# aliftffd/ViT-vs-Raw-IQ

Hardware: AMD Instinct MI355X
Metric: IQ frames/sec training (fwd+loss+bwd+clip+AdamW) (higher is better)
Workload: dtype bf16; 1 GPU; ViT-Tiny/16 224x224 C=1 19cls (BASELINE configs[1]); config_id=B, per_gpu_batch=256, global_batch=256, parallelism=dp1, hipgraph=True

## Files before the change

### include/iqvit.h

```cpp
#ifndef IQVIT_H
#define IQVIT_H
#include <stddef.h>
#include <stdint.h>

#ifdef __cplusplus
extern "C" {
#endif

typedef void* iq_stream_t;

enum { IQ_STATUS_OK = 0, IQ_STATUS_ARG = 1, IQ_STATUS_UNSUPPORTED = 2, IQ_STATUS_LAUNCH = 3 };

typedef struct iq_dropout {
  uint64_t seed;
  uint32_t step;
  uint32_t site;
  float p;
  const uint32_t* step_dev;
} iq_dropout_t;
#define IQ_SITE_IMPAIR 0xFFFFFFFFu
#define IQ_SITE_SYNTH 0xFFFFFFFEu

int iq_ln_supported(int D);
int iq_ln_fwd(const void* z, const float* gamma, const float* beta, void* x, float* mean, float* rstd, int M, int D,
              float eps, iq_stream_t stream);
size_t iq_ln_bwd_ws_bytes(int D);
int iq_ln_bwd(const void* dx, const void* z, const float* mean, const float* rstd, const float* gamma, void* dz,
              void* dy, const iq_dropout_t* drop, float* dgamma, float* dbeta, float* ws, int accumulate, int M,
              int D, iq_stream_t stream);
int iq_ln_bwd_partial_rows(int M, int D);

typedef struct iq_epilogue {
  const float* bias;
  int relu;
  const float* pe;
  int tok, seq, cls_off;
  iq_dropout_t drop;
  const void* gate;
  int ldg;
  float gate_scale;
  const void* residual;
  int ldr;
} iq_epilogue_t;
int iq_gemm_bf16_nt(const void* A, int lda, const void* B, int ldb, void* C, int ldc, int M, int N, int K,
                    const iq_epilogue_t* epi, iq_stream_t stream);

int iq_gemm_ln_supported(int D, int K);
int iq_gemm_bf16_ln(const void* A, int lda, const void* W, int ldw, const float* bias, const void* residual, int ldr,
                    const iq_dropout_t* drop, const float* gamma, const float* beta, float eps, void* Z, void* X,
                    float* mean, float* rstd, int M, int D, int K, iq_stream_t stream);

int iq_gemm_lnbwd_supported(int D, int K);
int iq_gemm_lnbwd_partial_rows(int M);
int iq_gemm_bf16_lnbwd(const void* A, int lda, const void* Wt, int ldw, const void* residual, int ldr, const void* z,
                       const float* mean, const float* rstd, const float* gamma, const iq_dropout_t* drop, void* dz,
                       void* dy, float* partial, int M, int D, int K, iq_stream_t stream);

int iq_ffn_chain_supported(int S, int D, int F);
int iq_ffn_chain_bwd_partial_rows(int M);
size_t iq_ffn_chain_gate_bytes(int M, int F);
int iq_ffn_chain_bwd(const void* dO, const void* W2t, const void* gate_bits, float gate_scale, void* gH, const void* W1t,
                     const void* residual, const void* z1, const float* mean, const float* rstd, const float* gamma,
                     const iq_dropout_t* drop, void* dz, void* dy, float* partial, const void* Wot, void* dA, int frames, int S,
                     int D, int F, iq_stream_t stream);
int iq_qkv_dgrad_ffn_chain_bwd(const void* gQKV, const void* Wqkv_t, const void* residual0, const void* z2, const float* mean2,
                               const float* rstd2, const float* gamma2, const iq_dropout_t* drop2, void* dz2, void* dy2, float* partial2,
                               const void* W2t, const void* gate_bits, float gate_scale, void* gH, const void* W1t, const void* residual,
                               const void* z1, const float* mean, const float* rstd, const float* gamma, const iq_dropout_t* drop, void* dz,
                               void* dy, float* partial, const void* Wot, void* dA, int frames, int S, int D, int F, iq_stream_t stream);
int iq_ffn_chain_fwd(const void* X1, const void* W1, const float* b1, const iq_dropout_t* drop1, void* H, const void* W2,
                     const float* b2, const iq_dropout_t* drop2, const float* gamma, const float* beta, float eps, void* Z,
                     void* X, float* mean, float* rstd, void* gate_bits, int frames, int S, int D, int F, iq_stream_t stream);
int iq_attn_out_ffn_chain_fwd(const void* A, const void* Wo, const float* bo, const iq_dropout_t* drop0, const void* R,
                              const float* gamma1, const float* beta1, void* Z1, void* X1, float* mean1, float* rstd1,
                              const void* W1, const float* b1, const iq_dropout_t* drop1, void* H, const void* W2, const float* b2,
                              const iq_dropout_t* drop2, const float* gamma2, const float* beta2, float eps, void* Z2, void* X,
                              float* mean2, float* rstd2, void* gate_bits, const void* Wq, const float* bq, void* Yq, int frames,
                              int S, int D, int F, iq_stream_t stream);

size_t iq_wgrad_ws_bytes(int M, int N, int K);
int iq_gemm_bf16_wgrad(const void* dY, int ldy, const void* X, int ldx, float* dW, float* dbias, int M, int N, int K,
                       float* ws, size_t ws_bytes, int accumulate, iq_stream_t stream);

typedef struct iq_wgrad_problem {
  const void* dY;
  int ldy;
  const void* X;
  int ldx;
  float* dW;
  float* dbias;
  int N, K;
} iq_wgrad_problem_t;
typedef struct iq_reduce_seg {
  const float* partials;
  int rows;
  int64_t row_stride;
  float* out;
  int64_t n;
} iq_reduce_seg_t;
size_t iq_wgrad_grouped_ws_bytes(const iq_wgrad_problem_t* probs, int nprob, int M, int max_workgroups);
int iq_gemm_bf16_wgrad_grouped(const iq_wgrad_problem_t* probs, int nprob, int M, float* ws, size_t ws_bytes,
                               int accumulate, int max_workgroups, const iq_reduce_seg_t* extra, int nextra,
                               iq_stream_t stream);

#define IQ_REDUCE_JOB_SEGS 12
typedef struct iq_reduce_job_seg {
  const float* partials;
  float* out;
  int64_t n;
  int64_t stride;
  int rows;
  int blk0;
  int tall;
} iq_reduce_job_seg_t;
typedef struct iq_reduce_job {
  iq_reduce_job_seg_t seg[IQ_REDUCE_JOB_SEGS];
  int nseg;
  int nblk;
  int accumulate;
} iq_reduce_job_t;
int iq_gemm_bf16_wgrad_grouped_deferred(const iq_wgrad_problem_t* probs, int nprob, int M, float* ws, size_t ws_bytes,
                                        int accumulate, int max_workgroups, const iq_reduce_seg_t* extra, int nextra,
                                        iq_reduce_job_t* job, iq_stream_t stream);
int iq_reduce_job_run(const iq_reduce_job_t* job, iq_stream_t stream);
int iq_gemm_lnbwd_ride_workgroups(int M, int D, int K, int job_blocks);
int iq_gemm_bf16_lnbwd_ride(const void* A, int lda, const void* Wt, int ldw, const void* residual, int ldr, const void* z,
                            const float* mean, const float* rstd, const float* gamma, const iq_dropout_t* drop, void* dz,
                            void* dy, float* partial, int M, int D, int K, const iq_reduce_job_t* job, iq_stream_t stream);

int iq_attn_supported(int S, int dh);
int iq_attn_fwd(const void* qkv, void* out, float* lse, int B, int S, int H, int dh, iq_stream_t stream);
int iq_attn_bwd(const void* qkv, const void* out, const void* dout, const float* lse, void* dqkv, int B, int S, int H,
                int dh, iq_stream_t stream);
int iq_attn_fwd_masked(const void* qkv, void* out, float* lse, const uint8_t* mask, long mask_hstride, int B, int S,
                       int H, int dh, iq_stream_t stream);
int iq_attn_bwd_masked(const void* qkv, const void* out, const void* dout, const float* lse, void* dqkv,
                       const uint8_t* mask, long mask_hstride, int B, int S, int H, int dh, iq_stream_t stream);
int iq_attn_probs(const void* qkv, const float* lse, float* out, long out_bstride, int B, int S, int H, int dh,
                  int rows, int heads, iq_stream_t stream);
int iq_attn_grad_probs(const void* qkv, const float* lse, const void* dout, float* out, long out_bstride, int B, int S,
                       int H, int dh, int rows, int heads, int positive, iq_stream_t stream);
int iq_attn_relevance_step(const void* qkv, const float* lse, const void* dout, const float* r_in, float* r_out, int B,
                           int S, int H, int dh, iq_stream_t stream);

int iq_frames_preprocess(const float* raw, float* out, int n_frames, int len, int take, const float* stats,
                         iq_stream_t stream);
typedef struct iq_impair {
  float phase_lo, phase_hi;
  float cfo_lo, cfo_hi;
  int   rot90;
  int   conj;
  int   shift_max;
  float gain_db_lo, gain_db_hi;
  float snr_db_lo, snr_db_hi;
  uint64_t seed; uint32_t step;
  uint64_t frame_base;
} iq_impair_t;
int iq_frames_impair(const float* raw, float* out, float* drawn, int n_frames, int len, int take, const float* stats,
                     const iq_impair_t* imp, iq_stream_t stream);
#define IQ_SYNTH_MAX_CLASSES 128
#define IQ_SYNTH_MAX_SNRS 64
typedef struct iq_synth_class { int kind; int offset; int count; } iq_synth_class_t;
typedef struct iq_synth {
  const float* points;
  const iq_synth_class_t* classes; int n_classes;
  const float* snrs_db; int n_snrs;
  int balanced;
  uint64_t seed; uint32_t stream;
  uint64_t frame_base;
} iq_synth_t;
int iq_frames_synth(float* raw , int64_t* labels, float* snr ,
                    float* drawn ,
                    int32_t* symbols , int n_frames, int len, const iq_synth_t* par, iq_stream_t stream);
typedef struct iq_waveform {
  const float* points; const iq_synth_class_t* classes; int n_classes;
  const float* snrs_db; int n_snrs; int balanced;
  uint64_t seed; uint32_t stream; uint64_t frame_base;
  int sps;
  int span;
  int n_phase;
  int timing;
  const float* pulse;
  const int32_t* fpulse;
  int n_taps;
  float los;
  float tap_sigma[8];
} iq_waveform_t;
int iq_frames_waveform(float* raw , int64_t* labels, float* snr, float* drawn ,
                       int32_t* symbols , float* taps , int n_frames, int len,
                       const iq_waveform_t* par, iq_stream_t stream);
enum { IQ_RX_GIVEN = 0, IQ_RX_OERDER_MEYR = 1, IQ_RX_ENERGY = 2 };
typedef struct iq_receiver {
  int sps;
  int span;
  int n_frac;
  int mode;
  int normalise;
  const float* table;
  const int32_t* u;
} iq_receiver_t;
int iq_frames_receive(const float* raw , float* sym , float* est ,
                      float* energy , int n_frames, int len, const iq_receiver_t* par, iq_stream_t stream);
int iq_frames_receive_bwd(const float* dsym , const float* sym, const float* est, float* dx ,
                          int n_frames, int len, const iq_receiver_t* par, iq_stream_t stream);
typedef struct iq_spectrogram {
  int n_fft;
  int hop;
  int pad;
  int width;
  int mode;
  float inv_norm, floor, scale, shift;
} iq_spectrogram_t;
int iq_frames_spectrogram(const float* x , const float* table ,
                          float* out , int n_frames, int len, const iq_spectrogram_t* par,
                          iq_stream_t stream);
int iq_frames_spectrogram_bwd(const float* x, const float* table, const float* dout ,
                              float* dx , int n_frames, int len, const iq_spectrogram_t* par,
                              iq_stream_t stream);
typedef struct iq_cyclic {
  int n_fft;
  int hop;
  int pad;
  int columns;
  int kind;
  int mode;
  float inv_norm, floor, scale, shift;
} iq_cyclic_t;
int iq_frames_cyclic(const float* x , const float* table , const float* rot ,
                     float* out , int n_frames, int len, const iq_cyclic_t* par, iq_stream_t stream);
int iq_frames_cyclic_bwd(const float* x, const float* table, const float* rot, const float* dout ,
                         float* dx , int n_frames, int len, const iq_cyclic_t* par, iq_stream_t stream);
int iq_patchify(const float* src, void* patches, int kind, int B, int C, int H, int W, int p, int Kpad,
                iq_stream_t stream);
int iq_cls_rows(const float* cls, const float* pe, void* x0, int B, int S, int D, const iq_dropout_t* drop,
                iq_stream_t stream);
int iq_embed_bwd_gather(const void* dx0, void* demb, float* dcls, int B, int S, int tok, int D, int has_cls,
                        const iq_dropout_t* drop, int accumulate, iq_stream_t stream);
int iq_embed_dgrad(const void* demb, const void* w_bf16, int Kpad, float* dsrc, int kind, int B, int C, int H, int W, int p,
                   int D, iq_stream_t stream);
int iq_linf_step(float* x_adv, const float* grad, const float* x0, float alpha, float eps, float lo, float hi, size_t n,
                 iq_stream_t stream);

int iq_head_fwd(const void* x, const float* ln_g, const float* ln_b, const float* W, const float* b, float* featn,
                float* hstat, float* logits, int B, int S, int D, int K, int pool, iq_stream_t stream);
int iq_ce_fwd_bwd(const float* logits, const int64_t* labels, int B, int K, float smoothing, float denom,
                  float* loss_sum, int32_t* n_correct, float* dlogits, iq_stream_t stream);
int iq_head_bwd(const float* dlogits, const float* featn, const float* hstat, const float* ln_g, const float* ln_b,
                const float* W, float* dW, float* db, float* dln_g, float* dln_b, void* dx, int B, int S, int D, int K,
                int pool, int accumulate, iq_stream_t stream);

size_t iq_gradnorm_ws_bytes(size_t n);
int iq_gradnorm_sq(const float* g, size_t n, float grad_scale, float* ws, float* out, iq_stream_t stream);
int iq_adamw_step(float* p, const float* g, float* m, float* v, void* shadow_bf16, size_t n, float lr, float beta1,
                  float beta2, float eps, float weight_decay, int step, const float* gnorm_sq, float max_norm,
                  float grad_scale, const float* dyn, iq_stream_t stream);
int iq_counter_add(uint32_t* ctr_u32, uint32_t inc_u32, float* ctr_f32, float inc_f32, iq_stream_t stream);
int iq_cast_bf16(const float* src, void* dst, size_t n, iq_stream_t stream);
int iq_transpose_cast_bf16(const float* src, void* dst, int rows, int cols, iq_stream_t stream);

typedef struct iq_model_cfg {
  int kind;
  int in_channels;
  int img_h, img_w, patch;
  int seq_length, conv_k, use_cls;
  int num_classes, d_model, n_head, n_layers, ffn_hidden;
  float drop_prob;
} iq_model_cfg_t;

typedef struct iq_model iq_model_t;

int iq_model_create(const iq_model_cfg_t* cfg, iq_model_t** out);
void iq_model_destroy(iq_model_t* m);
const char* iq_model_last_error(const iq_model_t* m);
int iq_model_tokens(const iq_model_t* m);
size_t iq_model_param_floats(const iq_model_t* m);
int iq_model_param_entries(const iq_model_t* m);
int iq_model_param_entry(const iq_model_t* m, int i, char* name, int name_cap, size_t* offset, int* ndim, int* dims);
size_t iq_model_shadow_bytes(const iq_model_t* m);
size_t iq_model_workspace_bytes(const iq_model_t* m, int batch, int training);
int iq_model_bind(iq_model_t* m, float* params, float* grads, const float* pe, void* shadow);
int iq_model_bind_step_counter(iq_model_t* m, uint32_t* counter);
int iq_model_refresh_shadow(iq_model_t* m, iq_stream_t stream);
int iq_model_refresh_transposed(iq_model_t* m, iq_stream_t stream);
int iq_model_forward(iq_model_t* m, const float* src, int batch, void* workspace, size_t ws_bytes, int training,
                     uint64_t seed, uint32_t step, float* enc_out, float* logits, iq_stream_t stream);
int iq_model_backward(iq_model_t* m, const float* dlogits, const float* denc, int batch, void* workspace,
                      size_t ws_bytes, int accumulate, int stage_hi, int stage_lo, iq_stream_t stream);
int iq_model_grad_range(const iq_model_t* m, int stage_hi, int stage_lo, size_t* off, size_t* len);
#define IQ_BWD_PARAM_GRADS 1
int iq_model_backward_input(iq_model_t* m, const float* dlogits, const float* denc, int batch, void* workspace,
                            size_t ws_bytes, float* dsrc, int flags, iq_stream_t stream);
int iq_model_attention(iq_model_t* m, const void* workspace, size_t ws_bytes, int batch, int layer, int rows,
                       int heads, float* out, long out_bstride, iq_stream_t stream);
int iq_model_attention_rollout(iq_model_t* m, const void* workspace, size_t ws_bytes, int batch, float alpha,
                               float* out, iq_stream_t stream);
int iq_model_attention_relevance(iq_model_t* m, const float* dlogits, int batch, void* workspace, size_t ws_bytes,
                                 float* rel, float* const* maps, int rows, int heads, int positive, long out_bstride,
                                 iq_stream_t stream);

#define IQ_PROF_FAMILIES 8
int iq_prof_enable(int on);
int iq_prof_collect(double* ms, long long* count);
size_t iq_prof_kernels(char* out, size_t cap, int reset);

#ifdef __cplusplus
}
#endif
#endif
```

### vit-vs-raw-iq_amd/_native.py

```python
from __future__ import annotations

import ctypes as C
import os

_HERE = os.path.dirname(os.path.abspath(__file__))
LIB_PATH = os.environ.get("IQ_LIBIQVIT") or os.path.join(_HERE, "libiqvit.so")

BWD_PARAM_GRADS = 1

STATUS = {0: "ok", 1: "invalid argument", 2: "unsupported shape/configuration", 3: "HIP launch error"}


class IqError(RuntimeError):
    pass


class Dropout(C.Structure):
    _fields_ = [("seed", C.c_uint64), ("step", C.c_uint32), ("site", C.c_uint32), ("p", C.c_float),
                ("step_dev", C.c_void_p)]


class Impair(C.Structure):
    _fields_ = [("phase_lo", C.c_float), ("phase_hi", C.c_float), ("cfo_lo", C.c_float), ("cfo_hi", C.c_float),
                ("rot90", C.c_int), ("conj", C.c_int), ("shift_max", C.c_int), ("gain_db_lo", C.c_float),
                ("gain_db_hi", C.c_float), ("snr_db_lo", C.c_float), ("snr_db_hi", C.c_float), ("seed", C.c_uint64),
                ("step", C.c_uint32), ("frame_base", C.c_uint64)]


class SynthClass(C.Structure):
    _fields_ = [("kind", C.c_int), ("offset", C.c_int), ("count", C.c_int)]


class Synth(C.Structure):
    _fields_ = [("points", C.c_void_p), ("classes", C.POINTER(SynthClass)), ("n_classes", C.c_int),
                ("snrs_db", C.POINTER(C.c_float)), ("n_snrs", C.c_int), ("balanced", C.c_int), ("seed", C.c_uint64),
                ("stream", C.c_uint32), ("frame_base", C.c_uint64)]


class Waveform(C.Structure):
    _fields_ = [("points", C.c_void_p), ("classes", C.POINTER(SynthClass)), ("n_classes", C.c_int),
                ("snrs_db", C.POINTER(C.c_float)), ("n_snrs", C.c_int), ("balanced", C.c_int), ("seed", C.c_uint64),
                ("stream", C.c_uint32), ("frame_base", C.c_uint64), ("sps", C.c_int), ("span", C.c_int), ("n_phase", C.c_int),
                ("timing", C.c_int), ("pulse", C.c_void_p), ("fpulse", C.c_void_p), ("n_taps", C.c_int), ("los", C.c_float),
                ("tap_sigma", C.c_float * 8)]


class Receiver(C.Structure):
    _fields_ = [("sps", C.c_int), ("span", C.c_int), ("n_frac", C.c_int), ("mode", C.c_int), ("normalise", C.c_int),
                ("table", C.c_void_p), ("u", C.c_void_p)]


class Spectrogram(C.Structure):
    _fields_ = [("n_fft", C.c_int), ("hop", C.c_int), ("pad", C.c_int), ("width", C.c_int), ("mode", C.c_int),
                ("inv_norm", C.c_float), ("floor", C.c_float), ("scale", C.c_float), ("shift", C.c_float)]


class Cyclic(C.Structure):
    _fields_ = [("n_fft", C.c_int), ("hop", C.c_int), ("pad", C.c_int), ("columns", C.c_int), ("kind", C.c_int),
                ("mode", C.c_int), ("inv_norm", C.c_float), ("floor", C.c_float), ("scale", C.c_float), ("shift", C.c_float)]


class Epilogue(C.Structure):
    _fields_ = [("bias", C.c_void_p), ("relu", C.c_int), ("pe", C.c_void_p), ("tok", C.c_int), ("seq", C.c_int),
                ("cls_off", C.c_int), ("drop", Dropout), ("gate", C.c_void_p), ("ldg", C.c_int),
                ("gate_scale", C.c_float), ("residual", C.c_void_p), ("ldr", C.c_int)]


class WgradProblem(C.Structure):
    _fields_ = [("dY", C.c_void_p), ("ldy", C.c_int), ("X", C.c_void_p), ("ldx", C.c_int), ("dW", C.c_void_p),
                ("dbias", C.c_void_p), ("N", C.c_int), ("K", C.c_int)]


class ReduceSeg(C.Structure):
    _fields_ = [("partials", C.c_void_p), ("rows", C.c_int), ("row_stride", C.c_int64), ("out", C.c_void_p),
                ("n", C.c_int64)]


class ReduceJobSeg(C.Structure):
    _fields_ = [("partials", C.c_void_p), ("out", C.c_void_p), ("n", C.c_int64), ("stride", C.c_int64), ("rows", C.c_int),
                ("blk0", C.c_int), ("tall", C.c_int)]


class ReduceJob(C.Structure):
    _fields_ = [("seg", ReduceJobSeg * 12), ("nseg", C.c_int), ("nblk", C.c_int), ("accumulate", C.c_int)]


class ModelCfg(C.Structure):
    _fields_ = [("kind", C.c_int), ("in_channels", C.c_int), ("img_h", C.c_int), ("img_w", C.c_int),
                ("patch", C.c_int), ("seq_length", C.c_int), ("conv_k", C.c_int), ("use_cls", C.c_int),
                ("num_classes", C.c_int), ("d_model", C.c_int), ("n_head", C.c_int), ("n_layers", C.c_int),
                ("ffn_hidden", C.c_int), ("drop_prob", C.c_float)]


_P, _I, _Z, _F = C.c_void_p, C.c_int, C.c_size_t, C.c_float
_U64, _U32 = C.c_uint64, C.c_uint32

SIGNATURES = {
    "iq_ln_supported": (_I, [_I]),
    "iq_ln_fwd": (_I, [_P, _P, _P, _P, _P, _P, _I, _I, _F, _P]),
    "iq_ln_bwd_ws_bytes": (_Z, [_I]),
    "iq_ln_bwd_partial_rows": (_I, [_I, _I]),
    "iq_ln_bwd": (_I, [_P, _P, _P, _P, _P, _P, _P, C.POINTER(Dropout), _P, _P, _P, _I, _I, _I, _P]),
    "iq_gemm_bf16_nt": (_I, [_P, _I, _P, _I, _P, _I, _I, _I, _I, C.POINTER(Epilogue), _P]),
    "iq_gemm_ln_supported": (_I, [_I, _I]),
    "iq_gemm_bf16_ln": (_I, [_P, _I, _P, _I, _P, _P, _I, C.POINTER(Dropout), _P, _P, _F, _P, _P, _P, _P, _I, _I, _I, _P]),
    "iq_gemm_lnbwd_supported": (_I, [_I, _I]),
    "iq_gemm_lnbwd_partial_rows": (_I, [_I]),
    "iq_gemm_bf16_lnbwd": (_I, [_P, _I, _P, _I, _P, _I, _P, _P, _P, _P, C.POINTER(Dropout), _P, _P, _P, _I, _I, _I, _P]),
    "iq_ffn_chain_supported": (_I, [_I, _I, _I]),
    "iq_ffn_chain_bwd_partial_rows": (_I, [_I]),
    "iq_ffn_chain_bwd": (_I, [_P, _P, _P, _F, _P, _P, _P, _P, _P, _P, _P, C.POINTER(Dropout), _P, _P, _P, _P, _P, _I, _I, _I, _I, _P]),
    "iq_qkv_dgrad_ffn_chain_bwd": (_I, [_P, _P, _P, _P, _P, _P, _P, C.POINTER(Dropout), _P, _P, _P,
                                        _P, _P, _F, _P, _P, _P, _P, _P, _P, _P, C.POINTER(Dropout), _P, _P, _P, _P, _P, _I, _I, _I, _I, _P]),
    "iq_ffn_chain_gate_bytes": (_Z, [_I, _I]),
    "iq_ffn_chain_fwd": (_I, [_P, _P, _P, C.POINTER(Dropout), _P, _P, _P, C.POINTER(Dropout), _P, _P, _F, _P, _P, _P, _P, _P, _I, _I,
                              _I, _I, _P]),
    "iq_attn_out_ffn_chain_fwd": (_I, [_P, _P, _P, C.POINTER(Dropout), _P, _P, _P, _P, _P, _P, _P,
                                       _P, _P, C.POINTER(Dropout), _P, _P, _P, C.POINTER(Dropout), _P, _P, _F, _P, _P, _P, _P, _P,
                                       _P, _P, _P, _I, _I, _I, _I, _P]),
    "iq_wgrad_ws_bytes": (_Z, [_I, _I, _I]),
    "iq_gemm_bf16_wgrad": (_I, [_P, _I, _P, _I, _P, _P, _I, _I, _I, _P, _Z, _I, _P]),
    "iq_wgrad_grouped_ws_bytes": (_Z, [_P, _I, _I, _I]),
    "iq_gemm_bf16_wgrad_grouped": (_I, [_P, _I, _I, _P, _Z, _I, _I, _P, _I, _P]),
    "iq_gemm_bf16_wgrad_grouped_deferred": (_I, [_P, _I, _I, _P, _Z, _I, _I, _P, _I, C.POINTER(ReduceJob), _P]),
    "iq_reduce_job_run": (_I, [C.POINTER(ReduceJob), _P]),
    "iq_gemm_bf16_lnbwd_ride": (_I, [_P, _I, _P, _I, _P, _I, _P, _P, _P, _P, C.POINTER(Dropout), _P, _P, _P, _I, _I, _I,
                                     C.POINTER(ReduceJob), _P]),
    "iq_gemm_lnbwd_ride_workgroups": (_I, [_I, _I, _I, _I]),
    "iq_attn_supported": (_I, [_I, _I]),
    "iq_attn_fwd": (_I, [_P, _P, _P, _I, _I, _I, _I, _P]),
    "iq_attn_bwd": (_I, [_P, _P, _P, _P, _P, _I, _I, _I, _I, _P]),
    "iq_attn_fwd_masked": (_I, [_P, _P, _P, _P, C.c_long, _I, _I, _I, _I, _P]),
    "iq_attn_bwd_masked": (_I, [_P, _P, _P, _P, _P, _P, C.c_long, _I, _I, _I, _I, _P]),
    "iq_attn_probs": (_I, [_P, _P, _P, C.c_long, _I, _I, _I, _I, _I, _I, _P]),
    "iq_attn_grad_probs": (_I, [_P, _P, _P, _P, C.c_long, _I, _I, _I, _I, _I, _I, _I, _P]),
    "iq_attn_relevance_step": (_I, [_P, _P, _P, _P, _P, _I, _I, _I, _I, _P]),
    "iq_frames_preprocess": (_I, [_P, _P, _I, _I, _I, C.POINTER(C.c_float), _P]),
    "iq_frames_impair": (_I, [_P, _P, _P, _I, _I, _I, C.POINTER(C.c_float), C.POINTER(Impair), _P]),
    "iq_frames_synth": (_I, [_P, _P, _P, _P, _P, _I, _I, C.POINTER(Synth), _P]),
    "iq_frames_waveform": (_I, [_P, _P, _P, _P, _P, _P, _I, _I, C.POINTER(Waveform), _P]),
    "iq_frames_receive": (_I, [_P, _P, _P, _P, _I, _I, C.POINTER(Receiver), _P]),
    "iq_frames_receive_bwd": (_I, [_P, _P, _P, _P, _I, _I, C.POINTER(Receiver), _P]),
    "iq_frames_spectrogram": (_I, [_P, _P, _P, _I, _I, C.POINTER(Spectrogram), _P]),
    "iq_frames_spectrogram_bwd": (_I, [_P, _P, _P, _P, _I, _I, C.POINTER(Spectrogram), _P]),
    "iq_frames_cyclic": (_I, [_P, _P, _P, _P, _I, _I, C.POINTER(Cyclic), _P]),
    "iq_frames_cyclic_bwd": (_I, [_P, _P, _P, _P, _P, _I, _I, C.POINTER(Cyclic), _P]),
    "iq_patchify": (_I, [_P, _P, _I, _I, _I, _I, _I, _I, _I, _P]),
    "iq_cls_rows": (_I, [_P, _P, _P, _I, _I, _I, C.POINTER(Dropout), _P]),
    "iq_embed_bwd_gather": (_I, [_P, _P, _P, _I, _I, _I, _I, _I, C.POINTER(Dropout), _I, _P]),
    "iq_embed_dgrad": (_I, [_P, _P, _I, _P, _I, _I, _I, _I, _I, _I, _I, _P]),
    "iq_linf_step": (_I, [_P, _P, _P, _F, _F, _F, _F, _Z, _P]),
    "iq_head_fwd": (_I, [_P, _P, _P, _P, _P, _P, _P, _P, _I, _I, _I, _I, _I, _P]),
    "iq_ce_fwd_bwd": (_I, [_P, _P, _I, _I, _F, _F, _P, _P, _P, _P]),
    "iq_head_bwd": (_I, [_P, _P, _P, _P, _P, _P, _P, _P, _P, _P, _P, _I, _I, _I, _I, _I, _I, _P]),
    "iq_gradnorm_ws_bytes": (_Z, [_Z]),
    "iq_gradnorm_sq": (_I, [_P, _Z, _F, _P, _P, _P]),
    "iq_adamw_step": (_I, [_P, _P, _P, _P, _P, _Z, _F, _F, _F, _F, _F, _I, _P, _F, _F, _P, _P]),
    "iq_counter_add": (_I, [_P, _U32, _P, _F, _P]),
    "iq_cast_bf16": (_I, [_P, _P, _Z, _P]),
    "iq_transpose_cast_bf16": (_I, [_P, _P, _I, _I, _P]),
    "iq_model_create": (_I, [C.POINTER(ModelCfg), C.POINTER(_P)]),
    "iq_model_destroy": (None, [_P]),
    "iq_model_last_error": (C.c_char_p, [_P]),
    "iq_model_tokens": (_I, [_P]),
    "iq_model_param_floats": (_Z, [_P]),
    "iq_model_param_entries": (_I, [_P]),
    "iq_model_param_entry": (_I, [_P, _I, C.c_char_p, _I, C.POINTER(_Z), C.POINTER(_I), C.POINTER(_I)]),
    "iq_model_shadow_bytes": (_Z, [_P]),
    "iq_model_workspace_bytes": (_Z, [_P, _I, _I]),
    "iq_model_bind": (_I, [_P, _P, _P, _P, _P]),
    "iq_model_bind_step_counter": (_I, [_P, _P]),
    "iq_model_refresh_shadow": (_I, [_P, _P]),
    "iq_model_refresh_transposed": (_I, [_P, _P]),
    "iq_model_forward": (_I, [_P, _P, _I, _P, _Z, _I, _U64, _U32, _P, _P, _P]),
    "iq_model_backward": (_I, [_P, _P, _P, _I, _P, _Z, _I, _I, _I, _P]),
    "iq_model_grad_range": (_I, [_P, _I, _I, C.POINTER(_Z), C.POINTER(_Z)]),
    "iq_model_backward_input": (_I, [_P, _P, _P, _I, _P, _Z, _P, _I, _P]),
    "iq_model_attention": (_I, [_P, _P, _Z, _I, _I, _I, _I, _P, C.c_long, _P]),
    "iq_model_attention_rollout": (_I, [_P, _P, _Z, _I, _F, _P, _P]),
    "iq_model_attention_relevance": (_I, [_P, _P, _I, _P, _Z, _P, C.POINTER(_P), _I, _I, _I, C.c_long, _P]),
    "iq_prof_enable": (_I, [_I]),
    "iq_prof_collect": (_I, [C.POINTER(C.c_double), C.POINTER(C.c_longlong)]),
    "iq_prof_kernels": (_Z, [C.c_char_p, _Z, _I]),
}

_lib = None


def lib():
    global _lib
    if _lib is None:
        if not os.path.exists(LIB_PATH):
            raise IqError(
                f"{LIB_PATH} not found: the HIP extension is not built. Run "
                "`python -c 'import __graft_entry__ as g; g.build()'` (or `make -C vit-vs-raw-iq_amd/csrc`). "
                "There is no CPU fallback.")
        L = C.CDLL(LIB_PATH)
        for name, (res, args) in SIGNATURES.items():
            fn = getattr(L, name)
            fn.restype = res
            fn.argtypes = args
        _lib = L
    return _lib


def check(rc, what, model=None):
    if rc != 0:
        detail = ""
        if model is not None:
            msg = lib().iq_model_last_error(model)
            if msg:
                detail = ": " + msg.decode()
        raise IqError(f"{what} failed: {STATUS.get(rc, rc)}{detail}")


def ptr(t):
    return None if t is None else t.data_ptr()


def stream_handle():
    import torch
    return torch.cuda.current_stream().cuda_stream
```

### vit-vs-raw-iq_amd/csrc/layernorm.hip

```cpp
#include "common.h"
#include "iqvit.h"
#include "prof.h"

namespace {

template <int LPR>
__device__ __forceinline__ float group_sum(float v) {
#pragma unroll
  for (int o = LPR / 2; o > 0; o >>= 1) v += __shfl_xor(v, o, 64);
  return v;
}

constexpr int LN_THREADS = 256;

template <int LPR, int NV, bool MASK = false>
__global__ __launch_bounds__(LN_THREADS) void ln_fwd_kernel(const bf16* __restrict__ Z, const float* __restrict__ gamma,
                                                            const float* __restrict__ beta, bf16* __restrict__ X,
                                                            float* __restrict__ mean_out, float* __restrict__ rstd_out,
                                                            int M, int D, float eps) {
  constexpr int RPW = 64 / LPR;
  constexpr int RPB = RPW * (LN_THREADS / 64);
  const int lane = threadIdx.x & 63, wave = threadIdx.x >> 6;
  const int j = lane % LPR, rsub = lane / LPR;
  float g[NV][8], b[NV][8];
#pragma unroll
  for (int v = 0; v < NV; ++v) {
    const int c = (v * LPR + j) * 8;
    const bool cv = !MASK || c < D;
#pragma unroll
    for (int e = 0; e < 8; ++e) { g[v][e] = cv ? gamma[c + e] : 0.f; b[v][e] = cv ? beta[c + e] : 0.f; }
  }
  const float invD = 1.0f / (float)D;
  for (long row0 = (long)blockIdx.x * RPB; row0 < M; row0 += (long)gridDim.x * RPB) {
    const long row = row0 + wave * RPW + rsub;
    const bool ok = row < M;
    float x[NV][8];
    float s = 0.f;
#pragma unroll
    for (int v = 0; v < NV; ++v) {
      bf16x8 t = {};
      if (ok && (!MASK || (v * LPR + j) * 8 < D)) t = *reinterpret_cast<const bf16x8*>(Z + row * D + (v * LPR + j) * 8);
      unpack8(t, x[v]);
#pragma unroll
      for (int e = 0; e < 8; ++e) s += x[v][e];
    }
    const float mean = group_sum<LPR>(s) * invD;
    float q = 0.f;
#pragma unroll
    for (int v = 0; v < NV; ++v)
#pragma unroll
      for (int e = 0; e < 8; ++e) { float d = x[v][e] - mean; q += (!MASK || (v * LPR + j) * 8 < D) ? d * d : 0.f; }
    const float var = group_sum<LPR>(q) * invD;
    const float rstd = 1.0f / sqrtf(var + eps);
    if (ok) {
#pragma unroll
      for (int v = 0; v < NV; ++v) {
        float y[8];
#pragma unroll
        for (int e = 0; e < 8; ++e) y[e] = g[v][e] * ((x[v][e] - mean) * rstd) + b[v][e];
        if (!MASK || (v * LPR + j) * 8 < D) *reinterpret_cast<bf16x8*>(X + row * D + (v * LPR + j) * 8) = pack8(y);
      }
      if (j == 0) { mean_out[row] = mean; rstd_out[row] = rstd; }
    }
  }
}

template <int LPR, int NV, bool DROP, bool MASK = false>
__global__ __launch_bounds__(LN_THREADS) void ln_bwd_kernel(const bf16* __restrict__ dX, const bf16* __restrict__ Z,
                                                            const float* __restrict__ mean_in, const float* __restrict__ rstd_in,
                                                            const float* __restrict__ gamma, bf16* __restrict__ dZ,
                                                            bf16* __restrict__ dY, IqRng rng, uint32_t thresh, float dscale,
                                                            float* __restrict__ partial, int M, int D) {
  constexpr int RPW = 64 / LPR;
  constexpr int RPB = RPW * (LN_THREADS / 64);
  extern __shared__ __attribute__((aligned(16))) float red[];
  const int lane = threadIdx.x & 63, wave = threadIdx.x >> 6;
  const int j = lane % LPR, rsub = lane / LPR;
  float g[NV][8], ag[NV][8], ab[NV][8];
#pragma unroll
  for (int v = 0; v < NV; ++v) {
    const int c = (v * LPR + j) * 8;
#pragma unroll
    for (int e = 0; e < 8; ++e) { g[v][e] = (!MASK || c < D) ? gamma[c + e] : 0.f; ag[v][e] = 0.f; ab[v][e] = 0.f; }
  }
  const float invD = 1.0f / (float)D;
  if (DROP) rng = rng_resolve(rng);
  for (long row0 = (long)blockIdx.x * RPB; row0 < M; row0 += (long)gridDim.x * RPB) {
    const long row = row0 + wave * RPW + rsub;
    const bool ok = row < M;
    float xh[NV][8], dy[NV][8];
    float mean = 0.f, rstd = 0.f;
    if (ok) { mean = mean_in[row]; rstd = rstd_in[row]; }
    float s1 = 0.f, s2 = 0.f;
#pragma unroll
    for (int v = 0; v < NV; ++v) {
      bf16x8 tz = {}, td = {};
      const bool cv = !MASK || (v * LPR + j) * 8 < D;
      if (ok && cv) {
        tz = *reinterpret_cast<const bf16x8*>(Z + row * D + (v * LPR + j) * 8);
        td = *reinterpret_cast<const bf16x8*>(dX + row * D + (v * LPR + j) * 8);
      }
      unpack8(tz, xh[v]);
      unpack8(td, dy[v]);
#pragma unroll
      for (int e = 0; e < 8; ++e) {
        xh[v][e] = cv ? (xh[v][e] - mean) * rstd : 0.f;
        ag[v][e] += dy[v][e] * xh[v][e];
        ab[v][e] += dy[v][e];
        dy[v][e] *= g[v][e];
        s1 += dy[v][e];
        s2 += dy[v][e] * xh[v][e];
      }
    }
    const float c1 = group_sum<LPR>(s1) * invD;
    const float c2 = group_sum<LPR>(s2) * invD;
    if (ok) {
#pragma unroll
      for (int v = 0; v < NV; ++v) {
        float o[8];
#pragma unroll
        for (int e = 0; e < 8; ++e) o[e] = rstd * (dy[v][e] - c1 - xh[v][e] * c2);
        const long off = row * D + (v * LPR + j) * 8;
        if (MASK && (v * LPR + j) * 8 >= D) continue;
        *reinterpret_cast<bf16x8*>(dZ + off) = pack8(o);
        if (DROP) {
          const uint32_t keep = dropout_keep8(rng, (uint64_t)off >> 3, thresh);
#pragma unroll
          for (int e = 0; e < 8; ++e) o[e] = ((keep >> e) & 1u) ? o[e] * dscale : 0.f;
          *reinterpret_cast<bf16x8*>(dY + off) = pack8(o);
        }
      }
    }
  }
  const int rslot = wave * RPW + rsub;
#pragma unroll
  for (int v = 0; v < NV; ++v) {
    const int c = (v * LPR + j) * 8;
    if (MASK && c >= D) continue;
#pragma unroll
    for (int e = 0; e < 8; ++e) {
      red[rslot * 2 * D + c + e] = ag[v][e];
      red[rslot * 2 * D + D + c + e] = ab[v][e];
    }
  }
  __syncthreads();
  for (int c = threadIdx.x; c < 2 * D; c += LN_THREADS) {
    float s = 0.f;
    for (int r = 0; r < RPB; ++r) s += red[r * 2 * D + c];
    partial[(long)blockIdx.x * 2 * D + c] = s;
  }
}

__global__ __launch_bounds__(1024) void ln_bwd_reduce_kernel(const float* __restrict__ partial, int nblk, int D,
                                                             float* __restrict__ dgamma, float* __restrict__ dbeta,
                                                             int accumulate) {
  __shared__ float sm[32][33];
  const int cl = threadIdx.x & 31, sl = threadIdx.x >> 5;
  const int c = blockIdx.x * 32 + cl;
  float s = 0.f;
  if (c < 2 * D) {
#pragma unroll 4
    for (int b = sl; b < nblk; b += 32) s += partial[(long)b * 2 * D + c];
  }
  sm[sl][cl] = s;
  __syncthreads();
  if (sl == 0 && c < 2 * D) {
    float t = 0.f;
#pragma unroll
    for (int i = 0; i < 32; ++i) t += sm[i][cl];
    float* dst = c < D ? dgamma + c : dbeta + (c - D);
    *dst = accumulate ? *dst + t : t;
  }
}

struct LnShape { int lpr, nv; };
inline bool ln_shape(int D, LnShape* s) {
  if (D <= 0 || D % 8) return false;
  int v = D / 8, lpr = 1;
  while (lpr < 64 && v % (lpr * 2) == 0) lpr *= 2;
  s->lpr = lpr; s->nv = v / lpr;
  return true;
}

template <typename F>
inline bool ln_dispatch(const LnShape& s, F&& f) {
#define IQ_LN_CASE(L, N) \
  if (s.lpr == L && s.nv == N) { f(std::integral_constant<int, L>{}, std::integral_constant<int, N>{}); return true; }
  IQ_LN_CASE(64, 1) IQ_LN_CASE(64, 2) IQ_LN_CASE(64, 3) IQ_LN_CASE(64, 4)
  IQ_LN_CASE(32, 1) IQ_LN_CASE(32, 3) IQ_LN_CASE(32, 5)
  IQ_LN_CASE(16, 1) IQ_LN_CASE(16, 3) IQ_LN_CASE(16, 5)
  IQ_LN_CASE(8, 1) IQ_LN_CASE(8, 3) IQ_LN_CASE(8, 5)
  IQ_LN_CASE(4, 1) IQ_LN_CASE(4, 3) IQ_LN_CASE(4, 5)
  IQ_LN_CASE(2, 1) IQ_LN_CASE(2, 3) IQ_LN_CASE(1, 1) IQ_LN_CASE(1, 3)
#undef IQ_LN_CASE
  return false;
}
inline int ln_masked_nv(int D) { return (D % 8 == 0 && D > 0 && D <= 2048) ? (D / 8 + 63) / 64 : 0; }
template <typename F>
inline bool ln_dispatch_masked(int D, F&& f) {
  switch (ln_masked_nv(D)) {
    case 1: f(std::integral_constant<int, 1>{}); return true;
    case 2: f(std::integral_constant<int, 2>{}); return true;
    case 3: f(std::integral_constant<int, 3>{}); return true;
    case 4: f(std::integral_constant<int, 4>{}); return true;
    default: return false;
  }
}

constexpr int LN_MAX_BLOCKS = 512;
constexpr int LN_FWD_MAX_BLOCKS = 4096;

inline int ln_grid(int M, int rpb, int cap = LN_MAX_BLOCKS) {
  long nb = ((long)M + rpb - 1) / rpb;
  if (nb > cap) nb = cap;
  if (nb < 1) nb = 1;
  return (int)nb;
}

}

extern "C" int iq_ln_supported(int D) {
  LnShape s;
  if (!ln_shape(D, &s)) return 0;
  return (ln_dispatch(s, [](auto, auto) {}) || ln_masked_nv(D) > 0) ? 1 : 0;
}

extern "C" int iq_ln_fwd(const void* z, const float* gamma, const float* beta, void* x, float* mean, float* rstd,
                         int M, int D, float eps, iq_stream_t stream) {
  LnShape s;
  if (M <= 0) return IQ_OK;
  if (!z || !gamma || !beta || !x || !mean || !rstd) return IQ_ERR_ARG;
  if (!ln_shape(D, &s)) return IQ_ERR_UNSUPPORTED;
  hipStream_t st = (hipStream_t)stream;
  IQ_PROF(IQ_FAM_LN_FWD, st);
  const double bytes = 2.0 * (double)M * D * 2 + 8.0 * M;
  bool ok = ln_dispatch(s, [&](auto lpr, auto nv) {
    constexpr int LPR = decltype(lpr)::value, NV = decltype(nv)::value;
    IQ_PROF_K(bytes, 0.0, "ln_fwd_kernel<%d, %d, false>", LPR, NV);
    ln_fwd_kernel<LPR, NV><<<ln_grid(M, (64 / LPR) * 4, LN_FWD_MAX_BLOCKS), LN_THREADS, 0, st>>>((const bf16*)z, gamma, beta, (bf16*)x, mean,
                                                                             rstd, M, D, eps);
  });
  if (!ok) ok = ln_dispatch_masked(D, [&](auto nv) {
    constexpr int NV = decltype(nv)::value;
    IQ_PROF_K(bytes, 0.0, "ln_fwd_kernel<64, %d, true>", NV);
    ln_fwd_kernel<64, NV, true><<<ln_grid(M, 4, LN_FWD_MAX_BLOCKS), LN_THREADS, 0, st>>>((const bf16*)z, gamma, beta, (bf16*)x,
                                                                                         mean, rstd, M, D, eps);
  });
  return ok ? iq_launch_status() : IQ_ERR_UNSUPPORTED;
}

extern "C" size_t iq_ln_bwd_ws_bytes(int D) { return (size_t)LN_MAX_BLOCKS * 2 * D * sizeof(float); }

extern "C" int iq_ln_bwd_partial_rows(int M, int D) {
  LnShape s;
  if (M <= 0 || !ln_shape(D, &s)) return 0;
  int rows = 0;
  bool ok = ln_dispatch(s, [&](auto lpr, auto nv) {
    constexpr int LPR = decltype(lpr)::value;
    rows = ln_grid(M, (64 / LPR) * 4);
  });
  if (!ok) rows = ln_masked_nv(D) > 0 ? ln_grid(M, 4) : 0;
  return rows;
}

extern "C" int iq_ln_bwd(const void* dx, const void* z, const float* mean, const float* rstd, const float* gamma,
                         void* dz, void* dy, const iq_dropout_t* drop, float* dgamma, float* dbeta, float* ws,
                         int accumulate, int M, int D, iq_stream_t stream) {
  LnShape s;
  if (M <= 0) return IQ_OK;
  if (!dx || !z || !mean || !rstd || !gamma || !dz || !ws) return IQ_ERR_ARG;
  if ((dgamma == nullptr) != (dbeta == nullptr)) return IQ_ERR_ARG;
  const bool reduce_now = dgamma != nullptr;
  if (!ln_shape(D, &s)) return IQ_ERR_UNSUPPORTED;
  int dropping; IqRng rng; uint32_t thresh; float dscale;
  (void)dropout_unpack(drop, &dropping, &rng, &thresh, &dscale);
  if (dropping && !dy) return IQ_ERR_ARG;
  hipStream_t st = (hipStream_t)stream;
  IQ_PROF(IQ_FAM_LN_BWD, st);
  const double bytes = 2.0 * (double)M * D * (3 + (dropping ? 1 : 0)) + 8.0 * M;
  int rc = IQ_OK;
  bool ok = ln_dispatch(s, [&](auto lpr, auto nv) {
    constexpr int LPR = decltype(lpr)::value, NV = decltype(nv)::value;
    constexpr int RPB = (64 / LPR) * 4;
    const int nblk = ln_grid(M, RPB);
    const size_t lds = (size_t)RPB * 2 * D * sizeof(float);
    if (lds > 160 * 1024) { rc = IQ_ERR_UNSUPPORTED; return; }
    IQ_PROF_K(bytes, 0.0, "ln_bwd_kernel<%d, %d, %s, false>", LPR, NV, dropping ? "true" : "false");
    if (dropping) {
      auto k = ln_bwd_kernel<LPR, NV, true>;
      if (lds > 48 * 1024) (void)hipFuncSetAttribute((const void*)k, hipFuncAttributeMaxDynamicSharedMemorySize, (int)lds);
      k<<<nblk, LN_THREADS, lds, st>>>((const bf16*)dx, (const bf16*)z, mean, rstd, gamma, (bf16*)dz, (bf16*)dy, rng,
                                       thresh, dscale, ws, M, D);
    } else {
      auto k = ln_bwd_kernel<LPR, NV, false>;
      if (lds > 48 * 1024) (void)hipFuncSetAttribute((const void*)k, hipFuncAttributeMaxDynamicSharedMemorySize, (int)lds);
      k<<<nblk, LN_THREADS, lds, st>>>((const bf16*)dx, (const bf16*)z, mean, rstd, gamma, (bf16*)dz, (bf16*)dy, rng,
                                       thresh, dscale, ws, M, D);
    }
    if (reduce_now) ln_bwd_reduce_kernel<<<(2 * D + 31) / 32, 1024, 0, st>>>(ws, nblk, D, dgamma, dbeta, accumulate);
  });
  if (!ok) ok = ln_dispatch_masked(D, [&](auto nv) {
    constexpr int NV = decltype(nv)::value;
    constexpr int RPB = 4;
    const int nblk = ln_grid(M, RPB);
    const size_t lds = (size_t)RPB * 2 * D * sizeof(float);
    IQ_PROF_K(bytes, 0.0, "ln_bwd_kernel<64, %d, %s, true>", NV, dropping ? "true" : "false");
    if (dropping)
      ln_bwd_kernel<64, NV, true, true><<<nblk, LN_THREADS, lds, st>>>((const bf16*)dx, (const bf16*)z, mean, rstd, gamma,
                                                                      (bf16*)dz, (bf16*)dy, rng, thresh, dscale, ws, M, D);
    else
      ln_bwd_kernel<64, NV, false, true><<<nblk, LN_THREADS, lds, st>>>((const bf16*)dx, (const bf16*)z, mean, rstd, gamma,
                                                                       (bf16*)dz, (bf16*)dy, rng, thresh, dscale, ws, M, D);
    if (reduce_now) ln_bwd_reduce_kernel<<<(2 * D + 31) / 32, 1024, 0, st>>>(ws, nblk, D, dgamma, dbeta, accumulate);
  });
  if (!ok) return IQ_ERR_UNSUPPORTED;
  return rc != IQ_OK ? rc : iq_launch_status();
}
```

### vit-vs-raw-iq_amd/csrc/misc.hip

```cpp
#include "common.h"
#include "iqvit.h"
#include "prof.h"

namespace {

__global__ void patchify_kernel(const float* __restrict__ src, bf16* __restrict__ dst, int kind, int B, int C, int H,
                                int W, int p, int tok, int P, int Kpad) {
  const long nchunk = (long)B * tok * (Kpad / 8);
  for (long id = (long)blockIdx.x * blockDim.x + threadIdx.x; id < nchunk; id += (long)gridDim.x * blockDim.x) {
    const int ch = (int)(id % (Kpad / 8));
    const long row = id / (Kpad / 8);
    const int b = (int)(row / tok), t = (int)(row % tok);
    float v[8];
    if (kind == 0 && (p & 7) == 0 && (W & 3) == 0 && ch * 8 < P) {
      const int k = ch * 8, gw = W / p;
      const int c = k / (p * p), rem = k % (p * p), py = rem / p, px = rem % p;
      const int gy = t / gw, gx = t % gw;
      const float* sp = src + (((long)b * C + c) * H + gy * p + py) * W + gx * p + px;
      const f32x4 a = *reinterpret_cast<const f32x4*>(sp), bq = *reinterpret_cast<const f32x4*>(sp + 4);
      v[0] = a[0]; v[1] = a[1]; v[2] = a[2]; v[3] = a[3]; v[4] = bq[0]; v[5] = bq[1]; v[6] = bq[2]; v[7] = bq[3];
      *reinterpret_cast<bf16x8*>(dst + row * Kpad + ch * 8) = pack8(v);
      continue;
    }
#pragma unroll
    for (int e = 0; e < 8; ++e) {
      const int k = ch * 8 + e;
      float x = 0.f;
      if (k < P) {
        if (kind == 0) {
          const int gw = W / p;
          const int c = k / (p * p), rem = k % (p * p), py = rem / p, px = rem % p;
          const int gy = t / gw, gx = t % gw;
          x = src[(((long)b * C + c) * H + gy * p + py) * W + gx * p + px];
        } else {
          const int c = k / p, j = k % p;
          x = src[((long)b * C + c) * H + (long)t * p + j];
        }
      }
      v[e] = x;
    }
    *reinterpret_cast<bf16x8*>(dst + row * Kpad + ch * 8) = pack8(v);
  }
}

__global__ void cls_rows_kernel(const float* __restrict__ cls, const float* __restrict__ pe, bf16* __restrict__ x0,
                                int B, int S, int D, int drop_on, IqRng rng, uint32_t thresh, float dscale) {
  const int nch = D / 8;
  const int id = blockIdx.x * blockDim.x + threadIdx.x;
  if (id >= B * nch) return;
  if (drop_on) rng = rng_resolve(rng);
  const int b = id / nch, ch = id % nch;
  float v[8];
#pragma unroll
  for (int e = 0; e < 8; ++e) v[e] = cls[ch * 8 + e] + pe[ch * 8 + e];
  const long off = (long)b * S * D + ch * 8;
  if (drop_on) {
    const uint32_t keep = dropout_keep8(rng, (uint64_t)off >> 3, thresh);
#pragma unroll
    for (int e = 0; e < 8; ++e) v[e] = ((keep >> e) & 1u) ? v[e] * dscale : 0.f;
  }
  *reinterpret_cast<bf16x8*>(x0 + off) = pack8(v);
}

__global__ void embed_bwd_gather_kernel(const bf16* __restrict__ dx0, bf16* __restrict__ demb, int B, int S, int tok,
                                        int D, int cls_off, int drop_on, IqRng rng, uint32_t thresh, float dscale) {
  const int nch = D / 8;
  const long n = (long)B * tok * nch;
  if (drop_on) rng = rng_resolve(rng);
  for (long id = (long)blockIdx.x * blockDim.x + threadIdx.x; id < n; id += (long)gridDim.x * blockDim.x) {
    const int ch = (int)(id % nch);
    const long row = id / nch;
    const int b = (int)(row / tok), t = (int)(row % tok);
    const long off = ((long)b * S + cls_off + t) * D + ch * 8;
    bf16x8 v = *reinterpret_cast<const bf16x8*>(dx0 + off);
    if (drop_on) {
      const uint32_t keep = dropout_keep8(rng, (uint64_t)off >> 3, thresh);
      float f[8];
      unpack8(v, f);
#pragma unroll
      for (int e = 0; e < 8; ++e) f[e] = ((keep >> e) & 1u) ? f[e] * dscale : 0.f;
      v = pack8(f);
    }
    *reinterpret_cast<bf16x8*>(demb + row * D + ch * 8) = v;
  }
}

__global__ __launch_bounds__(256) void dcls_kernel(const bf16* __restrict__ dx0, float* __restrict__ dcls, int B, int S, int D,
                                                   int drop_on, IqRng rng, uint32_t thresh, float dscale, int accumulate) {
  __shared__ float part[4][8];
  const int ch = blockIdx.x, lane = threadIdx.x & 63, wave = threadIdx.x >> 6;
  if (drop_on) rng = rng_resolve(rng);
  float s[8] = {0.f, 0.f, 0.f, 0.f, 0.f, 0.f, 0.f, 0.f};
  for (int b = threadIdx.x; b < B; b += 256) {
    const long off = (long)b * S * D + ch * 8;
    float v[8];
    unpack8(*reinterpret_cast<const bf16x8*>(dx0 + off), v);
    uint32_t keep = 0xffu;
    if (drop_on) keep = dropout_keep8(rng, (uint64_t)off >> 3, thresh);
#pragma unroll
    for (int e = 0; e < 8; ++e) s[e] += ((keep >> e) & 1u) ? (drop_on ? v[e] * dscale : v[e]) : 0.f;
  }
#pragma unroll
  for (int e = 0; e < 8; ++e) {
    const float t = wave_sum(s[e]);
    if (lane == 0) part[wave][e] = t;
  }
  __syncthreads();
  if (threadIdx.x < 8) {
    const float t = part[0][threadIdx.x] + part[1][threadIdx.x] + part[2][threadIdx.x] + part[3][threadIdx.x];
    float* dst = dcls + ch * 8 + threadIdx.x;
    *dst = accumulate ? *dst + t : t;
  }
}

__global__ __launch_bounds__(64) void head_fwd_kernel(const bf16* __restrict__ x, const float* __restrict__ ln_g,
                                                      const float* __restrict__ ln_b, const float* __restrict__ W,
                                                      const float* __restrict__ bias, float* __restrict__ feat_hat,
                                                      float* __restrict__ hstat, float* __restrict__ logits, int S,
                                                      int D, int K, int pool) {
  const int b = blockIdx.x, lane = threadIdx.x;
  const bf16* xb = x + (long)b * S * D;
  float* fh = feat_hat + (long)b * D;
  float s1 = 0.f;
  for (int d = lane; d < D; d += 64) {
    float f;
    if (pool == 0) {
      f = (float)xb[d];
    } else {
      f = 0.f;
      for (int s = 0; s < S; ++s) f += (float)xb[(long)s * D + d];
      f /= (float)S;
    }
    fh[d] = f;
    s1 += f;
  }
  if (ln_g) {
    const float mean = wave_sum(s1) / (float)D;
    float s2 = 0.f;
    for (int d = lane; d < D; d += 64) { const float c = fh[d] - mean; s2 += c * c; }
    const float rstd = 1.0f / sqrtf(wave_sum(s2) / (float)D + 1e-5f);
    for (int d = lane; d < D; d += 64) fh[d] = (fh[d] - mean) * rstd;
    if (lane == 0) { hstat[2 * b] = mean; hstat[2 * b + 1] = rstd; }
  }
  __syncthreads();
  if (D % 4 == 0 && D <= 1024) {
    __shared__ float fs[1024];
    for (int d = lane; d < D; d += 64) fs[d] = ln_g ? ln_g[d] * fh[d] + ln_b[d] : fh[d];
    __syncthreads();
    int lpk = 64;
    while (lpk * 4 > D) lpk >>= 1;
    if (lpk >= 1) {
      const int kpar = 64 / lpk, kk = lane / lpk, dl = lane % lpk;
      for (int k0 = 0; k0 < K; k0 += kpar * 4) {
        float a[4] = {0.f, 0.f, 0.f, 0.f};
#pragma unroll
        for (int u = 0; u < 4; ++u) {
          const int k = min(k0 + u * kpar + kk, K - 1);
          for (int d = 4 * dl; d < D; d += 4 * lpk) {
            const f32x4 w = *reinterpret_cast<const f32x4*>(W + (long)k * D + d);
            const f32x4 f = *reinterpret_cast<const f32x4*>(fs + d);
            a[u] += w[0] * f[0] + w[1] * f[1] + w[2] * f[2] + w[3] * f[3];
          }
        }
#pragma unroll
        for (int u = 0; u < 4; ++u) {
          float t = a[u];
          for (int o = lpk >> 1; o > 0; o >>= 1) t += __shfl_xor(t, o, 64);
          const int k = k0 + u * kpar + kk;
          if (dl == 0 && k < K) logits[(long)b * K + k] = t + bias[k];
        }
      }
      return;
    }
  }
  for (int k = 0; k < K; ++k) {
    float a = 0.f;
    for (int d = lane; d < D; d += 64) {
      const float f = ln_g ? ln_g[d] * fh[d] + ln_b[d] : fh[d];
      a += f * W[(long)k * D + d];
    }
    a = wave_sum(a);
    if (lane == 0) logits[(long)b * K + k] = a + bias[k];
  }
}

template <int KMAX>
__global__ __launch_bounds__(256) void ce_kernel(const float* __restrict__ logits, const int64_t* __restrict__ labels,
                                                 int B, int K, float smoothing, float denom,
                                                 float* __restrict__ loss_sum, int32_t* __restrict__ n_correct,
                                                 float* __restrict__ dlogits) {
  __shared__ float sl[256];
  __shared__ int sc[256];
  float lacc = 0.f;
  int cacc = 0;
  for (int b = threadIdx.x; b < B; b += blockDim.x) {
    const float* z = logits + (long)b * K;
    const int y = (int)labels[b];
    const bool y_ok = y >= 0 && y < K;
    if constexpr (KMAX > 0) {
      float zr[KMAX];
#pragma unroll
      for (int k = 0; k < KMAX; ++k) zr[k] = k < K ? z[k] : -3.0e38f;
      float mx = zr[0];
      int am = 0;
#pragma unroll
      for (int k = 1; k < KMAX; ++k)
        if (zr[k] > mx) { mx = zr[k]; am = k; }
      float se = 0.f, sz = 0.f, zy = 0.f;
      float ek[KMAX];
#pragma unroll
      for (int k = 0; k < KMAX; ++k) {
        ek[k] = k < K ? expf(zr[k] - mx) : 0.f;
        se += ek[k];
        sz += k < K ? zr[k] : 0.f;
        zy = k == y ? zr[k] : zy;
      }
      const float lse = mx + logf(se);
      const float sum_logp = sz - (float)K * lse;
      const float nll = y_ok ? -(zy - lse) : __builtin_nanf("");
      lacc += (1.0f - smoothing) * nll + smoothing * (-sum_logp / (float)K);
      cacc += (am == y) ? 1 : 0;
      if (dlogits) {
        const float inv = 1.0f / se;
#pragma unroll
        for (int k = 0; k < KMAX; ++k) {
          if (k < K) {
            const float tgt = (k == y ? 1.0f - smoothing : 0.f) + smoothing / (float)K;
            dlogits[(long)b * K + k] = y_ok ? (ek[k] * inv - tgt) / denom : __builtin_nanf("");
          }
        }
      }
    } else {
      float mx = z[0];
      int am = 0;
      for (int k = 1; k < K; ++k)
        if (z[k] > mx) { mx = z[k]; am = k; }
      float se = 0.f;
      for (int k = 0; k < K; ++k) se += expf(z[k] - mx);
      const float lse = mx + logf(se);
      float sum_logp = 0.f;
      for (int k = 0; k < K; ++k) sum_logp += z[k] - lse;
      const float nll = y_ok ? -(z[y] - lse) : __builtin_nanf("");
      lacc += (1.0f - smoothing) * nll + smoothing * (-sum_logp / (float)K);
      cacc += (am == y) ? 1 : 0;
      if (dlogits) {
        for (int k = 0; k < K; ++k) {
          const float pk = expf(z[k] - lse);
          const float tgt = (k == y ? 1.0f - smoothing : 0.f) + smoothing / (float)K;
          dlogits[(long)b * K + k] = y_ok ? (pk - tgt) / denom : __builtin_nanf("");
        }
      }
    }
  }
  sl[threadIdx.x] = lacc;
  sc[threadIdx.x] = cacc;
  __syncthreads();
  for (int o = 128; o > 0; o >>= 1) {
    if ((int)threadIdx.x < o) { sl[threadIdx.x] += sl[threadIdx.x + o]; sc[threadIdx.x] += sc[threadIdx.x + o]; }
    __syncthreads();
  }
  if (threadIdx.x == 0) {
    if (loss_sum) *loss_sum += sl[0];
    if (n_correct) *n_correct += sc[0];
  }
}

__global__ __launch_bounds__(256) void head_bwd_dx_kernel(const float* __restrict__ dlogits, const float* __restrict__ feat_hat,
                                                         const float* __restrict__ hstat, const float* __restrict__ ln_g,
                                                         const float* __restrict__ W, bf16* __restrict__ dx, int S,
                                                         int D, int K, int pool) {
  extern __shared__ float df[];
  const int b = blockIdx.x, lane = threadIdx.x & 63;
  const float* dl = dlogits + (long)b * K;
  const float* fh = feat_hat + (long)b * D;
  if (threadIdx.x < 64) {
    float s1 = 0.f, s2 = 0.f;
    for (int d = lane; d < D; d += 64) {
      float a = 0.f;
      for (int k = 0; k < K; ++k) a += dl[k] * W[(long)k * D + d];
      if (ln_g) {
        a *= ln_g[d];
        s1 += a;
        s2 += a * fh[d];
      }
      df[d] = a;
    }
    if (ln_g) {
      const float c1 = wave_sum(s1) / (float)D, c2 = wave_sum(s2) / (float)D;
      const float rstd = hstat[2 * b + 1];
      for (int d = lane; d < D; d += 64) df[d] = rstd * (df[d] - c1 - fh[d] * c2);
    }
  }
  __syncthreads();
  bf16* dxb = dx + (long)b * S * D;
  const float inv = 1.0f / (float)S;
  for (long i = threadIdx.x; i < (long)S * (D / 8); i += 256) {
    const int s = (int)(i / (D / 8)), ch = (int)(i % (D / 8));
    float v[8];
#pragma unroll
    for (int e = 0; e < 8; ++e) v[e] = pool == 0 ? (s == 0 ? df[ch * 8 + e] : 0.f) : df[ch * 8 + e] * inv;
    *reinterpret_cast<bf16x8*>(dxb + (long)s * D + ch * 8) = pack8(v);
  }
}

__global__ __launch_bounds__(256) void head_bwd_w_kernel(const float* __restrict__ dlogits, const float* __restrict__ feat_hat,
                                                         const float* __restrict__ ln_g, const float* __restrict__ ln_b,
                                                         const float* __restrict__ W, float* __restrict__ dW, float* __restrict__ db,
                                                         float* __restrict__ dln_g, float* __restrict__ dln_b, int B, int D, int K,
                                                         int accumulate) {
  __shared__ float sa[8][33], sb[8][33];
  const int ol = threadIdx.x & 31, sl = threadIdx.x >> 5;
  const int id = blockIdx.x * 32 + ol;
  const int k = id / D, d = id % D;
  const bool live = k < K || (k == K && ln_g);
  float a = 0.f, b2 = 0.f;
  if (live) {
    if (k < K) {
      const float g = ln_g ? ln_g[d] : 1.f, be = ln_g ? ln_b[d] : 0.f;
#pragma unroll 4
      for (int b = sl; b < B; b += 8) {
        const float dl = dlogits[(long)b * K + k];
        a += dl * (g * feat_hat[(long)b * D + d] + be);
        b2 += dl;
      }
    } else {
      for (int b = sl; b < B; b += 8) {
        float dfn = 0.f;
        for (int kk = 0; kk < K; ++kk) dfn += dlogits[(long)b * K + kk] * W[(long)kk * D + d];
        a += dfn * feat_hat[(long)b * D + d];
        b2 += dfn;
      }
    }
  }
  sa[sl][ol] = a;
  sb[sl][ol] = b2;
  __syncthreads();
  if (sl == 0 && live) {
    float ta = 0.f, tb = 0.f;
#pragma unroll
    for (int i = 0; i < 8; ++i) { ta += sa[i][ol]; tb += sb[i][ol]; }
    if (k < K) {
      dW[(long)k * D + d] = accumulate ? dW[(long)k * D + d] + ta : ta;
      if (d == 0) db[k] = accumulate ? db[k] + tb : tb;
    } else {
      dln_g[d] = accumulate ? dln_g[d] + ta : ta;
      dln_b[d] = accumulate ? dln_b[d] + tb : tb;
    }
  }
}

template <int KMAX>
__global__ __launch_bounds__(256) void head_bwd_w2_kernel(const float* __restrict__ dlogits, const float* __restrict__ feat_hat,
                                                          const float* __restrict__ ln_g, const float* __restrict__ ln_b,
                                                          const float* __restrict__ W, float* __restrict__ dW, float* __restrict__ db,
                                                          float* __restrict__ dln_g, float* __restrict__ dln_b, int B, int D, int K,
                                                          int accumulate) {
  __shared__ float sT[8][KMAX][33];
  __shared__ float sS[8][KMAX];
  __shared__ float sdl[64][KMAX];
  const int ol = threadIdx.x & 31, sl = threadIdx.x >> 5;
  const int d = blockIdx.x * 32 + ol;
  const bool live = d < D;
  float T[KMAX], sd[KMAX];
#pragma unroll
  for (int k = 0; k < KMAX; ++k) { T[k] = 0.f; sd[k] = 0.f; }
  for (int b0 = 0; b0 < B; b0 += 64) {
    __syncthreads();
    for (int i = threadIdx.x; i < 64 * KMAX; i += 256) {
      const int bb = i / KMAX, k = i - bb * KMAX;
      sdl[bb][k] = (b0 + bb < B && k < K) ? dlogits[(long)(b0 + bb) * K + k] : 0.f;
    }
    __syncthreads();
    float fv[8];
#pragma unroll
    for (int i = 0; i < 8; ++i) {
      const int bb = sl + 8 * i;
      fv[i] = (live && b0 + bb < B) ? feat_hat[(long)(b0 + bb) * D + d] : 0.f;
    }
#pragma unroll
    for (int i = 0; i < 8; ++i) {
      const int bb = sl + 8 * i;
#pragma unroll
      for (int k = 0; k < KMAX; ++k) {
        const float dl = sdl[bb][k];
        T[k] += dl * fv[i];
        sd[k] += dl;
      }
    }
  }
#pragma unroll
  for (int k = 0; k < KMAX; ++k) {
    sT[sl][k][ol] = T[k];
    if (ol == 0) sS[sl][k] = sd[k];
  }
  __syncthreads();
  if (sl == 0 && live) {
    const float g = ln_g ? ln_g[d] : 1.f, be = ln_g ? ln_b[d] : 0.f;
    float lg = 0.f, lb = 0.f;
    for (int k = 0; k < K; ++k) {
      float t = 0.f, sk = 0.f;
#pragma unroll
      for (int i = 0; i < 8; ++i) { t += sT[i][k][ol]; sk += sS[i][k]; }
      const float v = g * t + be * sk;
      dW[(long)k * D + d] = accumulate ? dW[(long)k * D + d] + v : v;
      if (d == 0) db[k] = accumulate ? db[k] + sk : sk;
      const float w = W[(long)k * D + d];
      lg += w * t;
      lb += w * sk;
    }
    if (ln_g) {
      dln_g[d] = accumulate ? dln_g[d] + lg : lg;
      dln_b[d] = accumulate ? dln_b[d] + lb : lb;
    }
  }
}

constexpr int GN_BLOCKS = 1024;

__global__ __launch_bounds__(256) void gradnorm_partial_kernel(const float* __restrict__ g, size_t n, float scale,
                                                               float* __restrict__ partial) {
  __shared__ float sm[4];
  float s = 0.f;
  const size_t n4 = n / 4;
  for (size_t i = (size_t)blockIdx.x * blockDim.x + threadIdx.x; i < n4; i += (size_t)gridDim.x * blockDim.x) {
    const f32x4 v = reinterpret_cast<const f32x4*>(g)[i];
    s += v[0] * v[0] + v[1] * v[1] + v[2] * v[2] + v[3] * v[3];
  }
  if (blockIdx.x == 0 && threadIdx.x < (n & 3)) { const float v = g[n4 * 4 + threadIdx.x]; s += v * v; }
  s = wave_sum(s);
  if ((threadIdx.x & 63) == 0) sm[threadIdx.x >> 6] = s;
  __syncthreads();
  if (threadIdx.x == 0) partial[blockIdx.x] = (sm[0] + sm[1] + sm[2] + sm[3]) * scale * scale;
}
__global__ __launch_bounds__(256) void gradnorm_final_kernel(const float* __restrict__ partial, int n, float* __restrict__ out) {
  __shared__ float sm[4];
  float s = 0.f;
  for (int i = threadIdx.x; i < n; i += 256) s += partial[i];
  s = wave_sum(s);
  if ((threadIdx.x & 63) == 0) sm[threadIdx.x >> 6] = s;
  __syncthreads();
  if (threadIdx.x == 0) out[0] = sm[0] + sm[1] + sm[2] + sm[3];
}

struct AdamParams {
  float lr, b1, b2, eps, wd, max_norm, grad_scale;
  int step;
  const float* gnorm_sq;
  const float* dyn;
};

__global__ __launch_bounds__(256) void adamw_kernel(float* __restrict__ p, const float* __restrict__ g,
                                                    float* __restrict__ m, float* __restrict__ v,
                                                    bf16* __restrict__ shadow, size_t n, AdamParams a) {
  float lr = a.lr;
  int step = a.step;
  if (a.dyn) { lr = a.dyn[0]; step = (int)a.dyn[1]; }
  float coef = a.grad_scale;
  if (a.gnorm_sq && a.max_norm > 0.f) {
    const float total = sqrtf(a.gnorm_sq[0]);
    coef *= fminf(1.0f, a.max_norm / (total + 1e-6f));
  }
  const float bc1 = 1.0f - powf(a.b1, (float)step);
  const float bc2 = 1.0f - powf(a.b2, (float)step);
  const float step_size = lr / bc1, inv_sqrt_bc2 = 1.0f / sqrtf(bc2), decay = 1.0f - lr * a.wd;
  const size_t n4 = n / 4;
  for (size_t i = (size_t)blockIdx.x * blockDim.x + threadIdx.x; i < n4; i += (size_t)gridDim.x * blockDim.x) {
    f32x4 pv = reinterpret_cast<f32x4*>(p)[i];
    const f32x4 gv = reinterpret_cast<const f32x4*>(g)[i];
    f32x4 mv = reinterpret_cast<f32x4*>(m)[i];
    f32x4 vv = reinterpret_cast<f32x4*>(v)[i];
    bf16x4 sh;
#pragma unroll
    for (int e = 0; e < 4; ++e) {
      const float gg = gv[e] * coef;
      float x = pv[e] * decay;
      mv[e] = a.b1 * mv[e] + (1.0f - a.b1) * gg;
      vv[e] = a.b2 * vv[e] + (1.0f - a.b2) * gg * gg;
      const float den = sqrtf(vv[e]) * inv_sqrt_bc2 + a.eps;
      x -= step_size * (mv[e] / den);
      pv[e] = x;
      sh[e] = (bf16)x;
    }
    reinterpret_cast<f32x4*>(p)[i] = pv;
    reinterpret_cast<f32x4*>(m)[i] = mv;
    reinterpret_cast<f32x4*>(v)[i] = vv;
    if (shadow) reinterpret_cast<bf16x4*>(shadow)[i] = sh;
  }
}

__global__ void counter_add_kernel(uint32_t* cu, uint32_t iu, float* cf, float incf) {
  if (threadIdx.x == 0 && blockIdx.x == 0) {
    if (cu) *cu += iu;
    if (cf) *cf += incf;
  }
}

__global__ __launch_bounds__(256) void cast_kernel(const float* __restrict__ src, bf16* __restrict__ dst, size_t n) {
  const size_t n4 = n / 4;
  for (size_t i = (size_t)blockIdx.x * blockDim.x + threadIdx.x; i < n4; i += (size_t)gridDim.x * blockDim.x) {
    const f32x4 v = reinterpret_cast<const f32x4*>(src)[i];
    bf16x4 o;
#pragma unroll
    for (int e = 0; e < 4; ++e) o[e] = (bf16)v[e];
    reinterpret_cast<bf16x4*>(dst)[i] = o;
  }
  if (blockIdx.x == 0 && threadIdx.x < (n & 3)) dst[n4 * 4 + threadIdx.x] = (bf16)src[n4 * 4 + threadIdx.x];
}

__global__ __launch_bounds__(256) void transpose_cast_kernel(const float* __restrict__ src, bf16* __restrict__ dst,
                                                             int rows, int cols) {
  __shared__ float t[32][33];
  const int bx = blockIdx.x * 32, by = blockIdx.y * 32;
  const int tx = threadIdx.x & 31, ty = threadIdx.x >> 5;
  for (int i = ty; i < 32; i += 8) {
    const int r = by + i, c = bx + tx;
    t[i][tx] = (r < rows && c < cols) ? src[(long)r * cols + c] : 0.f;
  }
  __syncthreads();
  for (int i = ty; i < 32; i += 8) {
    const int c = bx + i, r = by + tx;
    if (c < cols && r < rows) dst[(long)c * rows + r] = (bf16)t[tx][i];
  }
}

inline int grid_for(size_t n, int per_block, int cap) {
  size_t b = (n + per_block - 1) / per_block;
  if (b > (size_t)cap) b = cap;
  if (b < 1) b = 1;
  return (int)b;
}

}

extern "C" int iq_patchify(const float* src, void* patches, int kind, int B, int C, int H, int W, int p, int Kpad,
                           iq_stream_t stream) {
  IQ_PROF(IQ_FAM_MISC, stream);
  if (B <= 0) return IQ_OK;
  if (!src || !patches || C <= 0 || H <= 0 || p <= 0 || (Kpad % 8)) return IQ_ERR_ARG;
  int tok, P;
  if (kind == 0) {
    if (W <= 0) return IQ_ERR_ARG;
    tok = (H / p) * (W / p); P = C * p * p;
  } else if (kind == 1) {
    tok = H / p; P = C * p;
  } else {
    return IQ_ERR_ARG;
  }
  if (tok <= 0 || Kpad < P) return IQ_ERR_ARG;
  const size_t n = (size_t)B * tok * (Kpad / 8);
  patchify_kernel<<<grid_for(n, 256, 4096), 256, 0, (hipStream_t)stream>>>(src, (bf16*)patches, kind, B, C, H, W, p, tok,
                                                                          P, Kpad);
  return iq_launch_status();
}

extern "C" int iq_cls_rows(const float* cls, const float* pe, void* x0, int B, int S, int D, const iq_dropout_t* drop,
                           iq_stream_t stream) {
  IQ_PROF(IQ_FAM_MISC, stream);
  if (B <= 0) return IQ_OK;
  if (!cls || !pe || !x0 || (D % 8)) return IQ_ERR_ARG;
  int on; IqRng r; uint32_t th; float sc;
  (void)dropout_unpack(drop, &on, &r, &th, &sc);
  const int n = B * (D / 8);
  cls_rows_kernel<<<(n + 255) / 256, 256, 0, (hipStream_t)stream>>>(cls, pe, (bf16*)x0, B, S, D, on, r, th, sc);
  return iq_launch_status();
}

extern "C" int iq_embed_bwd_gather(const void* dx0, void* demb, float* dcls, int B, int S, int tok, int D, int has_cls,
                                   const iq_dropout_t* drop, int accumulate, iq_stream_t stream) {
  IQ_PROF(IQ_FAM_MISC, stream);
  if (B <= 0) return IQ_OK;
  if (!dx0 || !demb || (D % 8) || (has_cls && !dcls)) return IQ_ERR_ARG;
  int on; IqRng r; uint32_t th; float sc;
  (void)dropout_unpack(drop, &on, &r, &th, &sc);
  const size_t n = (size_t)B * tok * (D / 8);
  hipStream_t st = (hipStream_t)stream;
  embed_bwd_gather_kernel<<<grid_for(n, 256, 4096), 256, 0, st>>>((const bf16*)dx0, (bf16*)demb, B, S, tok, D,
                                                                  has_cls ? 1 : 0, on, r, th, sc);
  if (has_cls) dcls_kernel<<<D / 8, 256, 0, st>>>((const bf16*)dx0, dcls, B, S, D, on, r, th, sc, accumulate);
  return iq_launch_status();
}

extern "C" int iq_head_fwd(const void* x, const float* ln_g, const float* ln_b, const float* W, const float* b,
                           float* featn, float* hstat, float* logits, int B, int S, int D, int K, int pool,
                           iq_stream_t stream) {
  IQ_PROF(IQ_FAM_MISC, stream);
  if (B <= 0) return IQ_OK;
  if (!x || !W || !b || !featn || !logits || (ln_g && (!ln_b || !hstat))) return IQ_ERR_ARG;
  head_fwd_kernel<<<B, 64, 0, (hipStream_t)stream>>>((const bf16*)x, ln_g, ln_b, W, b, featn, hstat, logits, S, D, K, pool);
  return iq_launch_status();
}

extern "C" int iq_ce_fwd_bwd(const float* logits, const int64_t* labels, int B, int K, float smoothing, float denom,
                             float* loss_sum, int32_t* n_correct, float* dlogits, iq_stream_t stream) {
  IQ_PROF(IQ_FAM_MISC, stream);
  if (B <= 0) return IQ_OK;
  if (!logits || !labels || K <= 0 || denom <= 0.f) return IQ_ERR_ARG;
  if (K <= 32) ce_kernel<32><<<1, 256, 0, (hipStream_t)stream>>>(logits, labels, B, K, smoothing, denom, loss_sum, n_correct, dlogits);
  else ce_kernel<0><<<1, 256, 0, (hipStream_t)stream>>>(logits, labels, B, K, smoothing, denom, loss_sum, n_correct, dlogits);
  return iq_launch_status();
}

extern "C" int iq_head_bwd(const float* dlogits, const float* featn, const float* hstat, const float* ln_g,
                           const float* ln_b, const float* W, float* dW, float* db, float* dln_g, float* dln_b,
                           void* dx, int B, int S, int D, int K, int pool, int accumulate, iq_stream_t stream) {
  IQ_PROF(IQ_FAM_MISC, stream);
  if (B <= 0) return IQ_OK;
  if (!dlogits || !featn || !W || !dW || !db || !dx || (D % 8)) return IQ_ERR_ARG;
  if (ln_g && (!ln_b || !hstat || !dln_g || !dln_b)) return IQ_ERR_ARG;
  hipStream_t st = (hipStream_t)stream;
  head_bwd_dx_kernel<<<B, 256, D * sizeof(float), st>>>(dlogits, featn, hstat, ln_g, W, (bf16*)dx, S, D, K, pool);
  if (K <= 32) {
    head_bwd_w2_kernel<32><<<(D + 31) / 32, 256, 0, st>>>(dlogits, featn, ln_g, ln_b, W, dW, db, dln_g, dln_b, B, D, K, accumulate);
  } else {
    const int n = (K + 1) * D;
    head_bwd_w_kernel<<<(n + 31) / 32, 256, 0, st>>>(dlogits, featn, ln_g, ln_b, W, dW, db, dln_g, dln_b, B, D, K, accumulate);
  }
  return iq_launch_status();
}

extern "C" size_t iq_gradnorm_ws_bytes(size_t n) { (void)n; return GN_BLOCKS * sizeof(float); }

extern "C" int iq_gradnorm_sq(const float* g, size_t n, float grad_scale, float* ws, float* out, iq_stream_t stream) {
  IQ_PROF(IQ_FAM_OPT, stream);
  if (!g || !ws || !out || ((uintptr_t)g & 15)) return IQ_ERR_ARG;
  hipStream_t st = (hipStream_t)stream;
  const int nb = grid_for(n / 4 + 1, 256 * 4, GN_BLOCKS);
  gradnorm_partial_kernel<<<nb, 256, 0, st>>>(g, n, grad_scale, ws);
  gradnorm_final_kernel<<<1, 256, 0, st>>>(ws, nb, out);
  return iq_launch_status();
}

extern "C" int iq_adamw_step(float* p, const float* g, float* m, float* v, void* shadow_bf16, size_t n, float lr,
                             float beta1, float beta2, float eps, float weight_decay, int step, const float* gnorm_sq,
                             float max_norm, float grad_scale, const float* dyn, iq_stream_t stream) {
  IQ_PROF(IQ_FAM_OPT, stream);
  if (!p || !g || !m || !v || (n % 4)) return IQ_ERR_ARG;
  if (((uintptr_t)p | (uintptr_t)g | (uintptr_t)m | (uintptr_t)v) & 15) return IQ_ERR_ARG;
  if (step < 1 && !dyn) return IQ_ERR_ARG;
  AdamParams a = {lr, beta1, beta2, eps, weight_decay, max_norm, grad_scale, step, gnorm_sq, dyn};
  adamw_kernel<<<grid_for(n / 4, 256, 2048), 256, 0, (hipStream_t)stream>>>(p, g, m, v, (bf16*)shadow_bf16, n, a);
  return iq_launch_status();
}

extern "C" int iq_counter_add(uint32_t* ctr_u32, uint32_t inc_u32, float* ctr_f32, float inc_f32, iq_stream_t stream) {
  counter_add_kernel<<<1, 64, 0, (hipStream_t)stream>>>(ctr_u32, inc_u32, ctr_f32, inc_f32);
  return iq_launch_status();
}

extern "C" int iq_cast_bf16(const float* src, void* dst, size_t n, iq_stream_t stream) {
  IQ_PROF(IQ_FAM_MISC, stream);
  if (n == 0) return IQ_OK;
  if (!src || !dst || ((uintptr_t)src & 15) || ((uintptr_t)dst & 7)) return IQ_ERR_ARG;
  cast_kernel<<<grid_for(n / 4 + 1, 256, 2048), 256, 0, (hipStream_t)stream>>>(src, (bf16*)dst, n);
  return iq_launch_status();
}

extern "C" int iq_transpose_cast_bf16(const float* src, void* dst, int rows, int cols, iq_stream_t stream) {
  IQ_PROF(IQ_FAM_MISC, stream);
  if (rows <= 0 || cols <= 0) return IQ_OK;
  if (!src || !dst) return IQ_ERR_ARG;
  dim3 grid((cols + 31) / 32, (rows + 31) / 32);
  transpose_cast_kernel<<<grid, 256, 0, (hipStream_t)stream>>>(src, (bf16*)dst, rows, cols);
  return iq_launch_status();
}

__global__ __launch_bounds__(256) void frames_preprocess_kernel(const float* __restrict__ raw, float* __restrict__ out, long n_samp,
                                                                int len, int take, float i_mean, float i_std, float q_mean,
                                                                float q_std) {
  for (long id = (long)blockIdx.x * blockDim.x + threadIdx.x; id < n_samp; id += (long)gridDim.x * blockDim.x) {
    const long f = id / take;
    const int t = (int)(id - f * take);
    const float2 v = *reinterpret_cast<const float2*>(raw + (f * len + t) * 2);
    out[f * 2 * take + t] = (v.x - i_mean) / i_std;
    out[f * 2 * take + take + t] = (v.y - q_mean) / q_std;
  }
}

extern "C" int iq_frames_preprocess(const float* raw, float* out, int n_frames, int len, int take, const float* stats,
                                    iq_stream_t stream) {
  if (n_frames <= 0) return IQ_OK;
  if (!raw || !out || !stats || len <= 0 || take <= 0 || take > len) return IQ_ERR_ARG;
  if (!(stats[1] > 0.f) || !(stats[3] > 0.f)) return IQ_ERR_ARG;
  if ((uintptr_t)raw & 7) return IQ_ERR_ARG;
  hipStream_t st = (hipStream_t)stream;
  IQ_PROF(IQ_FAM_MISC, st);
  const long n = (long)n_frames * take;
  long nb = (n + 255) / 256;
  if (nb > 8192) nb = 8192;
  frames_preprocess_kernel<<<(int)nb, 256, 0, st>>>(raw, out, n, len, take, stats[0], stats[1], stats[2], stats[3]);
  return iq_launch_status();
}

int head_bwd_dx_launch(const float* dlogits, const float* featn, const float* hstat, const float* ln_g, const float* W, void* dx,
                       int B, int S, int D, int K, int pool, hipStream_t st) {
  IQ_PROF(IQ_FAM_MISC, st);
  if (B <= 0) return IQ_OK;
  head_bwd_dx_kernel<<<B, 256, D * sizeof(float), st>>>(dlogits, featn, hstat, ln_g, W, (bf16*)dx, S, D, K, pool);
  return iq_launch_status();
}

int embed_bwd_gather_launch(const void* dx0, void* demb, int B, int S, int tok, int D, int has_cls, const iq_dropout_t* drop,
                            hipStream_t st) {
  IQ_PROF(IQ_FAM_MISC, st);
  if (B <= 0) return IQ_OK;
  int on; IqRng r; uint32_t th; float sc;
  (void)dropout_unpack(drop, &on, &r, &th, &sc);
  const size_t n = (size_t)B * tok * (D / 8);
  embed_bwd_gather_kernel<<<grid_for(n, 256, 4096), 256, 0, st>>>((const bf16*)dx0, (bf16*)demb, B, S, tok, D, has_cls ? 1 : 0,
                                                                  on, r, th, sc);
  return iq_launch_status();
}

__global__ __launch_bounds__(256) void linf_step_kernel(float* __restrict__ x, const float* __restrict__ g, const float* __restrict__ x0,
                                                        float alpha, float eps, float lo, float hi, int has_lo, int has_hi, long n) {
  for (long i = (long)blockIdx.x * blockDim.x + threadIdx.x; i < n; i += (long)gridDim.x * blockDim.x) {
    const float gv = g[i];
    const float s = gv > 0.f ? 1.f : gv < 0.f ? -1.f : 0.f;
    float v = __fadd_rn(x[i], __fmul_rn(alpha, s));
    const float c = x0[i];
    v = fminf(fmaxf(v, __fsub_rn(c, eps)), __fadd_rn(c, eps));
    if (has_lo) v = fmaxf(v, lo);
    if (has_hi) v = fminf(v, hi);
    x[i] = v;
  }
}

extern "C" int iq_linf_step(float* x_adv, const float* grad, const float* x0, float alpha, float eps, float lo, float hi, size_t n,
                            iq_stream_t stream) {
  if (!x_adv || !grad || !x0) return IQ_ERR_ARG;
  if (!(alpha >= 0.f) || !(eps >= 0.f) || !(alpha < INFINITY) || !(eps < INFINITY)) return IQ_ERR_ARG;
  const bool has_lo = lo == lo, has_hi = hi == hi;
  if (has_lo && has_hi && lo > hi) return IQ_ERR_ARG;
  if (n == 0) return IQ_OK;
  hipStream_t st = (hipStream_t)stream;
  IQ_PROF(IQ_FAM_MISC, st);
  linf_step_kernel<<<grid_for(n, 256, 8192), 256, 0, st>>>(x_adv, grad, x0, alpha, eps, lo, hi, has_lo ? 1 : 0, has_hi ? 1 : 0,
                                                           (long)n);
  return iq_launch_status();
}
```

### vit-vs-raw-iq_amd/csrc/model.hip

```cpp
#include <hip/hip_runtime.h>
#include <stdio.h>
#include <string.h>

#include <string>
#include <vector>

#include "attn_maps.h"
#include "common.h"
#include "iqvit.h"
#include "prof.h"

int head_bwd_dx_launch(const float* dlogits, const float* featn, const float* hstat, const float* ln_g, const float* W, void* dx,
                       int B, int S, int D, int K, int pool, hipStream_t st);
int embed_bwd_gather_launch(const void* dx0, void* demb, int B, int S, int tok, int D, int has_cls, const iq_dropout_t* drop,
                            hipStream_t st);

namespace {

struct Entry {
  std::string name;
  size_t off;
  int ndim;
  int dims[4];
};

struct LayerOff {
  size_t wqkv, bqkv, wo, bo, g1, be1, w1, b1, w2, b2, g2, be2, end;
  size_t t_wqkv, t_wo, t_w1, t_w2;
};

inline size_t align_up(size_t v, size_t a) { return (v + a - 1) / a * a; }

struct WsPlan {
  size_t step_ctr, patches, x0, head_feat, head_stat;
  struct L { size_t qkv, att, lse, z1, mean1, rstd1, x1, hid, gate, z2, mean2, rstd2, x2; };
  std::vector<L> layers;
  size_t gA, gB, gAtt, demb, wgrad_ws, wgrad_ws_bytes, ln_part[3], embw_scratch;
  size_t gZ, gY, gZ1, gY1, gH, gQKV;
  size_t total;
};

__global__ void bf16_to_f32_kernel(const bf16* __restrict__ s, float* __restrict__ d, size_t n8) {
  for (size_t i = (size_t)blockIdx.x * blockDim.x + threadIdx.x; i < n8; i += (size_t)gridDim.x * blockDim.x) {
    const bf16x8 v = reinterpret_cast<const bf16x8*>(s)[i];
    f32x4 a = {(float)v[0], (float)v[1], (float)v[2], (float)v[3]};
    f32x4 b = {(float)v[4], (float)v[5], (float)v[6], (float)v[7]};
    reinterpret_cast<f32x4*>(d)[2 * i] = a;
    reinterpret_cast<f32x4*>(d)[2 * i + 1] = b;
  }
}
__global__ void f32_into_bf16_kernel(const float* __restrict__ s, bf16* __restrict__ d, size_t n8, int add) {
  for (size_t i = (size_t)blockIdx.x * blockDim.x + threadIdx.x; i < n8; i += (size_t)gridDim.x * blockDim.x) {
    const f32x4 a = reinterpret_cast<const f32x4*>(s)[2 * i], b = reinterpret_cast<const f32x4*>(s)[2 * i + 1];
    float f[8] = {a[0], a[1], a[2], a[3], b[0], b[1], b[2], b[3]};
    if (add) {
      const bf16x8 o = reinterpret_cast<const bf16x8*>(d)[i];
#pragma unroll
      for (int e = 0; e < 8; ++e) f[e] += (float)o[e];
    }
    reinterpret_cast<bf16x8*>(d)[i] = pack8(f);
  }
}
__global__ void cast_pad_kernel(const float* __restrict__ s, bf16* __restrict__ d, int rows, int cols, int ld) {
  const long n = (long)rows * ld;
  for (long i = (long)blockIdx.x * blockDim.x + threadIdx.x; i < n; i += (long)gridDim.x * blockDim.x) {
    const int r = (int)(i / ld), c = (int)(i % ld);
    d[i] = (bf16)(c < cols ? s[(long)r * cols + c] : 0.f);
  }
}
__global__ void unpad_kernel(const float* __restrict__ s, float* __restrict__ d, int rows, int cols, int ld, int add) {
  const long n = (long)rows * cols;
  for (long i = (long)blockIdx.x * blockDim.x + threadIdx.x; i < n; i += (long)gridDim.x * blockDim.x) {
    const int r = (int)(i / cols), c = (int)(i % cols);
    const float v = s[(long)r * ld + c];
    d[i] = add ? d[i] + v : v;
  }
}
struct TransDesc { unsigned long long src_off, dst_off; int rows, cols, tile0, tiles_x; };
__global__ __launch_bounds__(256) void transpose_table_kernel(const float* __restrict__ params, unsigned char* __restrict__ shadow,
                                                              const TransDesc* __restrict__ tab, int nent) {
  __shared__ float t[32][33];
  int e = 0;
  while (e + 1 < nent && (int)blockIdx.x >= tab[e + 1].tile0) ++e;
  const TransDesc d = tab[e];
  const int local = blockIdx.x - d.tile0;
  const int bx = (local % d.tiles_x) * 32, by = (local / d.tiles_x) * 32;
  const float* src = params + d.src_off;
  bf16* dst = reinterpret_cast<bf16*>(shadow + d.dst_off);
  const int tx = threadIdx.x & 31, ty = threadIdx.x >> 5;
  for (int i = ty; i < 32; i += 8) {
    const int r = by + i, c = bx + tx;
    t[i][tx] = (r < d.rows && c < d.cols) ? src[(long)r * d.cols + c] : 0.f;
  }
  __syncthreads();
  for (int i = ty; i < 32; i += 8) {
    const int c = bx + i, r = by + tx;
    if (c < d.cols && r < d.rows) dst[(long)c * d.rows + r] = (bf16)t[tx][i];
  }
}

__global__ void rel_start_kernel(float* r, int n, int S, int cls) {
  for (int i = blockIdx.x * blockDim.x + threadIdx.x; i < n; i += gridDim.x * blockDim.x) {
    const int k = i % S;
    r[i] = cls ? (k == 0 ? 1.f : 0.f) : 1.0f / S;
  }
}

struct RelHook {
  float* const* maps;
  int rows, heads, positive;
  long bstride;
  float* rel;
  float* r[2];
};

__global__ void set_u32_kernel(uint32_t* p, uint32_t v, int bump) {
  if (threadIdx.x == 0 && blockIdx.x == 0) *p = bump ? *p + 1u : v;
}

inline int blocks_for(size_t n, int cap = 4096) {
  size_t b = (n + 255) / 256;
  if (b > (size_t)cap) b = cap;
  if (b < 1) b = 1;
  return (int)b;
}

}

struct iq_model {
  iq_model_cfg_t c;
  int S, tok, has_cls, P, Ppad, dh, pool, head_ln;
  std::vector<Entry> entries;
  size_t nparam;
  size_t emb_w, emb_b, cls, emb_end;
  std::vector<LayerOff> L;
  size_t hln_g, hln_b, head_w, head_b, head_begin;
  size_t sh_flat, sh_embw, sh_table, shadow_bytes;
  std::vector<TransDesc> ttab;
  int ttiles = 0;
  const void* table_uploaded_to = nullptr;
  float* params = nullptr;
  float* grads = nullptr;
  const float* pe = nullptr;
  unsigned char* shadow = nullptr;
  std::string err;
  uint32_t* step_ctr = nullptr;
  uint64_t last_seed = 0;
  bool last_tr = false;
  bool last_train_fwd = false;
  const void* fwd_ws = nullptr;
  int fwd_batch = 0;

  iq_dropout_t bwd_site(uint32_t id, const uint32_t* step_dev, bool tr) const {
    iq_dropout_t d;
    d.seed = last_seed; d.step = 0; d.site = id; d.p = tr ? c.drop_prob : 0.f; d.step_dev = step_dev;
    return d;
  }

  size_t add(const std::string& name, std::vector<int> dims, size_t& cur, bool aligned = true) {
    if (aligned) cur = align_up(cur, 64);
    Entry e;
    e.name = name; e.off = cur; e.ndim = (int)dims.size();
    size_t n = 1;
    for (int i = 0; i < 4; ++i) { e.dims[i] = i < e.ndim ? dims[i] : 1; n *= (size_t)e.dims[i]; }
    entries.push_back(e);
    cur += n;
    return e.off;
  }
  const bf16* sh(size_t off) const { return reinterpret_cast<const bf16*>(shadow + sh_flat) + off; }
  const bf16* sht(size_t byte_off) const { return reinterpret_cast<const bf16*>(shadow + byte_off); }
};

namespace {

int fail(iq_model* m, int code, const std::string& msg) {
  if (m) m->err = msg;
  return code;
}

WsPlan plan_ws(const iq_model* m, int B) {
  WsPlan w;
  const size_t D = m->c.d_model, F = m->c.ffn_hidden, S = m->S, H = m->c.n_head;
  const size_t M = (size_t)B * S, MT = (size_t)B * m->tok;
  size_t cur = 0;
  auto take = [&](size_t bytes) { size_t o = cur; cur = align_up(cur + bytes, 256); return o; };
  w.step_ctr = take(256);
  w.patches = take(MT * m->Ppad * 2);
  w.x0 = take(M * D * 2);
  w.head_feat = take((size_t)B * D * 4);
  w.head_stat = take((size_t)B * 2 * 4);
  w.layers.resize(m->c.n_layers);
  for (auto& l : w.layers) {
    l.qkv = take(M * 3 * D * 2);
    l.att = take(M * D * 2);
    l.lse = take((size_t)B * H * S * 4);
    l.z1 = take(M * D * 2);
    l.mean1 = take(M * 4);
    l.rstd1 = take(M * 4);
    l.x1 = take(M * D * 2);
    l.hid = take(M * F * 2);
    l.gate = take(iq_ffn_chain_gate_bytes((int)M, (int)F));
    l.z2 = take(M * D * 2);
    l.mean2 = take(M * 4);
    l.rstd2 = take(M * 4);
    l.x2 = take(M * D * 2);
  }
  w.gA = take(M * D * 2);
  w.gB = take(M * D * 2);
  w.gZ = take(M * D * 2);
  w.gY = take(M * D * 2);
  w.gZ1 = take(M * D * 2);
  w.gY1 = take(M * D * 2);
  w.gH = take(M * F * 2);
  w.gQKV = take(M * 3 * D * 2);
  w.gAtt = take(M * D * 2);
  w.demb = take(MT * D * 2);
  size_t wb = 0;
  auto mx = [&](size_t v) { if (v > wb) wb = v; };
  {
    iq_wgrad_problem_t g[4];
    memset(g, 0, sizeof(g));
    g[0].N = (int)D; g[0].K = (int)F;
    g[1].N = (int)F; g[1].K = (int)D;
    g[2].N = (int)D; g[2].K = (int)D;
    g[3].N = (int)(3 * D); g[3].K = (int)D;
    mx(iq_wgrad_grouped_ws_bytes(g, 4, (int)M, 0));
    for (int k = 0; k < 4; ++k) mx(iq_wgrad_grouped_ws_bytes(g + k, 1, (int)M, 0));
  }
  mx(iq_wgrad_ws_bytes((int)MT, (int)D, m->Ppad));
  w.wgrad_ws_bytes = wb;
  w.wgrad_ws = take(wb);
  size_t ln_rows_fused = (size_t)iq_gemm_lnbwd_partial_rows((int)M);
  if ((size_t)iq_ffn_chain_bwd_partial_rows((int)M) > ln_rows_fused) ln_rows_fused = (size_t)iq_ffn_chain_bwd_partial_rows((int)M);
  ln_rows_fused *= 2 * D * sizeof(float);
  const size_t ln_bytes = ln_rows_fused > iq_ln_bwd_ws_bytes((int)D) ? ln_rows_fused : iq_ln_bwd_ws_bytes((int)D);
  for (int k = 0; k < 3; ++k) w.ln_part[k] = take(ln_bytes);
  w.embw_scratch = take((size_t)D * m->Ppad * 4 + 256);
  w.total = cur;
  return w;
}

inline bool use_fused_ln(int D, int K) { return iq_gemm_ln_supported(D, K) && (D <= 192 || K <= 256); }

struct Route {
  bool chain;
  bool chain_takes_qkv_dgrad;
};
inline Route layer_route(int M, int S, int D, int F) {
  Route r;
  r.chain = iq_ffn_chain_supported(S, D, F) && M >= 8192;
  r.chain_takes_qkv_dgrad = r.chain && M <= 32768;
  return r;
}

#define IQ_TRY(expr, what)                                                              \
  do {                                                                                  \
    int rc_ = (expr);                                                                   \
    if (rc_ != IQ_OK) return fail(m, rc_, std::string(what) + " failed (status " + std::to_string(rc_) + ")"); \
  } while (0)

iq_dropout_t site(const iq_model* m, uint64_t seed, const uint32_t* step_dev, uint32_t id, bool training) {
  iq_dropout_t d;
  d.seed = seed; d.step = 0; d.site = id; d.p = training ? m->c.drop_prob : 0.f; d.step_dev = step_dev;
  return d;
}

}

extern "C" int iq_model_create(const iq_model_cfg_t* cfg, iq_model_t** out) {
  if (!cfg || !out) return IQ_ERR_ARG;
  *out = nullptr;
  iq_model* m = new iq_model();
  m->c = *cfg;
  const iq_model_cfg_t& c = m->c;
  auto bad = [&](const char* msg) { fprintf(stderr, "iq_model_create: %s\n", msg); delete m; return IQ_ERR_UNSUPPORTED; };
  if (c.d_model <= 0 || c.n_head <= 0 || c.n_layers < 0 || c.ffn_hidden <= 0 || c.num_classes <= 0 || c.in_channels <= 0)
    { delete m; return IQ_ERR_ARG; }
  if (c.d_model % c.n_head) return bad("d_model must be divisible by n_head");
  m->dh = c.d_model / c.n_head;
  if (m->dh != 16 && m->dh != 32 && m->dh != 64) return bad("head dim (d_model/n_head) must be 16, 32 or 64");
  if (c.ffn_hidden % 8) return bad("ffn_hidden must be a multiple of 8");
  if (!iq_ln_supported(c.d_model)) return bad("d_model not supported by the LayerNorm kernel");
  if (!(c.drop_prob >= 0.f && c.drop_prob < 1.f)) return bad("drop_prob must be in [0,1)");
  if (c.kind == 0) {
    if (c.patch <= 0 || c.img_h < c.patch || c.img_w < c.patch) return bad("bad image / patch size");
    m->tok = (c.img_h / c.patch) * (c.img_w / c.patch);
    m->has_cls = 1;
    m->P = c.in_channels * c.patch * c.patch;
    m->pool = 0;
    m->head_ln = 0;
  } else if (c.kind == 1) {
    if (c.conv_k <= 0 || c.seq_length < c.conv_k || (c.seq_length % c.conv_k)) return bad("bad seq_length / segment_size");
    m->tok = c.seq_length / c.conv_k;
    m->has_cls = c.use_cls ? 1 : 0;
    m->P = c.in_channels * c.conv_k;
    m->pool = m->has_cls ? 0 : 1;
    m->head_ln = 1;
  } else {
    delete m;
    return IQ_ERR_ARG;
  }
  m->S = m->tok + m->has_cls;
  m->Ppad = (int)align_up((size_t)m->P, 32);
  if (!iq_attn_supported(m->S, m->dh)) return bad("sequence too long for the attention backward kernel at this head dim");

  const int D = c.d_model, F = c.ffn_hidden, K = c.num_classes;
  size_t cur = 0;
  const std::string emb = c.kind == 0 ? "encoder.patch_embedding.projection" : "encoder.sequence_embedding.projection";
  if (c.kind == 0) m->emb_w = m->add(emb + ".weight", {D, c.in_channels, c.patch, c.patch}, cur);
  else m->emb_w = m->add(emb + ".weight", {D, c.in_channels, c.conv_k}, cur);
  m->emb_b = m->add(emb + ".bias", {D}, cur);
  m->cls = 0;
  if (m->has_cls) m->cls = m->add("encoder.cls_token", {1, 1, D}, cur);
  cur = align_up(cur, 64);
  m->emb_end = cur;
  m->L.resize(c.n_layers);
  for (int i = 0; i < c.n_layers; ++i) {
    LayerOff& o = m->L[i];
    const std::string p = "encoder.layers." + std::to_string(i) + ".";
    o.wqkv = m->add(p + "attention.w_q.weight", {D, D}, cur);
    m->add(p + "attention.w_k.weight", {D, D}, cur, false);
    m->add(p + "attention.w_v.weight", {D, D}, cur, false);
    o.bqkv = m->add(p + "attention.w_q.bias", {D}, cur);
    m->add(p + "attention.w_k.bias", {D}, cur, false);
    m->add(p + "attention.w_v.bias", {D}, cur, false);
    o.wo = m->add(p + "attention.w_concat.weight", {D, D}, cur);
    o.bo = m->add(p + "attention.w_concat.bias", {D}, cur);
    o.g1 = m->add(p + "norm1.gamma", {D}, cur);
    o.be1 = m->add(p + "norm1.beta", {D}, cur);
    o.w1 = m->add(p + "ffn.linear1.weight", {F, D}, cur);
    o.b1 = m->add(p + "ffn.linear1.bias", {F}, cur);
    o.w2 = m->add(p + "ffn.linear2.weight", {D, F}, cur);
    o.b2 = m->add(p + "ffn.linear2.bias", {D}, cur);
    o.g2 = m->add(p + "norm2.gamma", {D}, cur);
    o.be2 = m->add(p + "norm2.beta", {D}, cur);
    cur = align_up(cur, 64);
    o.end = cur;
  }
  m->head_begin = cur;
  m->hln_g = m->hln_b = 0;
  if (m->head_ln) {
    m->hln_g = m->add("mlp_head.0.weight", {D}, cur);
    m->hln_b = m->add("mlp_head.0.bias", {D}, cur);
    m->head_w = m->add("mlp_head.1.weight", {K, D}, cur);
    m->head_b = m->add("mlp_head.1.bias", {K}, cur);
  } else {
    m->head_w = m->add("mlp_head.weight", {K, D}, cur);
    m->head_b = m->add("mlp_head.bias", {K}, cur);
  }
  m->nparam = align_up(cur, 64);

  size_t sb = 0;
  m->sh_flat = sb; sb = align_up(sb + m->nparam * 2, 256);
  m->sh_embw = sb; sb = align_up(sb + (size_t)D * m->Ppad * 2, 256);
  for (auto& o : m->L) {
    o.t_wqkv = sb; sb = align_up(sb + (size_t)3 * D * D * 2, 256);
    o.t_wo = sb; sb = align_up(sb + (size_t)D * D * 2, 256);
    o.t_w1 = sb; sb = align_up(sb + (size_t)F * D * 2, 256);
    o.t_w2 = sb; sb = align_up(sb + (size_t)D * F * 2, 256);
  }
  for (auto& o : m->L) {
    auto push = [&](size_t src, size_t dst, int rows, int cols) {
      TransDesc d;
      d.src_off = src; d.dst_off = dst; d.rows = rows; d.cols = cols; d.tile0 = m->ttiles; d.tiles_x = (cols + 31) / 32;
      m->ttiles += d.tiles_x * ((rows + 31) / 32);
      m->ttab.push_back(d);
    };
    push(o.wqkv, o.t_wqkv, 3 * D, D);
    push(o.wo, o.t_wo, D, D);
    push(o.w1, o.t_w1, F, D);
    push(o.w2, o.t_w2, D, F);
  }
  m->sh_table = sb; sb = align_up(sb + m->ttab.size() * sizeof(TransDesc) + 64, 256);
  m->shadow_bytes = sb;
  *out = m;
  return IQ_OK;
}

extern "C" void iq_model_destroy(iq_model_t* m) {
  if (!m) return;
  delete m;
}
extern "C" const char* iq_model_last_error(const iq_model_t* m) { return m ? m->err.c_str() : "null model"; }
extern "C" int iq_model_tokens(const iq_model_t* m) { return m ? m->S : 0; }
extern "C" size_t iq_model_param_floats(const iq_model_t* m) { return m ? m->nparam : 0; }
extern "C" int iq_model_param_entries(const iq_model_t* m) { return m ? (int)m->entries.size() : 0; }
extern "C" int iq_model_param_entry(const iq_model_t* m, int i, char* name, int name_cap, size_t* offset, int* ndim,
                                    int* dims) {
  if (!m || i < 0 || i >= (int)m->entries.size() || !name || name_cap <= 0 || !offset || !ndim || !dims) return IQ_ERR_ARG;
  const Entry& e = m->entries[i];
  snprintf(name, (size_t)name_cap, "%s", e.name.c_str());
  *offset = e.off;
  *ndim = e.ndim;
  for (int k = 0; k < 4; ++k) dims[k] = e.dims[k];
  return IQ_OK;
}
extern "C" size_t iq_model_shadow_bytes(const iq_model_t* m) { return m ? m->shadow_bytes : 0; }
extern "C" size_t iq_model_workspace_bytes(const iq_model_t* m, int batch, int training) {
  (void)training;
  if (!m || batch <= 0) return 0;
  return plan_ws(m, batch).total;
}

extern "C" int iq_model_bind(iq_model_t* m, float* params, float* grads, const float* pe, void* shadow) {
  if (!m) return IQ_ERR_ARG;
  if (!params || !pe || !shadow) return fail(m, IQ_ERR_ARG, "bind: params, pe and shadow are required");
  if (((uintptr_t)params | (uintptr_t)grads | (uintptr_t)shadow) & 255) return fail(m, IQ_ERR_ARG, "bind: buffers must be 256 B aligned");
  m->params = params; m->grads = grads; m->pe = pe; m->shadow = (unsigned char*)shadow;
  if (m->table_uploaded_to != shadow && !m->ttab.empty()) {
    if (hipMemcpy(m->shadow + m->sh_table, m->ttab.data(), m->ttab.size() * sizeof(TransDesc), hipMemcpyHostToDevice) != hipSuccess)
      return fail(m, IQ_ERR_LAUNCH, "bind: uploading the transpose table failed");
    m->table_uploaded_to = shadow;
  }
  return IQ_OK;
}

extern "C" int iq_model_bind_step_counter(iq_model_t* m, uint32_t* counter) {
  if (!m) return IQ_ERR_ARG;
  if ((uintptr_t)counter & 3) return fail(m, IQ_ERR_ARG, "bind_step_counter: counter must be 4 B aligned");
  m->step_ctr = counter;
  return IQ_OK;
}

static int refresh_impl(iq_model_t* m, bool cast_flat, iq_stream_t stream) {
  if (!m || !m->params || !m->shadow) return fail(m, IQ_ERR_ARG, "refresh_shadow: model not bound");
  hipStream_t st = (hipStream_t)stream;
  const int D = m->c.d_model;
  if (cast_flat) IQ_TRY(iq_cast_bf16(m->params, m->shadow + m->sh_flat, m->nparam, stream), "cast params");
  IQ_PROF(IQ_FAM_MISC, st);
  cast_pad_kernel<<<blocks_for((size_t)D * m->Ppad), 256, 0, st>>>(m->params + m->emb_w, (bf16*)(m->shadow + m->sh_embw), D,
                                                                  m->P, m->Ppad);
  if (m->ttiles > 0)
    transpose_table_kernel<<<m->ttiles, 256, 0, st>>>(m->params, m->shadow, (const TransDesc*)(m->shadow + m->sh_table),
                                                     (int)m->ttab.size());
  return iq_launch_status();
}

extern "C" int iq_model_refresh_shadow(iq_model_t* m, iq_stream_t stream) { return refresh_impl(m, true, stream); }
extern "C" int iq_model_refresh_transposed(iq_model_t* m, iq_stream_t stream) { return refresh_impl(m, false, stream); }

extern "C" int iq_model_forward(iq_model_t* m, const float* src, int batch, void* workspace, size_t ws_bytes,
                                int training, uint64_t seed, uint32_t step, float* enc_out, float* logits,
                                iq_stream_t stream) {
  if (!m) return IQ_ERR_ARG;
  if (!m->params || !m->shadow || !m->pe) return fail(m, IQ_ERR_ARG, "forward: model not bound");
  if (!src || !workspace || batch <= 0) return fail(m, IQ_ERR_ARG, "forward: bad arguments");
  if ((uintptr_t)workspace & 255) return fail(m, IQ_ERR_ARG, "forward: workspace must be 256 B aligned");
  const WsPlan w = plan_ws(m, batch);
  if (ws_bytes < w.total) return fail(m, IQ_ERR_ARG, "forward: workspace too small");
  hipStream_t st = (hipStream_t)stream;
  unsigned char* ws = (unsigned char*)workspace;
  const iq_model_cfg_t& c = m->c;
  const int D = c.d_model, F = c.ffn_hidden, S = m->S, H = c.n_head, B = batch;
  const int M = B * S, MT = B * m->tok;
  const Route route = layer_route(M, S, D, F);
  const bool tr = training != 0 && c.drop_prob > 0.f;
  uint32_t* step_dev = m->step_ctr ? m->step_ctr : (uint32_t*)(ws + w.step_ctr);
  m->last_tr = tr;
  m->last_train_fwd = true;
  if (tr) {
    set_u32_kernel<<<1, 64, 0, st>>>(step_dev, step, step == 0xFFFFFFFFu ? 1 : 0);
    m->last_seed = seed;
  }
  const float* P = m->params;
  m->fwd_ws = nullptr;

  if (c.kind == 0) IQ_TRY(iq_patchify(src, ws + w.patches, 0, B, c.in_channels, c.img_h, c.img_w, c.patch, m->Ppad, stream), "patchify");
  else IQ_TRY(iq_patchify(src, ws + w.patches, 1, B, c.in_channels, c.seq_length, 0, c.conv_k, m->Ppad, stream), "patchify");
  const iq_dropout_t d0 = site(m, seed, step_dev, 0, tr);
  if (m->has_cls) IQ_TRY(iq_cls_rows(P + m->cls, m->pe, ws + w.x0, B, S, D, &d0, stream), "cls rows");
  {
    iq_epilogue_t e;
    memset(&e, 0, sizeof(e));
    e.bias = P + m->emb_b; e.pe = m->pe; e.tok = m->tok; e.seq = S; e.cls_off = m->has_cls; e.drop = d0;
    IQ_TRY(iq_gemm_bf16_nt(ws + w.patches, m->Ppad, m->shadow + m->sh_embw, m->Ppad, ws + w.x0, D, MT, D, m->Ppad, &e, stream),
           "embedding GEMM");
  }
  const unsigned char* x = ws + w.x0;
  bool qkv_done = false;
  for (int l = 0; l < c.n_layers; ++l) {
    const LayerOff& o = m->L[l];
    const WsPlan::L& a = w.layers[l];
    iq_epilogue_t e;
    if (!qkv_done) {
      memset(&e, 0, sizeof(e));
      e.bias = P + o.bqkv;
      IQ_TRY(iq_gemm_bf16_nt(x, D, m->sh(o.wqkv), D, ws + a.qkv, 3 * D, M, 3 * D, D, &e, stream), "qkv GEMM");
    }
    qkv_done = false;
    IQ_TRY(iq_attn_fwd(ws + a.qkv, ws + a.att, (float*)(ws + a.lse), B, S, H, m->dh, stream), "attention fwd");
    const iq_dropout_t dr1 = site(m, seed, step_dev, 1 + 3 * l, tr);
    const iq_dropout_t drh = site(m, seed, step_dev, 2 + 3 * l, tr);
    const iq_dropout_t dr2 = site(m, seed, step_dev, 3 + 3 * l, tr);
    if (route.chain) {
      const bool next = l + 1 < c.n_layers;
      IQ_TRY(iq_attn_out_ffn_chain_fwd(ws + a.att, m->sh(o.wo), P + o.bo, &dr1, x, P + o.g1, P + o.be1, ws + a.z1, ws + a.x1,
                                       (float*)(ws + a.mean1), (float*)(ws + a.rstd1), m->sh(o.w1), P + o.b1, &drh, ws + a.hid,
                                       m->sh(o.w2), P + o.b2, &dr2, P + o.g2, P + o.be2, 1e-12f, ws + a.z2, ws + a.x2,
                                       (float*)(ws + a.mean2), (float*)(ws + a.rstd2), ws + a.gate,
                                       next ? m->sh(m->L[l + 1].wqkv) : nullptr, next ? P + m->L[l + 1].bqkv : nullptr,
                                       next ? ws + w.layers[l + 1].qkv : nullptr, B, S, D, F, stream),
             "out-proj + norm1 + ffn chain + norm2 (+ next q,k,v)");
      qkv_done = next;
      x = ws + a.x2;
      continue;
    }
    if (use_fused_ln(D, D)) {
      IQ_TRY(iq_gemm_bf16_ln(ws + a.att, D, m->sh(o.wo), D, P + o.bo, x, D, &dr1, P + o.g1, P + o.be1, 1e-12f, ws + a.z1,
                             ws + a.x1, (float*)(ws + a.mean1), (float*)(ws + a.rstd1), M, D, D, stream), "out-proj GEMM + norm1");
    } else {
      memset(&e, 0, sizeof(e));
      e.bias = P + o.bo; e.drop = dr1; e.residual = x; e.ldr = D;
      IQ_TRY(iq_gemm_bf16_nt(ws + a.att, D, m->sh(o.wo), D, ws + a.z1, D, M, D, D, &e, stream), "out-proj GEMM");
      IQ_TRY(iq_ln_fwd(ws + a.z1, P + o.g1, P + o.be1, ws + a.x1, (float*)(ws + a.mean1), (float*)(ws + a.rstd1), M, D, 1e-12f, stream), "norm1");
    }
    memset(&e, 0, sizeof(e));
    e.bias = P + o.b1; e.relu = 1; e.drop = drh;
    IQ_TRY(iq_gemm_bf16_nt(ws + a.x1, D, m->sh(o.w1), D, ws + a.hid, F, M, F, D, &e, stream), "ffn1 GEMM");
    if (use_fused_ln(D, F)) {
      IQ_TRY(iq_gemm_bf16_ln(ws + a.hid, F, m->sh(o.w2), F, P + o.b2, ws + a.x1, D, &dr2, P + o.g2, P + o.be2, 1e-12f,
                             ws + a.z2, ws + a.x2, (float*)(ws + a.mean2), (float*)(ws + a.rstd2), M, D, F, stream), "ffn2 GEMM + norm2");
    } else {
      memset(&e, 0, sizeof(e));
      e.bias = P + o.b2; e.drop = dr2; e.residual = ws + a.x1; e.ldr = D;
      IQ_TRY(iq_gemm_bf16_nt(ws + a.hid, F, m->sh(o.w2), F, ws + a.z2, D, M, D, F, &e, stream), "ffn2 GEMM");
      IQ_TRY(iq_ln_fwd(ws + a.z2, P + o.g2, P + o.be2, ws + a.x2, (float*)(ws + a.mean2), (float*)(ws + a.rstd2), M, D, 1e-12f, stream), "norm2");
    }
    x = ws + a.x2;
  }
  if (logits) {
    IQ_TRY(iq_head_fwd(x, m->head_ln ? P + m->hln_g : nullptr, m->head_ln ? P + m->hln_b : nullptr, P + m->head_w,
                       P + m->head_b, (float*)(ws + w.head_feat), (float*)(ws + w.head_stat), logits, B, S, D,
                       c.num_classes, m->pool, stream), "head");
  }
  if (enc_out) bf16_to_f32_kernel<<<blocks_for((size_t)M * D / 8), 256, 0, st>>>((const bf16*)x, enc_out, (size_t)M * D / 8);
  const int rc = iq_launch_status();
  if (rc == IQ_OK) { m->fwd_ws = workspace; m->fwd_batch = batch; }
  return rc;
}

static int maps_check(iq_model_t* m, const void* workspace, size_t ws_bytes, int batch, const char* what, WsPlan* w) {
  if (!workspace || batch <= 0) return fail(m, IQ_ERR_ARG, std::string(what) + ": bad arguments");
  if (!m->fwd_ws) return fail(m, IQ_ERR_ARG, std::string(what) + ": no forward has run in a workspace");
  if (m->fwd_ws != workspace) return fail(m, IQ_ERR_ARG, std::string(what) + ": the last forward ran in another workspace");
  if (m->fwd_batch != batch)
    return fail(m, IQ_ERR_ARG, std::string(what) + ": the last forward in this workspace had batch " + std::to_string(m->fwd_batch) +
                                   ", not " + std::to_string(batch));
  *w = plan_ws(m, batch);
  if (ws_bytes < w->total) return fail(m, IQ_ERR_ARG, std::string(what) + ": workspace too small");
  return IQ_OK;
}

extern "C" int iq_model_attention(iq_model_t* m, const void* workspace, size_t ws_bytes, int batch, int layer, int rows,
                                  int heads, float* out, long out_bstride, iq_stream_t stream) {
  if (!m) return IQ_ERR_ARG;
  WsPlan w;
  const int rc = maps_check(m, workspace, ws_bytes, batch, "attention", &w);
  if (rc != IQ_OK) return rc;
  if (layer < 0 || layer >= m->c.n_layers) return fail(m, IQ_ERR_ARG, "attention: layer index out of range");
  if (rows < 0 || rows > 2 || heads < 0 || heads > 1) return fail(m, IQ_ERR_ARG, "attention: rows must be 0, 1 or 2 and heads 0 or 1");
  if (!out) return fail(m, IQ_ERR_ARG, "attention: out is NULL");
  const int S = m->S, H = m->c.n_head;
  if (out_bstride < (long)(heads ? 1 : H) * S * (rows == 0 ? S : 1)) return fail(m, IQ_ERR_ARG, "attention: out_bstride too small");
  const unsigned char* ws = (const unsigned char*)workspace;
  const WsPlan::L& a = w.layers[layer];
  IQ_TRY(iq_attn_probs(ws + a.qkv, (const float*)(ws + a.lse), out, out_bstride, batch, S, H, m->dh, rows, heads, stream),
         "attention probabilities");
  return IQ_OK;
}

extern "C" int iq_model_attention_rollout(iq_model_t* m, const void* workspace, size_t ws_bytes, int batch, float alpha,
                                          float* out, iq_stream_t stream) {
  if (!m) return IQ_ERR_ARG;
  WsPlan w;
  const int rc = maps_check(m, workspace, ws_bytes, batch, "attention rollout", &w);
  if (rc != IQ_OK) return rc;
  if (!(alpha >= 0.f && alpha <= 1.f)) return fail(m, IQ_ERR_ARG, "attention rollout: alpha must be in [0, 1]");
  if (!out) return fail(m, IQ_ERR_ARG, "attention rollout: out is NULL");
  const unsigned char* ws = (const unsigned char*)workspace;
  const int L = m->c.n_layers;
  const long qs = L > 1 ? (long)(w.layers[1].qkv - w.layers[0].qkv) : 0, ls = L > 1 ? (long)(w.layers[1].lse - w.layers[0].lse) : 0;
  for (int l = 0; l < L; ++l)
    if ((long)(w.layers[l].qkv - w.layers[0].qkv) != l * qs || (long)(w.layers[l].lse - w.layers[0].lse) != l * ls)
      return fail(m, IQ_ERR_UNSUPPORTED, "attention rollout: workspace layers are not evenly spaced");
  const size_t q0 = L ? w.layers[0].qkv : 0, l0 = L ? w.layers[0].lse : 0;
  IQ_TRY(attn_rollout_launch(ws + q0, qs, ws + l0, ls, L, out, batch, m->S, m->c.n_head, m->dh, m->has_cls, alpha,
                             (hipStream_t)stream),
         "attention rollout");
  return IQ_OK;
}

extern "C" int iq_model_grad_range(const iq_model_t* m, int stage_hi, int stage_lo, size_t* off, size_t* len) {
  if (!m || !off || !len) return IQ_ERR_ARG;
  const int Lr = m->c.n_layers;
  if (stage_lo < 0 || stage_hi > Lr + 1 || stage_lo > stage_hi) return IQ_ERR_ARG;
  auto begin = [&](int s) { return s == 0 ? (size_t)0 : (s <= Lr ? (s == 1 ? m->emb_end : m->L[s - 2].end) : m->head_begin); };
  auto end = [&](int s) { return s == 0 ? m->emb_end : (s <= Lr ? m->L[s - 1].end : m->nparam); };
  *off = begin(stage_lo);
  *len = end(stage_hi) - *off;
  return IQ_OK;
}

static int backward_impl(iq_model_t* m, const float* dlogits, const float* denc, int batch, void* workspace, size_t ws_bytes,
                         int accumulate, int stage_hi, int stage_lo, bool pgrads, iq_stream_t stream,
                         const RelHook* rh = nullptr) {
  if (!m->params || (pgrads && !m->grads) || !m->shadow) return fail(m, IQ_ERR_ARG, "backward: model not bound (grads required)");
  if (!workspace || batch <= 0) return fail(m, IQ_ERR_ARG, "backward: bad arguments");
  const iq_model_cfg_t& c = m->c;
  const int Lr = c.n_layers;
  if (stage_lo < 0 || stage_hi > Lr + 1 || stage_lo > stage_hi) return fail(m, IQ_ERR_ARG, "backward: bad stage range");
  const WsPlan w = plan_ws(m, batch);
  if (ws_bytes < w.total) return fail(m, IQ_ERR_ARG, "backward: workspace too small");
  hipStream_t st = (hipStream_t)stream;
  unsigned char* ws = (unsigned char*)workspace;
  const int D = c.d_model, F = c.ffn_hidden, S = m->S, H = c.n_head, B = batch, K = c.num_classes;
  const int M = B * S, MT = B * m->tok;
  const bool tr = m->last_tr;
  const uint32_t* step_dev = m->step_ctr ? m->step_ctr : (const uint32_t*)(ws + w.step_ctr);
  const float* P = m->params;
  float* G = m->grads;
  float* wws = (float*)(ws + w.wgrad_ws);
  const float dscale = tr ? dropout_scale(c.drop_prob) : 1.f;

  if (stage_hi == Lr + 1) {
    if (!dlogits && !denc) return fail(m, IQ_ERR_ARG, "backward: dlogits or denc required at the head stage");
    if (dlogits && !pgrads) {
      IQ_TRY(head_bwd_dx_launch(dlogits, (const float*)(ws + w.head_feat), (const float*)(ws + w.head_stat),
                                m->head_ln ? P + m->hln_g : nullptr, P + m->head_w, ws + w.gA, B, S, D, K, m->pool, st), "head bwd (dx)");
    } else if (dlogits) {
      IQ_TRY(iq_head_bwd(dlogits, (const float*)(ws + w.head_feat), (const float*)(ws + w.head_stat),
                         m->head_ln ? P + m->hln_g : nullptr, m->head_ln ? P + m->hln_b : nullptr, P + m->head_w,
                         G + m->head_w, G + m->head_b, m->head_ln ? G + m->hln_g : nullptr,
                         m->head_ln ? G + m->hln_b : nullptr, ws + w.gA, B, S, D, K, m->pool, accumulate, stream), "head bwd");
    } else if (!accumulate && pgrads) {
      (void)hipMemsetAsync(G + m->head_begin, 0, (m->nparam - m->head_begin) * sizeof(float), st);
    }
    if (denc) f32_into_bf16_kernel<<<blocks_for((size_t)M * D / 8), 256, 0, st>>>(denc, (bf16*)(ws + w.gA), (size_t)M * D / 8, dlogits ? 1 : 0);
  }
  const bool fuse1 = iq_gemm_lnbwd_supported(D, F) != 0, fuse2 = iq_gemm_lnbwd_supported(D, 3 * D) != 0;
  const Route route = layer_route(M, S, D, F);
  const bool chain = fuse1 && m->last_train_fwd && route.chain;
  bool deferred = false;
  for (int sidx = (stage_hi > Lr ? Lr : stage_hi); sidx >= 1 && sidx >= stage_lo; --sidx) {
    const int l = sidx - 1;
    const LayerOff& o = m->L[l];
    const WsPlan::L& a = w.layers[l];
    const unsigned char* xin = l == 0 ? ws + w.x0 : ws + w.layers[l - 1].x2;
    unsigned char *gZ = ws + w.gZ, *gY = ws + w.gY, *gZ1 = ws + w.gZ1, *gY1 = ws + w.gY1;
    unsigned char *gH = ws + w.gH, *gQKV = ws + w.gQKV;
    iq_epilogue_t e;
    auto ln2_part = [&](int layer) { return (float*)(ws + w.ln_part[(layer & 1) ? 2 : 0]); };
    float* lp2 = ln2_part(l);
    float* lp1 = (float*)(ws + w.ln_part[1]);
    const bool norm2_here = l == Lr - 1 || !fuse2;
    if (norm2_here) {
      const iq_dropout_t dr2 = m->bwd_site(3 + 3 * l, step_dev, tr);
      IQ_TRY(iq_ln_bwd(ws + w.gA, ws + a.z2, (const float*)(ws + a.mean2), (const float*)(ws + a.rstd2), P + o.g2,
                       gZ, gY, &dr2, nullptr, nullptr, lp2, accumulate, M, D, stream), "norm2 bwd");
    }
    const unsigned char* dO2 = tr ? gY : gZ;
    const unsigned char* dAo = tr ? gY1 : gZ1;
    const iq_wgrad_problem_t wg[4] = {
        {dO2, D, ws + a.hid, F, G + o.w2, G + o.b2, D, F},
        {gH, F, ws + a.x1, D, G + o.w1, G + o.b1, F, D},
        {dAo, D, ws + a.att, D, G + o.wo, G + o.bo, D, D},
        {gQKV, 3 * D, xin, D, G + o.wqkv, G + o.bqkv, 3 * D, D}};
    const int rows2 = norm2_here ? iq_ln_bwd_partial_rows(M, D) : deferred ? iq_ffn_chain_bwd_partial_rows(M) : iq_gemm_lnbwd_partial_rows(M);
    const int rows1 = chain ? iq_ffn_chain_bwd_partial_rows(M) : fuse1 ? iq_gemm_lnbwd_partial_rows(M) : iq_ln_bwd_partial_rows(M, D);
    const iq_reduce_seg_t lnseg[4] = {{lp2, rows2, 2L * D, G + o.g2, D}, {lp2 + D, rows2, 2L * D, G + o.be2, D},
                                      {lp1, rows1, 2L * D, G + o.g1, D}, {lp1 + D, rows1, 2L * D, G + o.be1, D}};
    const iq_dropout_t dr1 = m->bwd_site(1 + 3 * l, step_dev, tr);
    if (chain && deferred) {
      const LayerOff& ou = m->L[l + 1];
      const iq_dropout_t dr2b = m->bwd_site(3 + 3 * l, step_dev, tr);
      IQ_TRY(iq_qkv_dgrad_ffn_chain_bwd(gQKV, m->sht(ou.t_wqkv), gZ1, ws + a.z2, (const float*)(ws + a.mean2), (const float*)(ws + a.rstd2),
                                        P + o.g2, &dr2b, gZ, gY, lp2, m->sht(o.t_w2), ws + a.gate, dscale, gH, m->sht(o.t_w1), gZ, ws + a.z1,
                                        (const float*)(ws + a.mean1), (const float*)(ws + a.rstd1), P + o.g1, &dr1, gZ1, gY1, lp1,
                                        m->sht(o.t_wo), ws + w.gAtt, B, S, D, F, stream),
             "qkv dgrad of the layer above + norm2 bwd + ffn chain bwd + norm1 bwd + out-proj dgrad");
    } else if (chain) {
      IQ_TRY(iq_ffn_chain_bwd(dO2, m->sht(o.t_w2), ws + a.gate, dscale, gH, m->sht(o.t_w1), gZ, ws + a.z1, (const float*)(ws + a.mean1),
                              (const float*)(ws + a.rstd1), P + o.g1, &dr1, gZ1, gY1, lp1, m->sht(o.t_wo), ws + w.gAtt, B, S, D, F, stream),
             "ffn chain bwd + norm1 bwd + out-proj dgrad");
    } else {
      memset(&e, 0, sizeof(e));
      e.gate = ws + a.hid; e.ldg = F; e.gate_scale = dscale;
      IQ_TRY(iq_gemm_bf16_nt(dO2, D, m->sht(o.t_w2), D, gH, F, M, F, D, &e, stream), "ffn2 dgrad");
      if (fuse1) {
        IQ_TRY(iq_gemm_bf16_lnbwd(gH, F, m->sht(o.t_w1), F, gZ, D, ws + a.z1, (const float*)(ws + a.mean1),
                                  (const float*)(ws + a.rstd1), P + o.g1, &dr1, gZ1, gY1, lp1, M, D, F, stream), "ffn1 dgrad + norm1 bwd");
      } else {
        memset(&e, 0, sizeof(e));
        e.residual = gZ; e.ldr = D;
        IQ_TRY(iq_gemm_bf16_nt(gH, F, m->sht(o.t_w1), F, ws + w.gB, D, M, D, F, &e, stream), "ffn1 dgrad");
        IQ_TRY(iq_ln_bwd(ws + w.gB, ws + a.z1, (const float*)(ws + a.mean1), (const float*)(ws + a.rstd1), P + o.g1,
                         gZ1, gY1, &dr1, nullptr, nullptr, lp1, accumulate, M, D, stream), "norm1 bwd");
      }
    }
    if (!chain) IQ_TRY(iq_gemm_bf16_nt(dAo, D, m->sht(o.t_wo), D, ws + w.gAtt, D, M, D, D, nullptr, stream), "out-proj dgrad");
    if (rh) {
      const float* lse = (const float*)(ws + a.lse);
      if (rh->maps && rh->maps[l])
        IQ_TRY(iq_attn_grad_probs(ws + a.qkv, lse, ws + w.gAtt, rh->maps[l], rh->bstride, B, S, H, m->dh, rh->rows, rh->heads,
                                  rh->positive, stream), "gradient-weighted attention map");
      if (rh->rel) {
        const int i = Lr - 1 - l;
        IQ_TRY(attn_relevance_step_launch(ws + a.qkv, lse, ws + w.gAtt, i ? rh->r[(i - 1) & 1] : nullptr, l ? rh->r[i & 1] : rh->rel,
                                          B, S, H, m->dh, i ? 0 : m->has_cls ? 1 : 2, st), "relevance step");
      }
      if (l == 0) break;
    }
    IQ_TRY(iq_attn_bwd(ws + a.qkv, ws + a.att, ws + w.gAtt, (const float*)(ws + a.lse), gQKV, B, S, H, m->dh, stream), "attention bwd");
    deferred = l > 0 && fuse2 && chain && route.chain_takes_qkv_dgrad && sidx - 1 >= stage_lo;
    const bool ride = pgrads && l > 0 && fuse2 && !deferred;
    iq_reduce_job_t job;
    if (ride) {
      IQ_TRY(iq_gemm_bf16_wgrad_grouped_deferred(wg, 4, M, wws, w.wgrad_ws_bytes, accumulate, 0, lnseg, 4, &job, stream),
             "layer weight gradients (partial tiles)");
    } else if (pgrads) {
      IQ_TRY(iq_gemm_bf16_wgrad_grouped(wg, 4, M, wws, w.wgrad_ws_bytes, accumulate, 0, lnseg, 4, stream), "layer weight gradients");
    }
    if (deferred) continue;
    if (l > 0 && fuse2) {
      const LayerOff& ob = m->L[l - 1];
      const WsPlan::L& ab = w.layers[l - 1];
      const iq_dropout_t dr2b = m->bwd_site(3 + 3 * (l - 1), step_dev, tr);
      IQ_TRY(iq_gemm_bf16_lnbwd_ride(gQKV, 3 * D, m->sht(o.t_wqkv), 3 * D, gZ1, D, ws + ab.z2, (const float*)(ws + ab.mean2),
                                     (const float*)(ws + ab.rstd2), P + ob.g2, &dr2b, gZ, gY, ln2_part(l - 1), M, D, 3 * D,
                                     ride ? &job : nullptr, stream),
             "qkv dgrad + norm2 bwd of the layer below (+ this layer's slab reduce)");
    } else {
      memset(&e, 0, sizeof(e));
      e.residual = gZ1; e.ldr = D;
      IQ_TRY(iq_gemm_bf16_nt(gQKV, 3 * D, m->sht(o.t_wqkv), 3 * D, ws + w.gA, D, M, D, 3 * D, &e, stream), "qkv dgrad");
    }
  }
  if (stage_lo == 0) {
    const iq_dropout_t dr0 = m->bwd_site(0, step_dev, tr);
    if (!pgrads) {
      IQ_TRY(embed_bwd_gather_launch(ws + w.gA, ws + w.demb, B, S, m->tok, D, m->has_cls, &dr0, st), "embedding bwd gather");
      return iq_launch_status();
    }
    IQ_TRY(iq_embed_bwd_gather(ws + w.gA, ws + w.demb, m->has_cls ? G + m->cls : nullptr, B, S, m->tok, D, m->has_cls,
                               &dr0, accumulate, stream), "embedding bwd gather");
    if (m->Ppad == m->P) {
      IQ_TRY(iq_gemm_bf16_wgrad(ws + w.demb, D, ws + w.patches, m->Ppad, G + m->emb_w, G + m->emb_b, MT, D, m->Ppad, wws,
                                w.wgrad_ws_bytes, accumulate, stream), "embedding wgrad");
    } else {
      float* scratch = (float*)(ws + w.embw_scratch);
      if (accumulate) (void)hipMemsetAsync(scratch, 0, (size_t)D * m->Ppad * sizeof(float), st);
      IQ_TRY(iq_gemm_bf16_wgrad(ws + w.demb, D, ws + w.patches, m->Ppad, scratch, G + m->emb_b, MT, D, m->Ppad, wws,
                                w.wgrad_ws_bytes, accumulate, stream), "embedding wgrad");
      unpad_kernel<<<blocks_for((size_t)D * m->P), 256, 0, st>>>(scratch, G + m->emb_w, D, m->P, m->Ppad, accumulate);
    }
  }
  return iq_launch_status();
}

extern "C" int iq_model_backward(iq_model_t* m, const float* dlogits, const float* denc, int batch, void* workspace,
                                 size_t ws_bytes, int accumulate, int stage_hi, int stage_lo, iq_stream_t stream) {
  if (!m) return IQ_ERR_ARG;
  return backward_impl(m, dlogits, denc, batch, workspace, ws_bytes, accumulate, stage_hi, stage_lo, true, stream);
}

extern "C" int iq_model_backward_input(iq_model_t* m, const float* dlogits, const float* denc, int batch, void* workspace,
                                       size_t ws_bytes, float* dsrc, int flags, iq_stream_t stream) {
  if (!m) return IQ_ERR_ARG;
  if (flags & ~IQ_BWD_PARAM_GRADS) return fail(m, IQ_ERR_ARG, "backward_input: unknown flags");
  if (!dsrc) return fail(m, IQ_ERR_ARG, "backward_input: dsrc is NULL");
  if (!dlogits && !denc) return fail(m, IQ_ERR_ARG, "backward_input: dlogits or denc required");
  const bool pgrads = (flags & IQ_BWD_PARAM_GRADS) != 0;
  if (!m->params || !m->shadow || !m->pe) return fail(m, IQ_ERR_ARG, "backward_input: model not bound");
  if (pgrads && !m->grads) return fail(m, IQ_ERR_ARG, "backward_input: IQ_BWD_PARAM_GRADS needs a bound gradient buffer");
  WsPlan w;
  const int rc = maps_check(m, workspace, ws_bytes, batch, "backward_input", &w);
  if (rc != IQ_OK) return rc;
  const int rb = backward_impl(m, dlogits, denc, batch, workspace, ws_bytes, 0, m->c.n_layers + 1, 0, pgrads, stream);
  if (rb != IQ_OK) return rb;
  const iq_model_cfg_t& c = m->c;
  unsigned char* ws = (unsigned char*)workspace;
  const int kind = c.kind, H = kind == 0 ? c.img_h : c.seq_length, W = kind == 0 ? c.img_w : 0, p = kind == 0 ? c.patch : c.conv_k;
  IQ_TRY(iq_embed_dgrad(ws + w.demb, m->shadow + m->sh_embw, m->Ppad, dsrc, kind, batch, c.in_channels, H, W, p, c.d_model, stream),
         "embedding data gradient");
  return IQ_OK;
}

extern "C" int iq_model_attention_relevance(iq_model_t* m, const float* dlogits, int batch, void* workspace, size_t ws_bytes,
                                            float* rel, float* const* maps, int rows, int heads, int positive, long out_bstride,
                                            iq_stream_t stream) {
  if (!m) return IQ_ERR_ARG;
  if (!m->params || !m->shadow || !m->pe) return fail(m, IQ_ERR_ARG, "attention relevance: model not bound");
  if (!dlogits) return fail(m, IQ_ERR_ARG, "attention relevance: dlogits is NULL");
  WsPlan w;
  const int rc = maps_check(m, workspace, ws_bytes, batch, "attention relevance", &w);
  if (rc != IQ_OK) return rc;
  if (rows < 0 || rows > 2 || heads < 0 || heads > 1)
    return fail(m, IQ_ERR_ARG, "attention relevance: rows must be 0, 1 or 2 and heads 0 or 1");
  if (positive < 0 || positive > 1) return fail(m, IQ_ERR_ARG, "attention relevance: positive must be 0 or 1");
  const int L = m->c.n_layers, S = m->S, H = m->c.n_head;
  bool any_map = false;
  for (int l = 0; maps && l < L; ++l) any_map = any_map || maps[l];
  if (!rel && !any_map) return fail(m, IQ_ERR_ARG, "attention relevance: rel and every map are NULL");
  if (any_map && out_bstride < (long)(heads ? 1 : H) * S * (rows == 0 ? S : 1))
    return fail(m, IQ_ERR_ARG, "attention relevance: out_bstride too small");
  RelHook h;
  h.maps = maps; h.rows = rows; h.heads = heads; h.positive = positive; h.bstride = out_bstride; h.rel = rel;
  h.r[0] = (float*)((unsigned char*)workspace + w.demb);
  h.r[1] = h.r[0] + (size_t)batch * S;
  if (2 * (size_t)batch * S * sizeof(float) > (size_t)batch * m->tok * m->c.d_model * 2)
    return fail(m, IQ_ERR_UNSUPPORTED, "attention relevance: no room for the relevance vectors");
  if (L == 0) {
    if (rel) rel_start_kernel<<<blocks_for((size_t)batch * S), 256, 0, (hipStream_t)stream>>>(rel, batch * S, S, m->has_cls);
    return iq_launch_status() == IQ_OK ? IQ_OK : fail(m, IQ_ERR_LAUNCH, "attention relevance: start vector launch failed");
  }
  return backward_impl(m, dlogits, nullptr, batch, workspace, ws_bytes, 0, L + 1, 1, false, stream, &h);
}
```

### vit-vs-raw-iq_amd/trainer.py

```python
from __future__ import annotations

import ctypes as C
import math
from typing import List, Optional, Sequence, Tuple

import torch
import torch.distributed as dist

from . import _native as N
from .modules import NativePlan


def make_buckets(n_layers: int, n_buckets: int) -> List[Tuple[int, int]]:
    stages = list(range(n_layers + 1, -1, -1))
    n_buckets = max(1, min(n_buckets, len(stages)))
    per = math.ceil(len(stages) / n_buckets)
    out = []
    for i in range(0, len(stages), per):
        chunk = stages[i:i + per]
        out.append((chunk[0], chunk[-1]))
    return out


class BucketReducer:

    def __init__(self, group=None):
        self.group = group
        self.pending = []

    @property
    def world(self) -> int:
        return dist.get_world_size(self.group) if dist.is_available() and dist.is_initialized() else 1

    def launch(self, flat: torch.Tensor, off: int, length: int):
        if self.world == 1 or length == 0:
            return
        self.pending.append(dist.all_reduce(flat[off:off + length], op=dist.ReduceOp.SUM, group=self.group,
                                            async_op=True))

    def wait(self):
        for w in self.pending:
            w.wait()
        self.pending = []


def shard_indices(n: int, rank: int, world: int, epoch: int, seed: int = 0) -> torch.Tensor:
    g = torch.Generator().manual_seed(seed * 1_000_003 + epoch)
    perm = torch.randperm(n, generator=g)
    per = math.ceil(n / world)
    total = per * world
    if total > n:
        perm = torch.cat([perm, perm[: total - n]])
    return perm[rank:total:world]


class FusedTrainer:

    def __init__(self, model, lr=1e-4, weight_decay=1e-3, betas=(0.9, 0.99), eps=1e-8, label_smoothing=0.1,
                 max_norm=1.0, device=None, group=None, n_buckets: int = 4, use_graph: bool = False,
                 dropout_seed: Optional[int] = None, sync_params: bool = True):
        self.model = model
        self.device = torch.device(device) if device is not None else next(model.parameters()).device
        if self.device.type != "cuda":
            raise N.IqError("FusedTrainer needs the model on an MI355X (cuda) device; there is no CPU fallback")
        self.plan: NativePlan = model.native_plan()
        self.L = N.lib()
        self.lr, self.wd, self.betas, self.eps = lr, weight_decay, betas, eps
        self.smoothing, self.max_norm = label_smoothing, max_norm
        self.reducer = BucketReducer(group)
        self.world = self.reducer.world
        self.rank = dist.get_rank(group) if self.world > 1 else 0
        if dropout_seed is not None:
            self.plan.seed = int(dropout_seed)
        self.plan.seed = (self.plan.seed + 0x9E3779B97F4A7C15 * self.rank) & ((1 << 63) - 1)
        with torch.cuda.device(self.device):
            self.plan.ensure(self.device)
            if self.world > 1 and sync_params:
                self._sync_parameters()
        n = self.plan.nparam
        d = self.device
        self.gflat = torch.zeros(n, dtype=torch.float32, device=d)
        self.exp_avg = torch.zeros(n, dtype=torch.float32, device=d)
        self.exp_avg_sq = torch.zeros(n, dtype=torch.float32, device=d)
        self.loss_sum = torch.zeros(1, dtype=torch.float32, device=d)
        self.n_correct = torch.zeros(1, dtype=torch.int32, device=d)
        self.gnorm_sq = torch.zeros(1, dtype=torch.float32, device=d)
        self.gn_ws = torch.empty(self.L.iq_gradnorm_ws_bytes(n), dtype=torch.uint8, device=d)
        self.dyn = torch.tensor([lr, 0.0], dtype=torch.float32, device=d)
        self.frames_seen = 0
        self.steps = 0
        self.buckets = make_buckets(self.plan.cfg.n_layers, n_buckets if self.world > 1 else 1)
        self.ranges = [self.plan.grad_range(hi, lo) for hi, lo in self.buckets]
        self.use_graph = bool(use_graph)
        self._slots = {}
        self._slot = None
        self._logits = None
        self._dlogits = None
        self._batch = 0

    def _sync_parameters(self):
        plan, g = self.plan, self.reducer.group
        dist.broadcast(plan.flat, src=dist.get_global_rank(g, 0) if g is not None else 0, group=g)
        plan.mark_dirty()
        plan.ensure(self.device)
        flat = plan.flat.double()
        sig = torch.stack([flat.sum(), flat.abs().sum(), (flat * flat).sum()])
        lo, hi = sig.clone(), sig.clone()
        dist.all_reduce(lo, op=dist.ReduceOp.MIN, group=g)
        dist.all_reduce(hi, op=dist.ReduceOp.MAX, group=g)
        if not torch.equal(lo, hi):
            raise N.IqError(f"rank {self.rank}: parameters differ across ranks after the start-up broadcast "
                            f"(checksums {sig.tolist()} vs min {lo.tolist()} / max {hi.tolist()})")

    def set_lr(self, lr: float):
        self.lr = float(lr)
        self.dyn[0] = self.lr

    MAX_SLOTS = 4

    @property
    def _graphs(self):
        return self._slot["graphs"] if self._slot is not None else None

    @_graphs.setter
    def _graphs(self, value):
        if value is None:
            for sl in self._slots.values():
                sl["graphs"] = None
        elif self._slot is not None:
            self._slot["graphs"] = value

    def _buffers(self, B: int):
        if self._batch != B:
            sl = self._slots.pop(B, None)
            if sl is None:
                K = self.plan.cfg.num_classes
                sl = {"logits": torch.empty(B, K, dtype=torch.float32, device=self.device),
                      "dlogits": torch.empty(B, K, dtype=torch.float32, device=self.device),
                      "static": None, "graphs": None, "captured": None}
                while len(self._slots) >= self.MAX_SLOTS:
                    self._slots.pop(next(iter(self._slots)))
            self._slots[B] = sl
            self._slot = sl
            self._logits, self._dlogits = sl["logits"], sl["dlogits"]
            self._batch = B
        self.plan.workspace(B, self.device)

    def _pointers(self):
        p = self.plan
        return (p.ws.data_ptr(), p.ws.numel(), p.flat.data_ptr(), p.shadow.data_ptr(), p.step_ctr.data_ptr(),
                self._logits.data_ptr(), self._dlogits.data_ptr(), self.gflat.data_ptr(), self._batch)

    def _segments(self, x: torch.Tensor, y: torch.Tensor, auto_step: bool):
        plan, L = self.plan, self.L
        B = x.shape[0]
        ws = plan.ws
        step_arg = 0xFFFFFFFF if auto_step else (self.steps + 1) & 0x7FFFFFFF

        def fwd_and_first_bucket():
            st = N.stream_handle()
            N.check(L.iq_model_forward(plan.h, x.data_ptr(), B, ws.data_ptr(), ws.numel(), 1, plan.seed, step_arg, None,
                                       self._logits.data_ptr(), st), "iq_model_forward", plan.h)
            N.check(L.iq_ce_fwd_bwd(self._logits.data_ptr(), y.data_ptr(), B, plan.cfg.num_classes, self.smoothing,
                                    float(B), self.loss_sum.data_ptr(), self.n_correct.data_ptr(),
                                    self._dlogits.data_ptr(), st), "iq_ce_fwd_bwd")
            bwd(0)()

        def bwd(i):
            hi, lo = self.buckets[i]

            def run():
                N.check(L.iq_model_backward(plan.h, self._dlogits.data_ptr(), None, B, ws.data_ptr(), ws.numel(), 0, hi,
                                            lo, N.stream_handle()), "iq_model_backward", plan.h)
            return run

        def optimizer():
            st = N.stream_handle()
            gscale = 1.0 / self.world
            N.check(L.iq_gradnorm_sq(self.gflat.data_ptr(), plan.nparam, gscale, self.gn_ws.data_ptr(),
                                     self.gnorm_sq.data_ptr(), st), "iq_gradnorm_sq")
            N.check(L.iq_counter_add(None, 0, self.dyn.data_ptr() + 4, 1.0, st), "iq_counter_add")
            N.check(L.iq_adamw_step(plan.flat.data_ptr(), self.gflat.data_ptr(), self.exp_avg.data_ptr(),
                                    self.exp_avg_sq.data_ptr(), plan.shadow.data_ptr(), plan.nparam, self.lr,
                                    self.betas[0], self.betas[1], self.eps, self.wd, 0, self.gnorm_sq.data_ptr(),
                                    self.max_norm, gscale, self.dyn.data_ptr(), st), "iq_adamw_step")
            N.check(L.iq_model_refresh_transposed(plan.h, st), "iq_model_refresh_transposed", plan.h)

        return [fwd_and_first_bucket] + [bwd(i) for i in range(1, len(self.buckets))] + [optimizer]

    def _run_segments(self, runners):
        nb = len(self.buckets)
        for i, run in enumerate(runners):
            if i == nb:
                self.reducer.wait()
            run()
            if i < nb:
                off, ln = self.ranges[i]
                self.reducer.launch(self.gflat, off, ln)

    def step(self, x: torch.Tensor, y: torch.Tensor):
        if not x.is_cuda or not y.is_cuda:
            raise N.IqError("FusedTrainer.step expects device tensors (batch resident in HBM)")
        x = x.contiguous().float()
        y = y.contiguous().long()
        B = x.shape[0]
        plan = self.plan
        if not plan.is_bound(self.device):
            plan.ensure(self.device)
        self._buffers(B)
        if self.gflat is not plan.gflat:
            plan._bind_native(self.gflat)
        plan.generation += 1
        if self.use_graph:
            sl = self._slot
            if sl["graphs"] is not None and sl["captured"] != self._pointers():
                sl["graphs"] = None
            if plan.ctr_value != self.steps:
                plan.step_ctr.fill_(self.steps)
                plan.ctr_value = self.steps
            if sl["graphs"] is None:
                if sl["static"] is None or sl["static"][0].shape != x.shape:
                    sl["static"] = (torch.empty_like(x), torch.empty_like(y))
                static = sl["static"]
                static[0].copy_(x)
                static[1].copy_(y)
                self._run_segments(self._segments(static[0], static[1], auto_step=True))
                torch.cuda.synchronize()
                graphs = []
                for seg in self._segments(static[0], static[1], auto_step=True):
                    g = torch.cuda.CUDAGraph()
                    with torch.cuda.graph(g, capture_error_mode="thread_local"):
                        seg()
                    graphs.append(g)
                sl["graphs"] = graphs
                sl["captured"] = self._pointers()
            else:
                sl["static"][0].copy_(x, non_blocking=True)
                sl["static"][1].copy_(y, non_blocking=True)
                self._run_segments([g.replay for g in sl["graphs"]])
        else:
            self._run_segments(self._segments(x, y, auto_step=False))
        self.steps += 1
        self.frames_seen += B
        plan.step = self.steps
        plan.ctr_value = self.steps

    def read_stats(self, reset=True):
        t = torch.tensor([float(self.loss_sum.item()), float(self.n_correct.item()), float(self.frames_seen)],
                         dtype=torch.float64, device=self.device)
        if self.world > 1:
            dist.all_reduce(t, group=self.reducer.group)
        loss, correct, frames = t.tolist()
        if reset:
            self.loss_sum.zero_()
            self.n_correct.zero_()
            self.frames_seen = 0
        return loss / max(frames, 1.0), correct / max(frames, 1.0), int(frames)

    @torch.no_grad()
    def evaluate(self, x: torch.Tensor, y: torch.Tensor, batch: int = 256):
        was = self.model.training
        self.model.eval()
        K = self.plan.cfg.num_classes
        ls = torch.zeros(1, device=self.device)
        nc = torch.zeros(1, dtype=torch.int32, device=self.device)
        for i in range(0, x.shape[0], batch):
            xb, yb = x[i:i + batch].to(self.device), y[i:i + batch].to(self.device).long()
            logits = self.model(xb)
            N.check(self.L.iq_ce_fwd_bwd(logits.data_ptr(), yb.data_ptr(), xb.shape[0], K, self.smoothing,
                                         float(xb.shape[0]), ls.data_ptr(), nc.data_ptr(), None, N.stream_handle()),
                    "iq_ce_fwd_bwd")
        self.model.train(was)
        t = torch.tensor([ls.item(), float(nc.item()), float(x.shape[0])], dtype=torch.float64, device=self.device)
        if self.world > 1:
            dist.all_reduce(t, group=self.reducer.group)
        loss, correct, frames = t.tolist()
        return loss / frames, correct / frames
```

Baseline: 54370 frames/s.

## Fuse small launches: head+norm2 bwd, step counter into patchify, refresh kernels

Several small kernels are merged. Head backward is fused with the top layer's norm2 backward in a single launch. The step-counter set is folded into patchify. The embedding gather is combined with the cls gradient. The transpose refresh and embedding-weight cast run as one launch. The goal is to cut per-launch overhead and idle gaps at low occupancy in a graph-captured step, at the cost of more complex multi-role kernels with heterogeneous block work.

```diff
diff --git a/include/iqvit.h b/include/iqvit.h
--- a/include/iqvit.h
+++ b/include/iqvit.h
@@ -29,6 +29,11 @@
               void* dy, const iq_dropout_t* drop, float* dgamma, float* dbeta, float* ws, int accumulate, int M,
               int D, iq_stream_t stream);
 int iq_ln_bwd_partial_rows(int M, int D);
+int iq_head_ln_bwd_supported(int D);
+int iq_head_ln_bwd(const float* dlogits, const float* featn, const float* hstat, const float* hln_g, const float* hln_b,
+                   const float* W, float* dW, float* db, float* dhln_g, float* dhln_b, const void* z, const float* mean,
+                   const float* rstd, const float* gamma, void* dz, void* dy, const iq_dropout_t* drop, float* ln_ws, int B,
+                   int S, int D, int K, int accumulate, iq_stream_t stream);
 
 typedef struct iq_epilogue {
   const float* bias;
@@ -232,10 +237,14 @@
                          float* dx , int n_frames, int len, const iq_cyclic_t* par, iq_stream_t stream);
 int iq_patchify(const float* src, void* patches, int kind, int B, int C, int H, int W, int p, int Kpad,
                 iq_stream_t stream);
+int iq_patchify_step(const float* src, void* patches, int kind, int B, int C, int H, int W, int p, int Kpad,
+                     uint32_t* step_dev, uint32_t step, iq_stream_t stream);
 int iq_cls_rows(const float* cls, const float* pe, void* x0, int B, int S, int D, const iq_dropout_t* drop,
                 iq_stream_t stream);
 int iq_embed_bwd_gather(const void* dx0, void* demb, float* dcls, int B, int S, int tok, int D, int has_cls,
                         const iq_dropout_t* drop, int accumulate, iq_stream_t stream);
+int iq_embed_bwd_gather_dcls(const void* dx0, void* demb, float* dcls, int B, int S, int tok, int D,
+                             const iq_dropout_t* drop, int accumulate, iq_stream_t stream);
 int iq_embed_dgrad(const void* demb, const void* w_bf16, int Kpad, float* dsrc, int kind, int B, int C, int H, int W, int p,
                    int D, iq_stream_t stream);
 int iq_linf_step(float* x_adv, const float* grad, const float* x0, float alpha, float eps, float lo, float hi, size_t n,
@@ -282,6 +291,7 @@
 int iq_model_bind_step_counter(iq_model_t* m, uint32_t* counter);
 int iq_model_refresh_shadow(iq_model_t* m, iq_stream_t stream);
 int iq_model_refresh_transposed(iq_model_t* m, iq_stream_t stream);
+int iq_model_refresh_step(iq_model_t* m, iq_stream_t stream);
 int iq_model_forward(iq_model_t* m, const float* src, int batch, void* workspace, size_t ws_bytes, int training,
                      uint64_t seed, uint32_t step, float* enc_out, float* logits, iq_stream_t stream);
 int iq_model_backward(iq_model_t* m, const float* dlogits, const float* denc, int batch, void* workspace,
diff --git a/vit-vs-raw-iq_amd/_native.py b/vit-vs-raw-iq_amd/_native.py
--- a/vit-vs-raw-iq_amd/_native.py
+++ b/vit-vs-raw-iq_amd/_native.py
@@ -153,6 +153,11 @@
     "iq_head_fwd": (_I, [_P, _P, _P, _P, _P, _P, _P, _P, _I, _I, _I, _I, _I, _P]),
     "iq_ce_fwd_bwd": (_I, [_P, _P, _I, _I, _F, _F, _P, _P, _P, _P]),
     "iq_head_bwd": (_I, [_P, _P, _P, _P, _P, _P, _P, _P, _P, _P, _P, _I, _I, _I, _I, _I, _I, _P]),
+    "iq_head_ln_bwd_supported": (_I, [_I]),
+    "iq_head_ln_bwd": (_I, [_P, _P, _P, _P, _P, _P, _P, _P, _P, _P, _P, _P, _P, _P, _P, _P, C.POINTER(Dropout), _P, _I, _I, _I,
+                            _I, _I, _P]),
+    "iq_patchify_step": (_I, [_P, _P, _I, _I, _I, _I, _I, _I, _I, _P, _U32, _P]),
+    "iq_embed_bwd_gather_dcls": (_I, [_P, _P, _P, _I, _I, _I, _I, C.POINTER(Dropout), _I, _P]),
     "iq_gradnorm_ws_bytes": (_Z, [_Z]),
     "iq_gradnorm_sq": (_I, [_P, _Z, _F, _P, _P, _P]),
     "iq_adamw_step": (_I, [_P, _P, _P, _P, _P, _Z, _F, _F, _F, _F, _F, _I, _P, _F, _F, _P, _P]),
@@ -172,6 +177,7 @@
     "iq_model_bind_step_counter": (_I, [_P, _P]),
     "iq_model_refresh_shadow": (_I, [_P, _P]),
     "iq_model_refresh_transposed": (_I, [_P, _P]),
+    "iq_model_refresh_step": (_I, [_P, _P]),
     "iq_model_forward": (_I, [_P, _P, _I, _P, _Z, _I, _U64, _U32, _P, _P, _P]),
     "iq_model_backward": (_I, [_P, _P, _P, _I, _P, _Z, _I, _I, _I, _P]),
     "iq_model_grad_range": (_I, [_P, _I, _I, C.POINTER(_Z), C.POINTER(_Z)]),
diff --git a/vit-vs-raw-iq_amd/csrc/head_bwd.h b/vit-vs-raw-iq_amd/csrc/head_bwd.h
--- /dev/null
+++ b/vit-vs-raw-iq_amd/csrc/head_bwd.h
@@ -0,0 +1,146 @@
+#pragma once
+#include "common.h"
+
+struct HeadBwdArgs {
+  const float *dlogits, *feat_hat, *hstat, *ln_g, *ln_b, *W;
+  float *dW, *db, *dln_g, *dln_b;
+  int B, K, accumulate;
+};
+
+__device__ __forceinline__ void head_cls_grad(const float* __restrict__ dlogits, const float* __restrict__ feat_hat,
+                                              const float* __restrict__ hstat, const float* __restrict__ ln_g,
+                                              const float* __restrict__ W, float* df, int b, int D, int K, int lane) {
+#pragma clang fp contract(off)
+  const float* dl = dlogits + (long)b * K;
+  const float* fh = feat_hat + (long)b * D;
+  float s1 = 0.f, s2 = 0.f;
+  for (int d = lane; d < D; d += 64) {
+    float a = 0.f;
+    for (int k = 0; k < K; ++k) a = __builtin_fmaf(dl[k], W[(long)k * D + d], a);
+    if (ln_g) {
+      a *= ln_g[d];
+      s1 += a;
+      s2 += a * fh[d];
+    }
+    df[d] = a;
+  }
+  if (ln_g) {
+    const float c1 = wave_sum(s1) / (float)D, c2 = wave_sum(s2) / (float)D;
+    const float rstd = hstat[2 * b + 1];
+    for (int d = lane; d < D; d += 64) df[d] = rstd * __builtin_fmaf(-fh[d], c2, df[d] - c1);
+  }
+}
+
+__device__ __forceinline__ void head_bwd_w_body(int blk, const float* __restrict__ dlogits, const float* __restrict__ feat_hat,
+                                                const float* __restrict__ ln_g, const float* __restrict__ ln_b,
+                                                const float* __restrict__ W, float* __restrict__ dW, float* __restrict__ db,
+                                                float* __restrict__ dln_g, float* __restrict__ dln_b, int B, int D, int K,
+                                                int accumulate) {
+  __shared__ float sa[8][33], sb[8][33];
+  const int ol = threadIdx.x & 31, sl = threadIdx.x >> 5;
+  const int id = blk * 32 + ol;
+  const int k = id / D, d = id % D;
+  const bool live = k < K || (k == K && ln_g);
+  float a = 0.f, b2 = 0.f;
+  if (live) {
+    if (k < K) {
+      const float g = ln_g ? ln_g[d] : 1.f, be = ln_g ? ln_b[d] : 0.f;
+#pragma unroll 4
+      for (int b = sl; b < B; b += 8) {
+        const float dl = dlogits[(long)b * K + k];
+        a += dl * (g * feat_hat[(long)b * D + d] + be);
+        b2 += dl;
+      }
+    } else {
+      for (int b = sl; b < B; b += 8) {
+        float dfn = 0.f;
+        for (int kk = 0; kk < K; ++kk) dfn += dlogits[(long)b * K + kk] * W[(long)kk * D + d];
+        a += dfn * feat_hat[(long)b * D + d];
+        b2 += dfn;
+      }
+    }
+  }
+  sa[sl][ol] = a;
+  sb[sl][ol] = b2;
+  __syncthreads();
+  if (sl == 0 && live) {
+    float ta = 0.f, tb = 0.f;
+#pragma unroll
+    for (int i = 0; i < 8; ++i) { ta += sa[i][ol]; tb += sb[i][ol]; }
+    if (k < K) {
+      dW[(long)k * D + d] = accumulate ? dW[(long)k * D + d] + ta : ta;
+      if (d == 0) db[k] = accumulate ? db[k] + tb : tb;
+    } else {
+      dln_g[d] = accumulate ? dln_g[d] + ta : ta;
+      dln_b[d] = accumulate ? dln_b[d] + tb : tb;
+    }
+  }
+}
+
+template <int KMAX>
+__device__ __forceinline__ void head_bwd_w2_body(int blk, const float* __restrict__ dlogits, const float* __restrict__ feat_hat,
+                                                 const float* __restrict__ ln_g, const float* __restrict__ ln_b,
+                                                 const float* __restrict__ W, float* __restrict__ dW, float* __restrict__ db,
+                                                 float* __restrict__ dln_g, float* __restrict__ dln_b, int B, int D, int K,
+                                                 int accumulate) {
+  __shared__ float sT[8][KMAX][33];
+  __shared__ float sS[8][KMAX];
+  __shared__ float sdl[64][KMAX];
+  const int ol = threadIdx.x & 31, sl = threadIdx.x >> 5;
+  const int d = blk * 32 + ol;
+  const bool live = d < D;
+  float T[KMAX], sd[KMAX];
+#pragma unroll
+  for (int k = 0; k < KMAX; ++k) { T[k] = 0.f; sd[k] = 0.f; }
+  for (int b0 = 0; b0 < B; b0 += 64) {
+    __syncthreads();
+    for (int i = threadIdx.x; i < 64 * KMAX; i += 256) {
+      const int bb = i / KMAX, k = i - bb * KMAX;
+      sdl[bb][k] = (b0 + bb < B && k < K) ? dlogits[(long)(b0 + bb) * K + k] : 0.f;
+    }
+    __syncthreads();
+    float fv[8];
+#pragma unroll
+    for (int i = 0; i < 8; ++i) {
+      const int bb = sl + 8 * i;
+      fv[i] = (live && b0 + bb < B) ? feat_hat[(long)(b0 + bb) * D + d] : 0.f;
+    }
+#pragma unroll
+    for (int i = 0; i < 8; ++i) {
+      const int bb = sl + 8 * i;
+#pragma unroll
+      for (int k = 0; k < KMAX; ++k) {
+        const float dl = sdl[bb][k];
+        T[k] += dl * fv[i];
+        sd[k] += dl;
+      }
+    }
+  }
+#pragma unroll
+  for (int k = 0; k < KMAX; ++k) {
+    sT[sl][k][ol] = T[k];
+    if (ol == 0) sS[sl][k] = sd[k];
+  }
+  __syncthreads();
+  if (sl == 0 && live) {
+    const float g = ln_g ? ln_g[d] : 1.f, be = ln_g ? ln_b[d] : 0.f;
+    float lg = 0.f, lb = 0.f;
+    for (int k = 0; k < K; ++k) {
+      float t = 0.f, sk = 0.f;
+#pragma unroll
+      for (int i = 0; i < 8; ++i) { t += sT[i][k][ol]; sk += sS[i][k]; }
+      const float v = g * t + be * sk;
+      dW[(long)k * D + d] = accumulate ? dW[(long)k * D + d] + v : v;
+      if (d == 0) db[k] = accumulate ? db[k] + sk : sk;
+      const float w = W[(long)k * D + d];
+      lg += w * t;
+      lb += w * sk;
+    }
+    if (ln_g) {
+      dln_g[d] = accumulate ? dln_g[d] + lg : lg;
+      dln_b[d] = accumulate ? dln_b[d] + lb : lb;
+    }
+  }
+}
+
+inline int head_bwd_w_blocks(int D, int K) { return K <= 32 ? (D + 31) / 32 : ((K + 1) * D + 31) / 32; }
diff --git a/vit-vs-raw-iq_amd/csrc/layernorm.hip b/vit-vs-raw-iq_amd/csrc/layernorm.hip
--- a/vit-vs-raw-iq_amd/csrc/layernorm.hip
+++ b/vit-vs-raw-iq_amd/csrc/layernorm.hip
@@ -1,4 +1,5 @@
 #include "common.h"
+#include "head_bwd.h"
 #include "iqvit.h"
 #include "prof.h"
 
@@ -148,6 +149,108 @@
     float s = 0.f;
     for (int r = 0; r < RPB; ++r) s += red[r * 2 * D + c];
     partial[(long)blockIdx.x * 2 * D + c] = s;
+  }
+}
+
+template <int LPR, int NV, bool DROP, int KMAX>
+__global__ __launch_bounds__(LN_THREADS) void head_ln_bwd_kernel(HeadBwdArgs h, int wblocks, int S, const bf16* __restrict__ Z,
+                                                                 const float* __restrict__ mean_in, const float* __restrict__ rstd_in,
+                                                                 const float* __restrict__ gamma, bf16* __restrict__ dZ,
+                                                                 bf16* __restrict__ dY, IqRng rng, uint32_t thresh, float dscale,
+                                                                 float* __restrict__ partial, int M, int D) {
+  if ((int)blockIdx.x < wblocks) {
+    if constexpr (KMAX > 0)
+      head_bwd_w2_body<KMAX>(blockIdx.x, h.dlogits, h.feat_hat, h.ln_g, h.ln_b, h.W, h.dW, h.db, h.dln_g, h.dln_b, h.B, D, h.K, h.accumulate);
+    else
+      head_bwd_w_body(blockIdx.x, h.dlogits, h.feat_hat, h.ln_g, h.ln_b, h.W, h.dW, h.db, h.dln_g, h.dln_b, h.B, D, h.K, h.accumulate);
+    return;
+  }
+  const int blk = blockIdx.x - wblocks, nblk = gridDim.x - wblocks;
+  constexpr int RPW = 64 / LPR;
+  constexpr int RPB = RPW * (LN_THREADS / 64);
+  extern __shared__ __attribute__((aligned(16))) float red[];
+  float* gl = red;
+  const int lane = threadIdx.x & 63, wave = threadIdx.x >> 6;
+  const int j = lane % LPR, rsub = lane / LPR;
+  const int rslot = wave * RPW + rsub;
+  float g[NV][8], ag[NV][8], ab[NV][8];
+#pragma unroll
+  for (int v = 0; v < NV; ++v) {
+    const int c = (v * LPR + j) * 8;
+#pragma unroll
+    for (int e = 0; e < 8; ++e) { g[v][e] = gamma[c + e]; ag[v][e] = 0.f; ab[v][e] = 0.f; }
+  }
+  const float invD = 1.0f / (float)D;
+  if (DROP) rng = rng_resolve(rng);
+  for (long row0 = (long)blk * RPB; row0 < M; row0 += (long)nblk * RPB) {
+#pragma clang fp contract(off)
+    for (int r = wave; r < RPB; r += LN_THREADS / 64) {
+      const long rr = row0 + r;
+      if (rr < M && rr % S == 0) head_cls_grad(h.dlogits, h.feat_hat, h.hstat, h.ln_g, h.W, gl + r * D, (int)(rr / S), D, h.K, lane);
+    }
+    __syncthreads();
+    const long row = row0 + rslot;
+    const bool ok = row < M;
+    const bool cls = ok && row % S == 0;
+    float xh[NV][8], dy[NV][8];
+    float mean = 0.f, rstd = 0.f;
+    if (cls) { mean = mean_in[row]; rstd = rstd_in[row]; }
+    float s1 = 0.f, s2 = 0.f;
+#pragma unroll
+    for (int v = 0; v < NV; ++v) {
+      bf16x8 tz = {}, td = {};
+      if (cls) {
+        tz = *reinterpret_cast<const bf16x8*>(Z + row * D + (v * LPR + j) * 8);
+        td = pack8(gl + rslot * D + (v * LPR + j) * 8);
+      }
+      unpack8(tz, xh[v]);
+      unpack8(td, dy[v]);
+#pragma unroll
+      for (int e = 0; e < 8; ++e) {
+        xh[v][e] = (xh[v][e] - mean) * rstd;
+        ag[v][e] = __builtin_fmaf(dy[v][e], xh[v][e], ag[v][e]);
+        ab[v][e] += dy[v][e];
+        dy[v][e] *= g[v][e];
+        s1 += dy[v][e];
+        s2 += dy[v][e] * xh[v][e];
+      }
+    }
+    const float c1 = group_sum<LPR>(s1) * invD;
+    const float c2 = group_sum<LPR>(s2) * invD;
+    if (ok) {
+#pragma unroll
+      for (int v = 0; v < NV; ++v) {
+        float o[8];
+#pragma unroll
+        for (int e = 0; e < 8; ++e) o[e] = rstd * __builtin_fmaf(-xh[v][e], c2, dy[v][e] - c1);
+        const long off = row * D + (v * LPR + j) * 8;
+        *reinterpret_cast<bf16x8*>(dZ + off) = pack8(o);
+        if (DROP) {
+          if (cls) {
+            const uint32_t keep = dropout_keep8(rng, (uint64_t)off >> 3, thresh);
+#pragma unroll
+            for (int e = 0; e < 8; ++e) o[e] = ((keep >> e) & 1u) ? o[e] * dscale : 0.f;
+          }
+          *reinterpret_cast<bf16x8*>(dY + off) = pack8(o);
+        }
+      }
+    }
+    __syncthreads();
+  }
+#pragma unroll
+  for (int v = 0; v < NV; ++v) {
+    const int c = (v * LPR + j) * 8;
+#pragma unroll
+    for (int e = 0; e < 8; ++e) {
+      red[rslot * 2 * D + c + e] = ag[v][e];
+      red[rslot * 2 * D + D + c + e] = ab[v][e];
+    }
+  }
+  __syncthreads();
+  for (int c = threadIdx.x; c < 2 * D; c += LN_THREADS) {
+    float s = 0.f;
+    for (int r = 0; r < RPB; ++r) s += red[r * 2 * D + c];
+    partial[(long)blk * 2 * D + c] = s;
   }
 }
 
@@ -316,3 +419,60 @@
   if (!ok) return IQ_ERR_UNSUPPORTED;
   return rc != IQ_OK ? rc : iq_launch_status();
 }
+
+namespace {
+template <typename F>
+inline bool head_ln_dispatch(const LnShape& s, F&& f) {
+#define IQ_HLN_CASE(L, N) \
+  if (s.lpr == L && s.nv == N) { f(std::integral_constant<int, L>{}, std::integral_constant<int, N>{}); return true; }
+  IQ_HLN_CASE(16, 1) IQ_HLN_CASE(8, 3) IQ_HLN_CASE(32, 1) IQ_HLN_CASE(16, 3) IQ_HLN_CASE(64, 1) IQ_HLN_CASE(32, 3)
+#undef IQ_HLN_CASE
+  return false;
+}
+}
+
+extern "C" int iq_head_ln_bwd_supported(int D) {
+  LnShape s;
+  return ln_shape(D, &s) && head_ln_dispatch(s, [](auto, auto) {}) ? 1 : 0;
+}
+
+extern "C" int iq_head_ln_bwd(const float* dlogits, const float* featn, const float* hstat, const float* hln_g,
+                              const float* hln_b, const float* W, float* dW, float* db, float* dhln_g, float* dhln_b,
+                              const void* z, const float* mean, const float* rstd, const float* gamma, void* dz, void* dy,
+                              const iq_dropout_t* drop, float* ln_ws, int B, int S, int D, int K, int accumulate,
+                              iq_stream_t stream) {
+  LnShape s;
+  if (B <= 0) return IQ_OK;
+  if (!dlogits || !featn || !W || !dW || !db || S <= 0 || K <= 0) return IQ_ERR_ARG;
+  if (hln_g && (!hln_b || !hstat || !dhln_g || !dhln_b)) return IQ_ERR_ARG;
+  if (!z || !mean || !rstd || !gamma || !dz || !ln_ws) return IQ_ERR_ARG;
+  if ((long)B * S > 0x7fffffffL) return IQ_ERR_ARG;
+  if (!ln_shape(D, &s)) return IQ_ERR_UNSUPPORTED;
+  int dropping; IqRng rng; uint32_t thresh; float dscale;
+  (void)dropout_unpack(drop, &dropping, &rng, &thresh, &dscale);
+  if (dropping && !dy) return IQ_ERR_ARG;
+  hipStream_t st = (hipStream_t)stream;
+  IQ_PROF(IQ_FAM_MISC, st);
+  const int M = B * S;
+  const HeadBwdArgs h = {dlogits, featn, hstat, hln_g, hln_b, W, dW, db, dhln_g, dhln_b, B, K, accumulate};
+  const int wblocks = head_bwd_w_blocks(D, K);
+  const double bytes = 2.0 * (double)M * D * (1 + (dropping ? 1 : 0)) + 2.0 * B * D * 3 + 4.0 * B * (K + D) + 8.0 * K * D;
+  int rc = IQ_OK;
+  const bool ok = head_ln_dispatch(s, [&](auto lpr, auto nv) {
+    constexpr int LPR = decltype(lpr)::value, NV = decltype(nv)::value;
+    constexpr int RPB = (64 / LPR) * 4;
+    const int nblk = ln_grid(M, RPB);
+    const size_t lds = (size_t)RPB * 2 * D * sizeof(float);
+    if (lds > 64 * 1024) { rc = IQ_ERR_UNSUPPORTED; return; }
+    IQ_PROF_K(bytes, 4.0 * B * K * D, "head_ln_bwd_kernel<%d, %d, %s, %d>", LPR, NV, dropping ? "true" : "false", K <= 32 ? 32 : 0);
+    auto go = [&](auto k) {
+      (void)hipFuncSetAttribute((const void*)k, hipFuncAttributeMaxDynamicSharedMemorySize, (int)lds);
+      k<<<wblocks + nblk, LN_THREADS, lds, st>>>(h, wblocks, S, (const bf16*)z, mean, rstd, gamma, (bf16*)dz, (bf16*)dy, rng, thresh,
+                                                 dscale, ln_ws, M, D);
+    };
+    if (K <= 32) { if (dropping) go(head_ln_bwd_kernel<LPR, NV, true, 32>); else go(head_ln_bwd_kernel<LPR, NV, false, 32>); }
+    else         { if (dropping) go(head_ln_bwd_kernel<LPR, NV, true, 0>); else go(head_ln_bwd_kernel<LPR, NV, false, 0>); }
+  });
+  if (!ok) return IQ_ERR_UNSUPPORTED;
+  return rc != IQ_OK ? rc : iq_launch_status();
+}
diff --git a/vit-vs-raw-iq_amd/csrc/misc.hip b/vit-vs-raw-iq_amd/csrc/misc.hip
--- a/vit-vs-raw-iq_amd/csrc/misc.hip
+++ b/vit-vs-raw-iq_amd/csrc/misc.hip
@@ -1,11 +1,13 @@
 #include "common.h"
+#include "head_bwd.h"
 #include "iqvit.h"
 #include "prof.h"
 
 namespace {
 
 __global__ void patchify_kernel(const float* __restrict__ src, bf16* __restrict__ dst, int kind, int B, int C, int H,
-                                int W, int p, int tok, int P, int Kpad) {
+                                int W, int p, int tok, int P, int Kpad, uint32_t* step_dev, uint32_t step, int bump) {
+  if (step_dev && blockIdx.x == 0 && threadIdx.x == 0) *step_dev = bump ? *step_dev + 1u : step;
   const long nchunk = (long)B * tok * (Kpad / 8);
   for (long id = (long)blockIdx.x * blockDim.x + threadIdx.x; id < nchunk; id += (long)gridDim.x * blockDim.x) {
     const int ch = (int)(id % (Kpad / 8));
@@ -62,12 +64,13 @@
   *reinterpret_cast<bf16x8*>(x0 + off) = pack8(v);
 }
 
-__global__ void embed_bwd_gather_kernel(const bf16* __restrict__ dx0, bf16* __restrict__ demb, int B, int S, int tok,
-                                        int D, int cls_off, int drop_on, IqRng rng, uint32_t thresh, float dscale) {
+__device__ __forceinline__ void embed_bwd_gather_body(int blk, int nblk, const bf16* __restrict__ dx0, bf16* __restrict__ demb,
+                                                      int B, int S, int tok, int D, int cls_off, int drop_on, IqRng rng,
+                                                      uint32_t thresh, float dscale) {
   const int nch = D / 8;
   const long n = (long)B * tok * nch;
   if (drop_on) rng = rng_resolve(rng);
-  for (long id = (long)blockIdx.x * blockDim.x + threadIdx.x; id < n; id += (long)gridDim.x * blockDim.x) {
+  for (long id = (long)blk * blockDim.x + threadIdx.x; id < n; id += (long)nblk * blockDim.x) {
     const int ch = (int)(id % nch);
     const long row = id / nch;
     const int b = (int)(row / tok), t = (int)(row % tok);
@@ -85,10 +88,15 @@
   }
 }
 
-__global__ __launch_bounds__(256) void dcls_kernel(const bf16* __restrict__ dx0, float* __restrict__ dcls, int B, int S, int D,
-                                                   int drop_on, IqRng rng, uint32_t thresh, float dscale, int accumulate) {
+__global__ void embed_bwd_gather_kernel(const bf16* __restrict__ dx0, bf16* __restrict__ demb, int B, int S, int tok,
+                                        int D, int cls_off, int drop_on, IqRng rng, uint32_t thresh, float dscale) {
+  embed_bwd_gather_body(blockIdx.x, gridDim.x, dx0, demb, B, S, tok, D, cls_off, drop_on, rng, thresh, dscale);
+}
+
+__device__ __forceinline__ void dcls_body(int ch, const bf16* __restrict__ dx0, float* __restrict__ dcls, int B, int S, int D,
+                                          int drop_on, IqRng rng, uint32_t thresh, float dscale, int accumulate) {
   __shared__ float part[4][8];
-  const int ch = blockIdx.x, lane = threadIdx.x & 63, wave = threadIdx.x >> 6;
+  const int lane = threadIdx.x & 63, wave = threadIdx.x >> 6;
   if (drop_on) rng = rng_resolve(rng);
   float s[8] = {0.f, 0.f, 0.f, 0.f, 0.f, 0.f, 0.f, 0.f};
   for (int b = threadIdx.x; b < B; b += 256) {
@@ -111,6 +119,20 @@
     float* dst = dcls + ch * 8 + threadIdx.x;
     *dst = accumulate ? *dst + t : t;
   }
+}
+
+__global__ __launch_bounds__(256) void dcls_kernel(const bf16* __restrict__ dx0, float* __restrict__ dcls, int B, int S, int D,
+                                                   int drop_on, IqRng rng, uint32_t thresh, float dscale, int accumulate) {
+  dcls_body(blockIdx.x, dx0, dcls, B, S, D, drop_on, rng, thresh, dscale, accumulate);
+}
+
+__global__ __launch_bounds__(256) void embed_bwd_gather_dcls_kernel(const bf16* __restrict__ dx0, bf16* __restrict__ demb,
+                                                                    float* __restrict__ dcls, int B, int S, int tok, int D,
+                                                                    int drop_on, IqRng rng, uint32_t thresh, float dscale,
+                                                                    int accumulate) {
+  const int nc = D / 8;
+  if ((int)blockIdx.x < nc) dcls_body(blockIdx.x, dx0, dcls, B, S, D, drop_on, rng, thresh, dscale, accumulate);
+  else embed_bwd_gather_body(blockIdx.x - nc, gridDim.x - nc, dx0, demb, B, S, tok, D, 1, drop_on, rng, thresh, dscale);
 }
 
 __global__ __launch_bounds__(64) void head_fwd_kernel(const bf16* __restrict__ x, const float* __restrict__ ln_g,
@@ -271,26 +293,7 @@
                                                          int D, int K, int pool) {
   extern __shared__ float df[];
   const int b = blockIdx.x, lane = threadIdx.x & 63;
-  const float* dl = dlogits + (long)b * K;
-  const float* fh = feat_hat + (long)b * D;
-  if (threadIdx.x < 64) {
-    float s1 = 0.f, s2 = 0.f;
-    for (int d = lane; d < D; d += 64) {
-      float a = 0.f;
-      for (int k = 0; k < K; ++k) a += dl[k] * W[(long)k * D + d];
-      if (ln_g) {
-        a *= ln_g[d];
-        s1 += a;
-        s2 += a * fh[d];
-      }
-      df[d] = a;
-    }
-    if (ln_g) {
-      const float c1 = wave_sum(s1) / (float)D, c2 = wave_sum(s2) / (float)D;
-      const float rstd = hstat[2 * b + 1];
-      for (int d = lane; d < D; d += 64) df[d] = rstd * (df[d] - c1 - fh[d] * c2);
-    }
-  }
+  if (threadIdx.x < 64) head_cls_grad(dlogits, feat_hat, hstat, ln_g, W, df, b, D, K, lane);
   __syncthreads();
   bf16* dxb = dx + (long)b * S * D;
   const float inv = 1.0f / (float)S;
@@ -308,45 +311,7 @@
                                                          const float* __restrict__ W, float* __restrict__ dW, float* __restrict__ db,
                                                          float* __restrict__ dln_g, float* __restrict__ dln_b, int B, int D, int K,
                                                          int accumulate) {
-  __shared__ float sa[8][33], sb[8][33];
-  const int ol = threadIdx.x & 31, sl = threadIdx.x >> 5;
-  const int id = blockIdx.x * 32 + ol;
-  const int k = id / D, d = id % D;
-  const bool live = k < K || (k == K && ln_g);
-  float a = 0.f, b2 = 0.f;
-  if (live) {
-    if (k < K) {
-      const float g = ln_g ? ln_g[d] : 1.f, be = ln_g ? ln_b[d] : 0.f;
-#pragma unroll 4
-      for (int b = sl; b < B; b += 8) {
-        const float dl = dlogits[(long)b * K + k];
-        a += dl * (g * feat_hat[(long)b * D + d] + be);
-        b2 += dl;
-      }
-    } else {
-      for (int b = sl; b < B; b += 8) {
-        float dfn = 0.f;
-        for (int kk = 0; kk < K; ++kk) dfn += dlogits[(long)b * K + kk] * W[(long)kk * D + d];
-        a += dfn * feat_hat[(long)b * D + d];
-        b2 += dfn;
-      }
-    }
-  }
-  sa[sl][ol] = a;
-  sb[sl][ol] = b2;
-  __syncthreads();
-  if (sl == 0 && live) {
-    float ta = 0.f, tb = 0.f;
-#pragma unroll
-    for (int i = 0; i < 8; ++i) { ta += sa[i][ol]; tb += sb[i][ol]; }
-    if (k < K) {
-      dW[(long)k * D + d] = accumulate ? dW[(long)k * D + d] + ta : ta;
-      if (d == 0) db[k] = accumulate ? db[k] + tb : tb;
-    } else {
-      dln_g[d] = accumulate ? dln_g[d] + ta : ta;
-      dln_b[d] = accumulate ? dln_b[d] + tb : tb;
-    }
-  }
+  head_bwd_w_body(blockIdx.x, dlogits, feat_hat, ln_g, ln_b, W, dW, db, dln_g, dln_b, B, D, K, accumulate);
 }
 
 template <int KMAX>
@@ -355,64 +320,7 @@
                                                           const float* __restrict__ W, float* __restrict__ dW, float* __restrict__ db,
                                                           float* __restrict__ dln_g, float* __restrict__ dln_b, int B, int D, int K,
                                                           int accumulate) {
-  __shared__ float sT[8][KMAX][33];
-  __shared__ float sS[8][KMAX];
-  __shared__ float sdl[64][KMAX];
-  const int ol = threadIdx.x & 31, sl = threadIdx.x >> 5;
-  const int d = blockIdx.x * 32 + ol;
-  const bool live = d < D;
-  float T[KMAX], sd[KMAX];
-#pragma unroll
-  for (int k = 0; k < KMAX; ++k) { T[k] = 0.f; sd[k] = 0.f; }
-  for (int b0 = 0; b0 < B; b0 += 64) {
-    __syncthreads();
-    for (int i = threadIdx.x; i < 64 * KMAX; i += 256) {
-      const int bb = i / KMAX, k = i - bb * KMAX;
-      sdl[bb][k] = (b0 + bb < B && k < K) ? dlogits[(long)(b0 + bb) * K + k] : 0.f;
-    }
-    __syncthreads();
-    float fv[8];
-#pragma unroll
-    for (int i = 0; i < 8; ++i) {
-      const int bb = sl + 8 * i;
-      fv[i] = (live && b0 + bb < B) ? feat_hat[(long)(b0 + bb) * D + d] : 0.f;
-    }
-#pragma unroll
-    for (int i = 0; i < 8; ++i) {
-      const int bb = sl + 8 * i;
-#pragma unroll
-      for (int k = 0; k < KMAX; ++k) {
-        const float dl = sdl[bb][k];
-        T[k] += dl * fv[i];
-        sd[k] += dl;
-      }
-    }
-  }
-#pragma unroll
-  for (int k = 0; k < KMAX; ++k) {
-    sT[sl][k][ol] = T[k];
-    if (ol == 0) sS[sl][k] = sd[k];
-  }
-  __syncthreads();
-  if (sl == 0 && live) {
-    const float g = ln_g ? ln_g[d] : 1.f, be = ln_g ? ln_b[d] : 0.f;
-    float lg = 0.f, lb = 0.f;
-    for (int k = 0; k < K; ++k) {
-      float t = 0.f, sk = 0.f;
-#pragma unroll
-      for (int i = 0; i < 8; ++i) { t += sT[i][k][ol]; sk += sS[i][k]; }
-      const float v = g * t + be * sk;
-      dW[(long)k * D + d] = accumulate ? dW[(long)k * D + d] + v : v;
-      if (d == 0) db[k] = accumulate ? db[k] + sk : sk;
-      const float w = W[(long)k * D + d];
-      lg += w * t;
-      lb += w * sk;
-    }
-    if (ln_g) {
-      dln_g[d] = accumulate ? dln_g[d] + lg : lg;
-      dln_b[d] = accumulate ? dln_b[d] + lb : lb;
-    }
-  }
+  head_bwd_w2_body<KMAX>(blockIdx.x, dlogits, feat_hat, ln_g, ln_b, W, dW, db, dln_g, dln_b, B, D, K, accumulate);
 }
 
 constexpr int GN_BLOCKS = 1024;
@@ -534,8 +442,13 @@
 
 extern "C" int iq_patchify(const float* src, void* patches, int kind, int B, int C, int H, int W, int p, int Kpad,
                            iq_stream_t stream) {
-  IQ_PROF(IQ_FAM_MISC, stream);
-  if (B <= 0) return IQ_OK;
+  return iq_patchify_step(src, patches, kind, B, C, H, W, p, Kpad, nullptr, 0, stream);
+}
+
+extern "C" int iq_patchify_step(const float* src, void* patches, int kind, int B, int C, int H, int W, int p, int Kpad,
+                                uint32_t* step_dev, uint32_t step, iq_stream_t stream) {
+  IQ_PROF(IQ_FAM_MISC, stream);
+  if (B <= 0) return step_dev ? IQ_ERR_ARG : IQ_OK;
   if (!src || !patches || C <= 0 || H <= 0 || p <= 0 || (Kpad % 8)) return IQ_ERR_ARG;
   int tok, P;
   if (kind == 0) {
@@ -548,8 +461,9 @@
   }
   if (tok <= 0 || Kpad < P) return IQ_ERR_ARG;
   const size_t n = (size_t)B * tok * (Kpad / 8);
+  if (step_dev) IQ_PROF_K(4.0 * B * C * H * (kind == 0 ? W : 1) + 2.0 * B * tok * Kpad, 0.0, "patchify_kernel");
   patchify_kernel<<<grid_for(n, 256, 4096), 256, 0, (hipStream_t)stream>>>(src, (bf16*)patches, kind, B, C, H, W, p, tok,
-                                                                          P, Kpad);
+                                                                          P, Kpad, step_dev, step, step == 0xFFFFFFFFu ? 1 : 0);
   return iq_launch_status();
 }
 
@@ -577,6 +491,20 @@
   embed_bwd_gather_kernel<<<grid_for(n, 256, 4096), 256, 0, st>>>((const bf16*)dx0, (bf16*)demb, B, S, tok, D,
                                                                   has_cls ? 1 : 0, on, r, th, sc);
   if (has_cls) dcls_kernel<<<D / 8, 256, 0, st>>>((const bf16*)dx0, dcls, B, S, D, on, r, th, sc, accumulate);
+  return iq_launch_status();
+}
+
+extern "C" int iq_embed_bwd_gather_dcls(const void* dx0, void* demb, float* dcls, int B, int S, int tok, int D,
+                                        const iq_dropout_t* drop, int accumulate, iq_stream_t stream) {
+  IQ_PROF(IQ_FAM_MISC, stream);
+  if (B <= 0) return IQ_OK;
+  if (!dx0 || !demb || !dcls || D <= 0 || (D % 8)) return IQ_ERR_ARG;
+  int on; IqRng r; uint32_t th; float sc;
+  (void)dropout_unpack(drop, &on, &r, &th, &sc);
+  const size_t n = (size_t)B * tok * (D / 8);
+  IQ_PROF_K(4.0 * n * 8 + 2.0 * B * D, 0.0, "embed_bwd_gather_dcls_kernel");
+  embed_bwd_gather_dcls_kernel<<<D / 8 + grid_for(n, 256, 4096), 256, 0, (hipStream_t)stream>>>(
+      (const bf16*)dx0, (bf16*)demb, dcls, B, S, tok, D, on, r, th, sc, accumulate);
   return iq_launch_status();
 }
 
diff --git a/vit-vs-raw-iq_amd/csrc/model.hip b/vit-vs-raw-iq_amd/csrc/model.hip
--- a/vit-vs-raw-iq_amd/csrc/model.hip
+++ b/vit-vs-raw-iq_amd/csrc/model.hip
@@ -61,12 +61,16 @@
     reinterpret_cast<bf16x8*>(d)[i] = pack8(f);
   }
 }
-__global__ void cast_pad_kernel(const float* __restrict__ s, bf16* __restrict__ d, int rows, int cols, int ld) {
+__device__ __forceinline__ void cast_pad_body(int blk, int nblk, const float* __restrict__ s, bf16* __restrict__ d, int rows,
+                                              int cols, int ld) {
   const long n = (long)rows * ld;
-  for (long i = (long)blockIdx.x * blockDim.x + threadIdx.x; i < n; i += (long)gridDim.x * blockDim.x) {
+  for (long i = (long)blk * blockDim.x + threadIdx.x; i < n; i += (long)nblk * blockDim.x) {
     const int r = (int)(i / ld), c = (int)(i % ld);
     d[i] = (bf16)(c < cols ? s[(long)r * cols + c] : 0.f);
   }
+}
+__global__ void cast_pad_kernel(const float* __restrict__ s, bf16* __restrict__ d, int rows, int cols, int ld) {
+  cast_pad_body(blockIdx.x, gridDim.x, s, d, rows, cols, ld);
 }
 __global__ void unpad_kernel(const float* __restrict__ s, float* __restrict__ d, int rows, int cols, int ld, int add) {
   const long n = (long)rows * cols;
@@ -77,8 +81,8 @@
   }
 }
 struct TransDesc { unsigned long long src_off, dst_off; int rows, cols, tile0, tiles_x; };
-__global__ __launch_bounds__(256) void transpose_table_kernel(const float* __restrict__ params, unsigned char* __restrict__ shadow,
-                                                              const TransDesc* __restrict__ tab, int nent) {
+__device__ __forceinline__ void transpose_table_body(const float* __restrict__ params, unsigned char* __restrict__ shadow,
+                                                     const TransDesc* __restrict__ tab, int nent) {
   __shared__ float t[32][33];
   int e = 0;
   while (e + 1 < nent && (int)blockIdx.x >= tab[e + 1].tile0) ++e;
@@ -98,6 +102,17 @@
     if (c < d.cols && r < d.rows) dst[(long)c * d.rows + r] = (bf16)t[tx][i];
   }
 }
+__global__ __launch_bounds__(256) void transpose_table_kernel(const float* __restrict__ params, unsigned char* __restrict__ shadow,
+                                                              const TransDesc* __restrict__ tab, int nent) {
+  transpose_table_body(params, shadow, tab, nent);
+}
+__global__ __launch_bounds__(256) void refresh_step_kernel(const float* __restrict__ params, unsigned char* __restrict__ shadow,
+                                                           const TransDesc* __restrict__ tab, int nent, int ttiles,
+                                                           const float* __restrict__ embw, bf16* __restrict__ embw_sh, int rows,
+                                                           int cols, int ld) {
+  if ((int)blockIdx.x < ttiles) transpose_table_body(params, shadow, tab, nent);
+  else cast_pad_body(blockIdx.x - ttiles, gridDim.x - ttiles, embw, embw_sh, rows, cols, ld);
+}
 
 __global__ void rel_start_kernel(float* r, int n, int S, int cls) {
   for (int i = blockIdx.x * blockDim.x + threadIdx.x; i < n; i += gridDim.x * blockDim.x) {
@@ -113,10 +128,6 @@
   float* rel;
   float* r[2];
 };
-
-__global__ void set_u32_kernel(uint32_t* p, uint32_t v, int bump) {
-  if (threadIdx.x == 0 && blockIdx.x == 0) *p = bump ? *p + 1u : v;
-}
 
 inline int blocks_for(size_t n, int cap = 4096) {
   size_t b = (n + 255) / 256;
@@ -438,6 +449,18 @@
 
 extern "C" int iq_model_refresh_shadow(iq_model_t* m, iq_stream_t stream) { return refresh_impl(m, true, stream); }
 extern "C" int iq_model_refresh_transposed(iq_model_t* m, iq_stream_t stream) { return refresh_impl(m, false, stream); }
+extern "C" int iq_model_refresh_step(iq_model_t* m, iq_stream_t stream) {
+  if (!m || !m->params || !m->shadow) return fail(m, IQ_ERR_ARG, "refresh_step: model not bound");
+  if (m->ttiles <= 0) return refresh_impl(m, false, stream);
+  hipStream_t st = (hipStream_t)stream;
+  const int D = m->c.d_model;
+  IQ_PROF(IQ_FAM_MISC, st);
+  IQ_PROF_K(6.0 * m->ttiles * 1024 + 6.0 * D * m->Ppad, 0.0, "refresh_step_kernel");
+  refresh_step_kernel<<<m->ttiles + blocks_for((size_t)D * m->Ppad), 256, 0, st>>>(
+      m->params, m->shadow, (const TransDesc*)(m->shadow + m->sh_table), (int)m->ttab.size(), m->ttiles, m->params + m->emb_w,
+      (bf16*)(m->shadow + m->sh_embw), D, m->P, m->Ppad);
+  return iq_launch_status();
+}
 
 extern "C" int iq_model_forward(iq_model_t* m, const float* src, int batch, void* workspace, size_t ws_bytes,
                                 int training, uint64_t seed, uint32_t step, float* enc_out, float* logits,
@@ -458,15 +481,13 @@
   uint32_t* step_dev = m->step_ctr ? m->step_ctr : (uint32_t*)(ws + w.step_ctr);
   m->last_tr = tr;
   m->last_train_fwd = true;
-  if (tr) {
-    set_u32_kernel<<<1, 64, 0, st>>>(step_dev, step, step == 0xFFFFFFFFu ? 1 : 0);
-    m->last_seed = seed;
-  }
+  if (tr) m->last_seed = seed;
   const float* P = m->params;
   m->fwd_ws = nullptr;
 
-  if (c.kind == 0) IQ_TRY(iq_patchify(src, ws + w.patches, 0, B, c.in_channels, c.img_h, c.img_w, c.patch, m->Ppad, stream), "patchify");
-  else IQ_TRY(iq_patchify(src, ws + w.patches, 1, B, c.in_channels, c.seq_length, 0, c.conv_k, m->Ppad, stream), "patchify");
+  uint32_t* set_step = tr ? step_dev : nullptr;
+  if (c.kind == 0) IQ_TRY(iq_patchify_step(src, ws + w.patches, 0, B, c.in_channels, c.img_h, c.img_w, c.patch, m->Ppad, set_step, step, stream), "patchify");
+  else IQ_TRY(iq_patchify_step(src, ws + w.patches, 1, B, c.in_channels, c.seq_length, 0, c.conv_k, m->Ppad, set_step, step, stream), "patchify");
   const iq_dropout_t d0 = site(m, seed, step_dev, 0, tr);
   if (m->has_cls) IQ_TRY(iq_cls_rows(P + m->cls, m->pe, ws + w.x0, B, S, D, &d0, stream), "cls rows");
   {
@@ -622,9 +643,21 @@
   float* wws = (float*)(ws + w.wgrad_ws);
   const float dscale = tr ? dropout_scale(c.drop_prob) : 1.f;
 
+  const bool head_ln = stage_hi == Lr + 1 && stage_lo <= Lr && Lr >= 1 && dlogits && !denc && pgrads && m->pool == 0 &&
+                       iq_head_ln_bwd_supported(D) != 0;
+  auto ln2_part_of = [&](int layer) { return (float*)(ws + w.ln_part[(layer & 1) ? 2 : 0]); };
   if (stage_hi == Lr + 1) {
     if (!dlogits && !denc) return fail(m, IQ_ERR_ARG, "backward: dlogits or denc required at the head stage");
-    if (dlogits && !pgrads) {
+    if (head_ln) {
+      const LayerOff& o = m->L[Lr - 1];
+      const WsPlan::L& a = w.layers[Lr - 1];
+      const iq_dropout_t dr2 = m->bwd_site(3 + 3 * (Lr - 1), step_dev, tr);
+      IQ_TRY(iq_head_ln_bwd(dlogits, (const float*)(ws + w.head_feat), (const float*)(ws + w.head_stat),
+                            m->head_ln ? P + m->hln_g : nullptr, m->head_ln ? P + m->hln_b : nullptr, P + m->head_w,
+                            G + m->head_w, G + m->head_b, m->head_ln ? G + m->hln_g : nullptr, m->head_ln ? G + m->hln_b : nullptr,
+                            ws + a.z2, (const float*)(ws + a.mean2), (const float*)(ws + a.rstd2), P + o.g2, ws + w.gZ, ws + w.gY,
+                            &dr2, ln2_part_of(Lr - 1), B, S, D, K, accumulate, stream), "head bwd + top norm2 bwd");
+    } else if (dlogits && !pgrads) {
       IQ_TRY(head_bwd_dx_launch(dlogits, (const float*)(ws + w.head_feat), (const float*)(ws + w.head_stat),
                                 m->head_ln ? P + m->hln_g : nullptr, P + m->head_w, ws + w.gA, B, S, D, K, m->pool, st), "head bwd (dx)");
     } else if (dlogits) {
@@ -649,11 +682,11 @@
     unsigned char *gZ = ws + w.gZ, *gY = ws + w.gY, *gZ1 = ws + w.gZ1, *gY1 = ws + w.gY1;
     unsigned char *gH = ws + w.gH, *gQKV = ws + w.gQKV;
     iq_epilogue_t e;
-    auto ln2_part = [&](int layer) { return (float*)(ws + w.ln_part[(layer & 1) ? 2 : 0]); };
+    auto ln2_part = ln2_part_of;
     float* lp2 = ln2_part(l);
     float* lp1 = (float*)(ws + w.ln_part[1]);
     const bool norm2_here = l == Lr - 1 || !fuse2;
-    if (norm2_here) {
+    if (norm2_here && !(head_ln && l == Lr - 1)) {
       const iq_dropout_t dr2 = m->bwd_site(3 + 3 * l, step_dev, tr);
       IQ_TRY(iq_ln_bwd(ws + w.gA, ws + a.z2, (const float*)(ws + a.mean2), (const float*)(ws + a.rstd2), P + o.g2,
                        gZ, gY, &dr2, nullptr, nullptr, lp2, accumulate, M, D, stream), "norm2 bwd");
@@ -741,8 +774,12 @@
       IQ_TRY(embed_bwd_gather_launch(ws + w.gA, ws + w.demb, B, S, m->tok, D, m->has_cls, &dr0, st), "embedding bwd gather");
       return iq_launch_status();
     }
-    IQ_TRY(iq_embed_bwd_gather(ws + w.gA, ws + w.demb, m->has_cls ? G + m->cls : nullptr, B, S, m->tok, D, m->has_cls,
-                               &dr0, accumulate, stream), "embedding bwd gather");
+    if (m->has_cls)
+      IQ_TRY(iq_embed_bwd_gather_dcls(ws + w.gA, ws + w.demb, G + m->cls, B, S, m->tok, D, &dr0, accumulate, stream),
+             "embedding bwd gather + cls gradient");
+    else
+      IQ_TRY(iq_embed_bwd_gather(ws + w.gA, ws + w.demb, nullptr, B, S, m->tok, D, 0, &dr0, accumulate, stream),
+             "embedding bwd gather");
     if (m->Ppad == m->P) {
       IQ_TRY(iq_gemm_bf16_wgrad(ws + w.demb, D, ws + w.patches, m->Ppad, G + m->emb_w, G + m->emb_b, MT, D, m->Ppad, wws,
                                 w.wgrad_ws_bytes, accumulate, stream), "embedding wgrad");
diff --git a/vit-vs-raw-iq_amd/trainer.py b/vit-vs-raw-iq_amd/trainer.py
--- a/vit-vs-raw-iq_amd/trainer.py
+++ b/vit-vs-raw-iq_amd/trainer.py
@@ -184,7 +184,7 @@
                                     self.exp_avg_sq.data_ptr(), plan.shadow.data_ptr(), plan.nparam, self.lr,
                                     self.betas[0], self.betas[1], self.eps, self.wd, 0, self.gnorm_sq.data_ptr(),
                                     self.max_norm, gscale, self.dyn.data_ptr(), st), "iq_adamw_step")
-            N.check(L.iq_model_refresh_transposed(plan.h, st), "iq_model_refresh_transposed", plan.h)
+            N.check(L.iq_model_refresh_step(plan.h, st), "iq_model_refresh_step", plan.h)
 
         return [fwd_and_first_bucket] + [bwd(i) for i in range(1, len(self.buckets))] + [optimizer]
 
```

Result: no change. 54620 frames/s, median of 6 (+0.5%).
